# shao-chi/Image-Caption

Measured on AMD Instinct MI355X. Metric: train images/sec @ batch=64, 36×2048 feats, seq_len=20; 1/2/4/8 MI355X, higher is better.
Workload: dtype bf16; 1 GPU; C2 train step: B=64/GPU, N=36 regions x F=2048, P=84, T=20, 6+6 blocks d=512 h=8 f=2048, V=10000, dropout 0.3/0.1, Adam lr 5e-4; global_batch=64, seq_len=20, parallelism=dp1

## Files before the change

image-caption_amd/capgen/_lib.py:

```python
from __future__ import annotations

import ctypes as C
import os

import torch

_HERE = os.path.dirname(os.path.abspath(__file__))
LIB_PATH = os.environ.get("CAPGEN_LIB_PATH") or os.path.join(_HERE, "libcapgen.so")
ABI_VERSION = 13

F32, BF16 = 0, 1


class capgen_config(C.Structure):
    _fields_ = [
        ("num_vocab", C.c_int32), ("max_length", C.c_int32),
        ("dim_features", C.c_int32), ("dim_positions", C.c_int32),
        ("enc_d", C.c_int32), ("enc_ff", C.c_int32), ("enc_blocks", C.c_int32), ("enc_heads", C.c_int32),
        ("dim_word_embedding", C.c_int32),
        ("dec_d", C.c_int32), ("dec_ff", C.c_int32), ("dec_blocks", C.c_int32), ("dec_heads", C.c_int32),
        ("dropout", C.c_float), ("attention_dropout", C.c_float),
        ("pad_idx", C.c_int32), ("encode_mask", C.c_int32), ("focal_loss", C.c_int32),
        ("split_position", C.c_int32), ("split_image_objects", C.c_int32),
        ("move_first_image_feature", C.c_int32),
        ("dtype", C.c_int32), ("max_batch", C.c_int32), ("max_regions", C.c_int32),
        ("lr", C.c_float), ("beta1", C.c_float), ("beta2", C.c_float), ("eps", C.c_float),
        ("seed", C.c_uint64),
    ]


class capgen_param_info(C.Structure):
    _fields_ = [("name", C.c_char * 96), ("ndim", C.c_int32), ("rows", C.c_int64), ("cols", C.c_int64),
                ("offset", C.c_int64), ("row_stride", C.c_int64)]


_P = C.c_void_p
_SIGS = {
    "capgen_last_error": (C.c_char_p, []),
    "capgen_abi_version": (C.c_int, []),
    "capgen_set_knob": (C.c_int, [C.c_char_p, C.c_int, _P]),
    "capgen_debug_build": (C.c_int, []),
    "capgen_param_table": (C.c_int, [C.POINTER(capgen_config), C.POINTER(capgen_param_info), C.c_int,
                                     C.POINTER(C.c_int), C.POINTER(C.c_int64)]),
    "capgen_create": (C.c_int, [C.POINTER(capgen_config), C.c_int, C.POINTER(_P)]),
    "capgen_destroy": (C.c_int, [_P]),
    "capgen_get_params": (C.c_int, [_P, _P, C.c_int64]),
    "capgen_set_params": (C.c_int, [_P, _P, C.c_int64]),
    "capgen_get_grads": (C.c_int, [_P, _P, C.c_int64]),
    "capgen_set_grads": (C.c_int, [_P, _P, C.c_int64]),
    "capgen_get_adam_state": (C.c_int, [_P, C.POINTER(C.c_int64), _P, _P, C.c_int64]),
    "capgen_set_adam_state": (C.c_int, [_P, C.c_int64, _P, _P, C.c_int64]),
    "capgen_arenas": (C.c_int, [_P, C.POINTER(_P), C.POINTER(_P), C.POINTER(C.c_int64)]),
    "capgen_set_training": (C.c_int, [_P, C.c_int]),
    "capgen_set_graph": (C.c_int, [_P, C.c_int]),
    "capgen_set_decode_log_softmax": (C.c_int, [_P, C.c_int]),
    "capgen_set_lr": (C.c_int, [_P, C.c_float]),
    "capgen_get_lr": (C.c_int, [_P, C.POINTER(C.c_float)]),
    "capgen_set_grad_clip": (C.c_int, [_P, C.c_float]),
    "capgen_last_grad_norm": (C.c_int, [_P, C.POINTER(C.c_float)]),
    "capgen_forward": (C.c_int, [_P, _P, C.c_int, _P, _P, C.c_int, C.c_int, C.c_int, _P, _P]),
    "capgen_backward": (C.c_int, [_P, _P]),
    "capgen_adam_step": (C.c_int, [_P, _P]),
    "capgen_train_step": (C.c_int, [_P, _P, C.c_int, _P, _P, C.c_int, C.c_int, C.c_int, _P, _P]),
    "capgen_compute_loss": (C.c_int, [_P, _P, C.c_int, _P, _P, C.c_int, C.c_int, C.c_int, _P, _P]),
    "capgen_copy_logits": (C.c_int, [_P, _P, C.c_int64, _P]),
    "capgen_greedy": (C.c_int, [_P, _P, C.c_int, _P, C.c_int, C.c_int, _P, _P, _P]),
    "capgen_beam": (C.c_int, [_P, _P, C.c_int, _P, C.c_int, C.c_int, C.c_int, _P, _P]),
    "capgen_sample": (C.c_int, [_P, _P, C.c_int, _P, C.c_int, C.c_int, C.c_int, C.c_float, C.c_int, C.c_uint64, _P, _P,
                                _P]),
    "capgen_sample_nucleus": (C.c_int, [_P, _P, C.c_int, _P, C.c_int, C.c_int, C.c_int, C.c_float, C.c_int, C.c_float,
                                        C.c_uint64, _P, _P, _P]),
    "capgen_set_rng_seed": (C.c_int, [_P, C.c_uint64]),
    "capgen_debug_gemm": (C.c_int, [C.c_int, C.c_int, C.c_int, _P, C.c_int64, C.c_int, _P, C.c_int64, C.c_int,
                                    _P, C.c_int64, C.c_int, C.c_int, _P, C.c_float, C.c_int, C.c_int, _P]),
    "capgen_debug_gemm_tiled": (C.c_int, [C.c_int, C.c_int, C.c_int, _P, C.c_int64, _P, C.c_int64, C.c_int, _P, _P,
                                          C.c_int64, C.c_int, _P, C.c_int, C.c_int, _P, C.c_int64, _P]),
    "capgen_debug_gemm_tiled_ln": (C.c_int, [C.c_int, C.c_int, _P, _P, _P, _P, _P, C.c_int, _P, C.c_int, C.c_int, _P, _P,
                                             _P, _P, C.c_int64, C.c_int, _P]),
    "capgen_debug_gemm_variant": (C.c_int, [C.c_int]),
    "capgen_debug_splitk_protocol": (C.c_int, [C.c_int]),
    "capgen_debug_splitk_diag": (C.c_int, [_P, C.c_int]),
    "capgen_debug_gemm_timing_buf": (C.c_int, [_P]),
    "capgen_debug_copy_buffer": (C.c_int, [_P, C.c_int, _P, C.c_int64]),
    "capgen_train_step_indexed": (C.c_int, [_P, _P, C.c_int, _P, C.c_int, _P, _P, C.c_int, C.c_int, C.c_int, _P,
                                            _P]),
    "capgen_train_step_weighted": (C.c_int, [_P, _P, C.c_int, _P, C.c_int, _P, _P, _P, C.c_int, C.c_int, C.c_int, _P,
                                             C.c_int, _P]),
    "capgen_rl_sample": (C.c_int, [_P, _P, C.c_int, _P, _P, C.c_int, C.c_int, C.c_int, _P, _P, _P, _P]),
    "capgen_rl_finish": (C.c_int, [_P, _P, C.c_float, _P, C.c_int, _P]),
    "capgen_debug_attention": (C.c_int, [C.c_int, C.c_int, C.c_int, C.c_int, C.c_int, C.c_int, _P, _P, _P, _P,
                                         C.c_int, C.c_float, _P, _P, _P, _P, _P, _P, _P]),
    "capgen_debug_attention_bwd_wo": (C.c_int, [C.c_int, C.c_int, C.c_int, C.c_int, _P, _P, _P, _P, C.c_int, _P, _P,
                                                _P, _P, _P, _P]),
    "capgen_debug_qkv_attention": (C.c_int, [C.c_int, C.c_int, C.c_int, _P, _P, _P, _P, _P, _P, C.c_int, C.c_int, _P]),
    "capgen_debug_cross_attention": (C.c_int, [C.c_int, C.c_int, C.c_int, C.c_int, _P, _P, _P, _P, _P, _P, _P]),
    "capgen_debug_layernorm_fwd": (C.c_int, [C.c_int, C.c_int, C.c_int, _P, _P, C.c_float, C.c_int, C.c_uint64, _P, _P,
                                             C.c_int, _P, _P, _P, C.c_int64, C.c_int, _P, _P, _P, _P, _P, _P]),
    "capgen_debug_layernorm_bwd": (C.c_int, [C.c_int, C.c_int, C.c_int, _P, _P, _P, _P, _P, _P, C.c_int64, C.c_int, _P,
                                             C.c_float, C.c_int, C.c_uint64, _P, _P, _P, _P, _P, C.c_int, C.c_int64,
                                             _P]),
    "capgen_debug_column_sum": (C.c_int, [C.c_int, _P, C.c_int, C.c_int, C.c_int64, C.c_float, _P, _P, C.c_int,
                                          C.c_int64, _P]),
    "capgen_debug_stripe_reduce": (C.c_int, [_P, C.c_int, C.c_int64, C.c_int64, _P, C.c_int, C.c_int, _P]),
    "capgen_debug_embedding_gather": (C.c_int, [_P, _P, C.c_int64, C.c_int, C.c_int, _P, C.c_int, _P]),
    "capgen_debug_embedding_scatter_add": (C.c_int, [_P, _P, C.c_int, C.c_int, C.c_int, _P, C.c_int, _P]),
    "capgen_debug_pack_encoder_input": (C.c_int, [_P, C.c_int, _P, C.c_int, C.c_int, C.c_int, C.c_int, _P, C.c_int, _P,
                                                  _P, C.c_int, C.c_int, _P, _P]),
    "capgen_debug_prepare_captions": (C.c_int, [_P, C.c_int, C.c_int, C.c_int, _P, _P, _P, _P, _P, _P]),
    "capgen_debug_cross_entropy_rows": (C.c_int, [_P, _P, C.c_int, C.c_int, C.c_int, _P, _P, C.c_int, _P]),
    "capgen_debug_ce_finish": (C.c_int, [_P, C.c_int64, _P, _P, C.c_int, C.c_int, C.c_int, _P, _P, _P]),
    "capgen_debug_cross_entropy_rows_weighted": (C.c_int, [_P, _P, _P, C.c_int, C.c_int, C.c_int, C.c_int, _P, _P,
                                                           C.c_int, _P]),
    "capgen_debug_ce_finish_weighted": (C.c_int, [_P, C.c_int64, _P, _P, _P, C.c_int, C.c_int, C.c_int, C.c_int, _P,
                                                  _P, _P]),
    "capgen_debug_loss_finalize": (C.c_int, [_P, C.c_int, _P, C.c_int, _P, _P, _P, C.c_int, _P]),
    "capgen_debug_adam": (C.c_int, [_P, _P, _P, _P, C.c_int64, C.c_float, C.c_float, C.c_float, C.c_float, _P, _P, _P,
                                    C.c_int64, C.c_int, C.c_int, C.POINTER(C.c_int64), C.POINTER(C.c_int64),
                                    C.POINTER(_P), _P]),
    "capgen_debug_adam_scaled": (C.c_int, [_P, _P, _P, _P, C.c_int64, C.c_float, C.c_float, C.c_float, C.c_float, _P, _P,
                                           _P, C.c_int64, C.c_int, C.c_int, C.POINTER(C.c_int64), C.POINTER(C.c_int64),
                                           C.POINTER(_P), _P, _P]),
    "capgen_debug_grad_norm": (C.c_int, [_P, C.c_int64, C.c_float, C.c_int, _P, C.c_int, _P, _P]),
    "capgen_debug_to_bf16": (C.c_int, [_P, _P, C.c_int64, _P]),
    "capgen_debug_arena_checksum": (C.c_int, [_P, C.c_int64, C.POINTER(C.c_uint64), _P]),
    "capgen_debug_argmax_softmax": (C.c_int, [_P, C.c_int, C.c_int, _P, C.c_int64, C.c_int, _P, C.c_int64, C.c_int,
                                              _P]),
    "capgen_debug_sample_softmax": (C.c_int, [_P, C.c_int, C.c_int, C.c_float, C.c_int, C.c_uint64, C.c_uint32, _P,
                                              C.c_int64, C.c_int, _P, C.c_int64, _P, C.c_int64, C.c_int, _P]),
    "capgen_debug_sample_nucleus": (C.c_int, [_P, C.c_int, C.c_int, C.c_float, C.c_int, C.c_float, C.c_uint64,
                                              C.c_uint32, _P, C.c_int64, C.c_int, _P, C.c_int64, _P, C.c_int64,
                                              C.c_int, _P, _P]),
    "capgen_debug_slab_argmax": (C.c_int, [_P, _P, C.c_int, C.c_int, _P, C.c_int64, C.c_int, _P, C.c_int64, _P]),
    "capgen_debug_beam_step_topk": (C.c_int, [_P, _P, _P, C.c_int, C.c_int, C.c_int, C.c_int, C.c_int, _P, _P, _P, _P,
                                              _P, _P]),
    "capgen_debug_beam_slab_step": (C.c_int, [_P, _P, _P, C.c_int, C.c_int, C.c_int, C.c_int, C.c_int, _P, _P, _P, _P,
                                              _P, C.c_int, _P, _P, _P, _P, C.c_int, C.c_int, _P]),
    "capgen_debug_rl_rows": (C.c_int, [_P, C.c_int, C.c_int, _P, _P, _P, _P, _P]),
    "capgen_debug_rl_image": (C.c_int, [_P, _P, C.c_int, C.c_int, _P, _P, _P]),
    "capgen_debug_rl_numer": (C.c_int, [_P, _P, _P, C.c_int, C.c_int, _P, _P]),
    "capgen_debug_rl_loss": (C.c_int, [_P, _P, C.c_float, _P, _P, _P]),
    "capgen_debug_rl_grad": (C.c_int, [_P, _P, _P, _P, _P, _P, _P, C.c_int, C.c_int, C.c_int, C.c_int, C.c_float, _P,
                                       C.c_int, _P]),
    "capgen_debug_gemm_classifier": (C.c_int, [C.c_int, C.c_int, C.c_int, _P, C.c_int64, _P, C.c_int64, _P, C.c_int64,
                                               _P, _P, C.c_int64, _P, _P, _P]),
    "capgen_dp_unique_id": (C.c_int, [C.c_char_p]),
    "capgen_dp_init": (C.c_int, [_P, C.c_char_p, C.c_int, C.c_int]),
    "capgen_dp_set_global_count": (C.c_int, [_P, C.c_float]),
    "capgen_dp_sync_adam_state": (C.c_int, [_P]),
    "capgen_dp_comm_info": (C.c_int, [_P, _P, _P]),
    "capgen_dp_check": (C.c_int, [_P, _P, _P]),
    "capgen_params_checksum": (C.c_int, [_P, _P]),
    "capgen_dp_buckets": (C.c_int, [_P, _P, _P, C.c_int, _P]),
    "capgen_dp_debug_shard": (C.c_int, [_P, C.c_int, C.c_int]),
    "capgen_tune_load": (C.c_int, [C.c_char_p]),
    "capgen_tune_save": (C.c_int, [C.c_char_p]),
    "capgen_tune_live_count": (C.c_int, []),
    "capgen_debug_hazard": (C.c_int, [C.c_int, C.c_char_p, C.c_int, C.POINTER(C.c_int)]),
    "capgen_debug_side_delay": (C.c_int, [C.c_double]),
    "capgen_debug_collectives": (C.c_int, [_P, C.c_int, C.c_char_p, C.c_int]),
    "capgen_debug_stamps": (C.c_int, [_P, C.c_int, _P, C.c_int, C.c_char_p, C.c_int]),
    "capgen_scst_rewards": (C.c_int, [_P, C.c_int64, _P, C.c_int64, C.c_int, C.c_int, C.c_int, C.c_int, C.c_int,
                                      C.c_int64, C.c_double, C.c_double, _P]),
}
EXPORTED = tuple(_SIGS)

_lib = None


def load():
    global _lib
    if _lib is not None:
        return _lib
    if not os.path.exists(LIB_PATH):
        raise ImportError(f"capgen: {LIB_PATH} is missing — build it with "
                          "`python -c 'import __graft_entry__ as g; g.build()'` (make -C image-caption_amd/csrc)")
    lib = C.CDLL(LIB_PATH)
    for name, (res, args) in _SIGS.items():
        fn = getattr(lib, name)
        fn.restype = res
        fn.argtypes = args
    if lib.capgen_abi_version() != ABI_VERSION:
        raise ImportError("capgen: libcapgen.so ABI version mismatch")
    _lib = lib
    return lib


def check(rc: int) -> None:
    if rc != 0:
        raise RuntimeError("capgen: " + load().capgen_last_error().decode(errors="replace"))


def to_c_config(cfg) -> capgen_config:
    cfg.check_supported()
    c = capgen_config()
    c.num_vocab, c.max_length = cfg.num_vocab, cfg.max_length
    c.dim_features, c.dim_positions = cfg.encode_dim_features, cfg.encode_dim_positions
    c.enc_d, c.enc_ff = cfg.encode_input_size, cfg.encode_hidden_size
    c.enc_blocks, c.enc_heads = cfg.encode_num_blocks, cfg.encode_num_heads
    c.dim_word_embedding = cfg.dim_word_embedding
    c.dec_d, c.dec_ff = cfg.decode_input_size, cfg.decode_hidden_size
    c.dec_blocks, c.dec_heads = cfg.decode_num_blocks, cfg.decode_num_heads
    c.dropout, c.attention_dropout = cfg.dropout, cfg.attention_dropout
    c.pad_idx, c.encode_mask, c.focal_loss = cfg.pad_idx, int(cfg.encode_mask), int(cfg.focal_loss)
    c.split_position = int(cfg.split_position)
    c.split_image_objects = int(cfg.split_image_objects)
    c.move_first_image_feature = int(cfg.move_first_image_feature)
    c.dtype = F32 if cfg.dtype == "fp32" else BF16
    c.max_batch, c.max_regions = cfg.max_batch, cfg.max_regions
    c.lr, c.beta1, c.beta2, c.eps = cfg.learning_rate, cfg.beta1, cfg.beta2, cfg.eps
    c.seed = cfg.seed & 0xFFFFFFFFFFFFFFFF
    return c


def param_table(cfg):
    lib = load()
    c = to_c_config(cfg)
    n = C.c_int(0)
    total = C.c_int64(0)
    check(lib.capgen_param_table(C.byref(c), None, 0, C.byref(n), C.byref(total)))
    arr = (capgen_param_info * n.value)()
    check(lib.capgen_param_table(C.byref(c), arr, n.value, C.byref(n), C.byref(total)))
    out = [(p.name.decode(), p.ndim, p.rows, p.cols, p.offset, p.row_stride) for p in arr]
    return out, total.value


TUNE_TABLE = os.path.join(_HERE, "tune_gfx950.txt")


def tune_save(path: str = TUNE_TABLE) -> int:
    n = load().capgen_tune_save(path.encode())
    if n < 0:
        check(1)
    return n


def tune_load(path: str) -> int:
    return load().capgen_tune_load(path.encode())


def tune_live_count() -> int:
    return load().capgen_tune_live_count()


def hazard_start() -> None:
    check(load().capgen_debug_hazard(1, None, 0, None))


def hazard_stop() -> None:
    check(load().capgen_debug_hazard(0, None, 0, None))


def hazard_check(cap: int = 8192):
    buf = C.create_string_buffer(cap)
    n = C.c_int(0)
    check(load().capgen_debug_hazard(2, buf, cap, C.byref(n)))
    return n.value, buf.value.decode(errors="replace")


def side_delay(us: float) -> None:
    check(load().capgen_debug_side_delay(float(us)))
# ... 11 lines not shown
```

image-caption_amd/csrc/attn_mfma_dev.h:

```cpp
#pragma once
#include "attention.h"

namespace capgen {
namespace amf {

typedef __attribute__((ext_vector_type(8))) __bf16 bf16x8;
typedef __attribute__((ext_vector_type(4))) float f32x4;
typedef __attribute__((ext_vector_type(4))) __bf16 bf16x4;
typedef short s4 __attribute__((ext_vector_type(4)));
typedef __attribute__((address_space(3))) s4 lds_s4;

constexpr int DK = 64;
constexpr int IMG = 64 * 128;

__device__ __forceinline__ int swz(int k, int chunk) { return chunk ^ (((k >> 1) & 3) << 1); }

__device__ __forceinline__ bf16x8 frag_t(const char* img, int cb, int ks, int lane) {
  const int g = lane >> 4, i = lane & 15, q = i >> 2, p = i & 3;
  const int k = ks * 32 + 4 * g + q;
  const int ch = (cb >> 3) + (p >> 1), sub = (p & 1) * 8;
  const s4 lo = __builtin_amdgcn_ds_read_tr16_b64_v4i16((lds_s4*)(img + k * 128 + swz(k, ch) * 16 + sub));
  const s4 hi = __builtin_amdgcn_ds_read_tr16_b64_v4i16((lds_s4*)(img + (k + 16) * 128 + swz(k + 16, ch) * 16 + sub));
  return __builtin_bit_cast(bf16x8, __builtin_shufflevector(lo, hi, 0, 1, 2, 3, 4, 5, 6, 7));
}
// ... 11 lines not shown
                           : uint4{0u, 0u, 0u, 0u};
    }
#pragma unroll
  for (int i = 0; i < NI; ++i)
#pragma unroll
    for (int u = 0; u < 2; ++u) {
      const int c = tid + 256 * u, row = c >> 3, ch = c & 7;
      *reinterpret_cast<uint4*>(img[i] + row * 128 + swz(row, ch) * 16) = v[i][u];
    }
}

__device__ __forceinline__ void stage_key_ok(unsigned char* kok, const AttnGeom& g, int b, int tid) {
  if (tid < 64) {
    const int j = tid;
    bool ok = j < g.Lk;
    if (ok && g.key_valid) ok = g.key_valid[(int64_t)(g.kv_bmod ? b % g.kv_bmod : b) * g.kv_bs + j] != 0;
    if (ok && g.key_ids) ok = g.key_ids[(int64_t)b * g.kid_bs + j] != g.pad_idx;
    kok[j] = ok;
  }
}

__device__ __forceinline__ void put4(char* img, int row, int col, f32x4 v) {
  const bf16x4 b = {(bf16)v[0], (bf16)v[1], (bf16)v[2], (bf16)v[3]};
  *reinterpret_cast<bf16x4*>(img + row * 128 + swz(row, col >> 3) * 16 + (col & 7) * 2) = b;
}

__device__ __forceinline__ bf16x8 frag_r(const char* img, int row, int ks, int lane) {
  return *reinterpret_cast<const bf16x8*>(img + row * 128 + swz(row, ks * 4 + (lane >> 4)) * 16);
}

__device__ __forceinline__ void scores(const char* Aimg, int q0, const char* Bimg, int lane, f32x4 (&s)[4]) {
  const bf16x8 a0 = frag_r(Aimg, q0 + (lane & 15), 0, lane), a1 = frag_r(Aimg, q0 + (lane & 15), 1, lane);
#pragma unroll
  for (int j = 0; j < 4; ++j) {
    s[j] = f32x4{0.f, 0.f, 0.f, 0.f};
    s[j] = __builtin_amdgcn_mfma_f32_16x16x32_bf16(frag_r(Bimg, 16 * j + (lane & 15), 0, lane), a0, s[j], 0, 0, 0);
    s[j] = __builtin_amdgcn_mfma_f32_16x16x32_bf16(frag_r(Bimg, 16 * j + (lane & 15), 1, lane), a1, s[j], 0, 0, 0);
  }
}

__device__ __forceinline__ void softmax_rows(const AttnGeom& g, const unsigned char* kok, int q, int lane,
                                             const f32x4 (&s)[4], f32x4 (&p)[4]) {
  const float inv_t = 1.f / g.temperature;
  float mx = -INFINITY;
  f32x4 x[4];
#pragma unroll
  for (int j = 0; j < 4; ++j)
#pragma unroll
    for (int r = 0; r < 4; ++r) {
      const int key = 16 * j + 4 * (lane >> 4) + r;
      const bool m = !kok[key] || (g.causal && key > g.q_pos0 + q);
      x[j][r] = m ? -INFINITY : s[j][r] * inv_t;
      mx = fmaxf(mx, x[j][r]);
    }
  mx = fmaxf(mx, __shfl_xor(mx, 16, 64));
  mx = fmaxf(mx, __shfl_xor(mx, 32, 64));
  float sum = 0.f;
#pragma unroll
  for (int j = 0; j < 4; ++j)
#pragma unroll
    for (int r = 0; r < 4; ++r) {
      x[j][r] = expf(x[j][r] - mx);
      sum += x[j][r];
    }
  sum += __shfl_xor(sum, 16, 64);
  sum += __shfl_xor(sum, 32, 64);
#pragma unroll
  for (int j = 0; j < 4; ++j)
#pragma unroll
    for (int r = 0; r < 4; ++r) p[j][r] = x[j][r] / sum;
}

__device__ __forceinline__ bf16x8 pack8(const f32x4& lo, const f32x4& hi) {
  return bf16x8{(bf16)lo[0], (bf16)lo[1], (bf16)lo[2], (bf16)lo[3], (bf16)hi[0], (bf16)hi[1], (bf16)hi[2], (bf16)hi[3]};
}

__device__ __forceinline__ void store4(bf16* p, f32x4 v, float mul) {
  *reinterpret_cast<bf16x4*>(p) = bf16x4{(bf16)(v[0] * mul), (bf16)(v[1] * mul), (bf16)(v[2] * mul), (bf16)(v[3] * mul)};
}


__device__ __forceinline__ void attn_fwd_images(const AttnGeom& g, bf16* __restrict__ o, float* __restrict__ probs,
                                                int b, int h, const char* Qimg, const char* Kimg, const char* Vimg,
                                                const unsigned char* kok) {
  const int tid = threadIdx.x, lane = tid & 63, w = tid >> 6;
  const int q0 = 16 * w, q = q0 + (lane & 15);
  if (q0 >= g.Lq) return;
  f32x4 s[4], p[4];
  scores(Qimg, q0, Kimg, lane, s);
  softmax_rows(g, kok, q, lane, s, p);
  const int64_t row_idx = (((int64_t)b * g.H + h) * g.Lq + q) * g.Lk;
  if (probs && q < g.Lq) {
#pragma unroll
    for (int j = 0; j < 4; ++j)
#pragma unroll
      for (int r = 0; r < 4; ++r) {
        const int key = 16 * j + 4 * (lane >> 4) + r;
        if (key < g.Lk) probs[row_idx + key] = p[j][r];
      }
  }
  if (g.drop.seed_ptr) {
    const uint64_t seed = *g.drop.seed_ptr;
#pragma unroll
    for (int j = 0; j < 4; ++j)
#pragma unroll
      for (int r = 0; r < 4; ++r) {
        const int key = 16 * j + 4 * (lane >> 4) + r;
        const bool keep = drop_keep(seed, g.drop.site, (uint32_t)(row_idx + key), g.drop.thresh);
        p[j][r] = keep ? p[j][r] * g.drop.scale : 0.f;
      }
  }
  const bf16x8 pf0 = pack8(p[0], p[1]), pf1 = pack8(p[2], p[3]);
  bf16* ob = o + (int64_t)b * g.o_bs + h * DK;
#pragma unroll
  for (int t = 0; t < 4; ++t) {
    f32x4 acc = f32x4{0.f, 0.f, 0.f, 0.f};
    acc = __builtin_amdgcn_mfma_f32_16x16x32_bf16(frag_t(Vimg, 16 * t, 0, lane), pf0, acc, 0, 0, 0);
    acc = __builtin_amdgcn_mfma_f32_16x16x32_bf16(frag_t(Vimg, 16 * t, 1, lane), pf1, acc, 0, 0, 0);
    if (q < g.Lq) store4(ob + (int64_t)q * g.o_ld + 16 * t + 4 * (lane >> 4), acc, 1.f);
  }
}

__device__ __forceinline__ void attn_fwd_staged(const AttnGeom& g, bf16* __restrict__ o, float* __restrict__ probs,
                                                int b, int h, const char* sm) {
  attn_fwd_images(g, o, probs, b, h, sm, sm + IMG, sm + 2 * IMG, reinterpret_cast<const unsigned char*>(sm + 3 * IMG));
}

__device__ __forceinline__ void attn_fwd_one(const AttnGeom& g, bf16* __restrict__ o, float* __restrict__ probs, int b,
                                             int h, char* sm) {
  char* Qimg = sm;
  char* Kimg = sm + IMG;
  char* Vimg = sm + 2 * IMG;
  unsigned char* kok = reinterpret_cast<unsigned char*>(sm + 3 * IMG);
  const int tid = threadIdx.x;
  const int bk = g.kv_bmod ? b % g.kv_bmod : b;
  {
    char* const img[3] = {Qimg, Kimg, Vimg};
    const bf16* const src[3] = {reinterpret_cast<const bf16*>(g.q) + (int64_t)b * g.q_bs + h * DK,
                                reinterpret_cast<const bf16*>(g.k) + (int64_t)bk * g.k_bs + h * DK,
                                reinterpret_cast<const bf16*>(g.v) + (int64_t)bk * g.v_bs + h * DK};
    const int64_t ld[3] = {g.q_ld, g.k_ld, g.v_ld};
    const int L[3] = {g.Lq, g.Lk, g.Lk};
    stage_images<3>(img, src, ld, L, tid);
    stage_key_ok(kok, g, b, tid);
  }
  __syncthreads();
  attn_fwd_staged(g, o, probs, b, h, sm);
}

__device__ __forceinline__ void attn_bwd_staged(const AttnGeom& g, bf16* __restrict__ dq, bf16* __restrict__ dkp,
                                                bf16* __restrict__ dvp, int b, int h, const char* Kimg,
                                                const char* dOimg, const char* Qimg, const char* Vimg, char* Pdimg,
                                                char* dSimg, const unsigned char* kok) {
  const int tid = threadIdx.x, lane = tid & 63, w = tid >> 6;
  const int64_t qoff = (int64_t)b * g.q_bs + h * DK, koff = (int64_t)b * g.k_bs + h * DK,
                voff = (int64_t)b * g.v_bs + h * DK;
  const int q0 = 16 * w, q = q0 + (lane & 15);
  const float inv_t = 1.f / g.temperature;
  f32x4 ds[4], pd[4];
  if (q0 < g.Lq) {
    f32x4 s[4], p[4], dp[4];
    scores(Qimg, q0, Kimg, lane, s);
    softmax_rows(g, kok, q, lane, s, p);
    scores(dOimg, q0, Vimg, lane, dp);
    const int64_t row_idx = (((int64_t)b * g.H + h) * g.Lq + q) * g.Lk;
    const uint64_t seed = g.drop.seed_ptr ? *g.drop.seed_ptr : 0;
    float rs = 0.f;
#pragma unroll
    for (int j = 0; j < 4; ++j)
#pragma unroll
      for (int r = 0; r < 4; ++r) {
        const int key = 16 * j + 4 * (lane >> 4) + r;
        float d = dp[j][r], pp = p[j][r];
        if (g.drop.seed_ptr) {
          const bool keep = drop_keep(seed, g.drop.site, (uint32_t)(row_idx + key), g.drop.thresh);
          d = keep ? d * g.drop.scale : 0.f;
          pp = keep ? pp * g.drop.scale : 0.f;
        }
        dp[j][r] = d;
        pd[j][r] = pp;
        rs += p[j][r] * d;
      }
    rs += __shfl_xor(rs, 16, 64);
    rs += __shfl_xor(rs, 32, 64);
    const bool live = q < g.Lq;
#pragma unroll
    for (int j = 0; j < 4; ++j)
#pragma unroll
      for (int r = 0; r < 4; ++r) {
        ds[j][r] = live ? p[j][r] * (dp[j][r] - rs) : 0.f;
        pd[j][r] = live ? pd[j][r] : 0.f;
      }
  } else {
#pragma unroll
    for (int j = 0; j < 4; ++j) ds[j] = pd[j] = f32x4{0.f, 0.f, 0.f, 0.f};
  }
#pragma unroll
  for (int j = 0; j < 4; ++j) {
    put4(Pdimg, q, 16 * j + 4 * (lane >> 4), pd[j]);
    put4(dSimg, q, 16 * j + 4 * (lane >> 4), ds[j]);
  }
  __syncthreads();
  if (q0 < g.Lq) {
    const bf16x8 f0 = pack8(ds[0], ds[1]), f1 = pack8(ds[2], ds[3]);
    bf16* dqb = dq + qoff;
#pragma unroll
    for (int t = 0; t < 4; ++t) {
      f32x4 acc = f32x4{0.f, 0.f, 0.f, 0.f};
      acc = __builtin_amdgcn_mfma_f32_16x16x32_bf16(frag_t(Kimg, 16 * t, 0, lane), f0, acc, 0, 0, 0);
      acc = __builtin_amdgcn_mfma_f32_16x16x32_bf16(frag_t(Kimg, 16 * t, 1, lane), f1, acc, 0, 0, 0);
      if (q < g.Lq) store4(dqb + (int64_t)q * g.q_ld + 16 * t + 4 * (lane >> 4), acc, inv_t);
    }
  }
  const int k0 = 16 * w;
  if (k0 >= g.Lk) return;
  const int key = k0 + (lane & 15);
  const int nks = (g.Lq + 31) / 32;
  bf16* dvb = dvp + voff;
  bf16* dkb = dkp + koff;
#pragma unroll
  for (int t = 0; t < 4; ++t) {
    f32x4 av = f32x4{0.f, 0.f, 0.f, 0.f}, ak = f32x4{0.f, 0.f, 0.f, 0.f};
    for (int ks = 0; ks < nks; ++ks) {
      av = __builtin_amdgcn_mfma_f32_16x16x32_bf16(frag_t(dOimg, 16 * t, ks, lane), frag_t(Pdimg, k0, ks, lane), av,
                                                   0, 0, 0);
      ak = __builtin_amdgcn_mfma_f32_16x16x32_bf16(frag_t(Qimg, 16 * t, ks, lane), frag_t(dSimg, k0, ks, lane), ak,
                                                   0, 0, 0);
    }
    if (key < g.Lk) {
      store4(dvb + (int64_t)key * g.v_ld + 16 * t + 4 * (lane >> 4), av, 1.f);
      store4(dkb + (int64_t)key * g.k_ld + 16 * t + 4 * (lane >> 4), ak, inv_t);
    }
  }
}

constexpr int kFwdSmem = 3 * IMG + 64;

}
}
```

image-caption_amd/csrc/capgen_host.h:

```cpp
#pragma once
#include <string>
#include <utility>

namespace capgen {

struct Error {
  std::string msg;
  explicit Error(std::string m) : msg(std::move(m)) {}
};

inline void require(bool ok, const std::string& what) {
  if (!ok) throw Error(what);
}

enum class Knob : int {
  FusedCe, GroupDw, FusedQkv, FusedAttnBwd, ColsumSide, DecodeCrossMfma, SlabDecode, DecodeGroupLds, AttnWave,
  CeVec8, BregDecode, DecodeLnFold, FusedBeamStep, OverlapFront, OverlapDec0, StripeClear, BucketBlocks, Zero, FwdGraph, Streams,
  EventFence, DeferLoss, FrontJoin, ClipAdamGrid, Autotune, AutotuneLog,
  Skip, DebugDropJoin, SplitkProto, AllowPartialLines, DwVariant, HostTiming,
  Count
};
int knob(Knob k);
int knob_set(const char* name, int value, int* old);
bool debug_build();

}
```

image-caption_amd/csrc/engine.hip:

```cpp
#include <rccl/rccl.h>

#include <algorithm>
#include <array>
#include <chrono>
#include <cstdio>
#include <cstdlib>
#include <cmath>
#include <cstring>
#include <map>
#include <memory>
#include <vector>

#include "../../include/capgen.h"
#include "attention.h"
#include "gemm.h"
#include "hazard.h"
#include "layout.h"
#include "ops.h"
#include "qkv_attn.h"
#include "variants.h"
#include "rl.h"

using namespace capgen;

// ... 470 lines not shown
    l.prio = prio(s);
    if (stamp_on) l.stamp = stamp(s, "ln_bwd " + std::to_string(l.M));
    layernorm_bwd(l, act, s);
  }
  void attf(AttnGeom g, void* o, float* probs, DType t, hipStream_t s) {
    g.prio = prio(s);
    if (stamp_on) g.stamp = stamp(s, "attn_fwd " + std::to_string(g.Lq) + "x" + std::to_string(g.Lk));
    attention_fwd(g, o, probs, t, s);
  }
  void attb(AttnGeom g, const float* probs, const void* dout, void* dq, void* dk, void* dv, DType t,
            hipStream_t s) {
    g.prio = prio(s);
    if (stamp_on) g.stamp = stamp(s, "attn_bwd " + std::to_string(g.Lq) + "x" + std::to_string(g.Lk));
    attention_bwd(g, probs, dout, dq, dk, dv, t, s);
  }

  bool fused_qkv_on = knob(Knob::FusedQkv) != 0;
  void self_attention(const void* X, int64_t wqkv, int M, int d, const AttnGeom& g, void* qkv, void* att, float* probs,
                      hipStream_t s) {
    if (fused_qkv_on && act == DType::BF16 && !keep_probs(g)) {
      QkvAttn qa;
      qa.g = g, qa.g.prio = prio(s);
      qa.X = reinterpret_cast<const bf16*>(X), qa.ldx = d, qa.W = WT(wqkv);
      qa.d = d, qa.qkv = reinterpret_cast<bf16*>(qkv), qa.ldqkv = 3 * d, qa.o = reinterpret_cast<bf16*>(att);
      if (qkv_attn_ok(qa)) {
        if (stamp_on) qa.g.stamp = stamp(s, "qkv_attn " + std::to_string(g.Lq) + "x" + std::to_string(g.Lk));
        qkv_attn_fwd(qa, s);
        return;
      }
    }
    linear(X, d, wqkv, d, qkv, 3 * d, act, M, 3 * d, d, nullptr, 0, s);
    attf(g, att, probs, act, s);
  }

  bool cross_fusable(int Lq) const {
    return fused_qkv_on && act == DType::BF16 && wtile && L.dd == 512 && L.Hd * 64 == L.dd && Lq >= 1 && Lq <= 64;
  }
  void cross_attention(const AttnGeom& c, const void* D1, int64_t wq, int d, void* qc, void* attc, float* probs,
                       bool q_done, hipStream_t s) {
    if (!q_done) {
      QkvAttn qa;
      qa.g = c, qa.g.prio = prio(s), qa.cross = 1;
      qa.X = reinterpret_cast<const bf16*>(D1), qa.ldx = d, qa.W = WT(wq);
      qa.d = d, qa.qkv = reinterpret_cast<bf16*>(qc), qa.ldqkv = d, qa.o = reinterpret_cast<bf16*>(attc);
      require(!probs && qkv_attn_ok(qa), "internal: cross-attention geometry the fused launch does not take");
      if (stamp_on) qa.g.stamp = stamp(s, "qkv_attn cross " + std::to_string(c.Lq) + "x" + std::to_string(c.Lk));
      qkv_attn_fwd(qa, s);
      return;
    }
    attf(c, attc, probs, act, s);
  }

  void linear(const void* X, int64_t ldx, int64_t woff, int64_t ldw, void* C, int64_t ldc, DType tout, int M,
              int N, int K, const float* bias, int relu, hipStream_t s, const void* bt = nullptr) {
    GemmArgs ga;
    ga.M = M, ga.N = N, ga.K = K, ga.A = X, ga.lda = ldx, ga.B = W(woff), ga.ldb = ldw, ga.C = C, ga.ldc = ldc;
    ga.bt = bt;
    ga.bias = bias;
    ga.relu = relu;
    ga.prio = prio(s);
    if (stamp_on) ga.stamp = stamp(s, "gemm fwd " + dims(M, N, K));
    gemm(ga, act, tout, false, false, s);
  }
  void linear_ln(const void* X, int64_t ldx, int64_t woff, int64_t ldw, int M, int N, int K, const LnFwd& ln,
                 hipStream_t s) {
    linear(X, ldx, woff, ldw, const_cast<void*>(ln.a), N, act, M, N, K, nullptr, 0, s);
    lnf(ln, s);
  }
  void linear_dx(const void* dY, int64_t ldy, int64_t woff, int64_t ldw, void* dX, int64_t ldx, int M, int N, int K,
                 int beta, const void* relu_aux, const float* alpha_ptr, hipStream_t s, float* colsum = nullptr) {
    GemmArgs ga;
    ga.colsum = colsum;
    ga.colsum_stripes = NSTRIPE, ga.colsum_stride = n_small;
    ga.M = M, ga.N = K, ga.K = N, ga.A = dY, ga.lda = ldy, ga.B = W(woff), ga.ldb = ldw, ga.C = dX, ga.ldc = ldx;
    ga.beta = beta;
    ga.aux = relu_aux;
    ga.ldaux = ldx;
    ga.alpha_ptr = alpha_ptr;
    ga.prio = prio(s);
    if (stamp_on) ga.stamp = stamp(s, "gemm dX " + dims(M, K, N));
    gemm(ga, act, act, false, true, s);
  }
  void linear_dw(const void* dY, int64_t ldy, const void* X, int64_t ldx, int64_t goff, int64_t ldg, int M, int N,
                 int K, const float* alpha_ptr, hipStream_t s) {
    GemmArgs ga;
    ga.M = N, ga.N = K, ga.K = M, ga.A = dY, ga.lda = ldy, ga.B = X, ga.ldb = ldx, ga.C = G(goff), ga.ldc = ldg;
    ga.alpha_ptr = alpha_ptr;
    ga.prio = prio(s);
    if (stamp_on) ga.stamp = stamp(s, "gemm dW " + dims(N, K, M));
    gemm(ga, act, DType::F32, true, true, s);
  }

  void plan_acts(Planner& p, int B, int N, int T) {
    const int64_t Me = (int64_t)B * N, L = T - 1, Md = (int64_t)B * L, d = L_().d, dd = L_().dd;
    const int64_t Mx = std::max(Me, Md);
    const size_t e = es_();
    auto T_ = [&](void*& ptr, int64_t n) { ptr = p.raw(n * e); };
    T_(a.Aenc, Me * L_().Kp);
    p.take(a.valid, Me);
    T_(a.ev0, Me * d);
    p.take(a.em0, Me);
    p.take(a.er0, Me);
    a.X.resize(L_().Le + 1);
    for (auto& x : a.X) T_(x, Me * d);
    a.enc.resize(L_().Le);
    for (auto& l : a.enc) {
      T_(l.qkv, Me * 3 * d);
      p.take(l.P, (size_t)B * L_().He * N * N);
      T_(l.att, Me * d);
      T_(l.v1, Me * d);
      p.take(l.m1, Me);
      p.take(l.r1, Me);
      T_(l.Y, Me * d);
      T_(l.H, Me * L_().fe);
      T_(l.v2, Me * d);
      p.take(l.m2, Me);
      p.take(l.r2, Me);
    }
    T_(a.KV, Me * L_().Ld * 2 * dd);
    p.take(a.ids, Md);
    p.take(a.tgt, Md);
    p.take(a.count, 4);
    T_(a.E, Md * L_().dwe);
    T_(a.dv0, Md * dd);
    T_(a.tmpf, Md * dd);
    p.take(a.dm0, Md);
    p.take(a.dr0, Md);
    a.D.resize(L_().Ld + 1);
    for (auto& x : a.D) T_(x, Md * dd);
    a.dec.resize(L_().Ld);
    for (auto& l : a.dec) {
      T_(l.qkv, Md * 3 * dd);
      p.take(l.Ps, (size_t)B * L_().Hd * L * L);
      T_(l.atts, Md * dd);
      T_(l.vs, Md * dd);
      p.take(l.ms, Md);
      p.take(l.rs, Md);
      T_(l.D1, Md * dd);
      T_(l.qc, Md * dd);
      p.take(l.Pc, (size_t)B * L_().Hd * L * N);
      T_(l.attc, Md * dd);
      T_(l.vc, Md * dd);
      p.take(l.mc, Md);
      p.take(l.rc, Md);
      T_(l.D2, Md * dd);
      T_(l.H, Md * L_().fd);
      T_(l.vf, Md * dd);
      p.take(l.mf, Md);
      p.take(l.rf, Md);
    }
    p.take(a.logits, Md * L_().V);
    T_(a.dlogits, Md * L_().V);
    a.ce_stats = reinterpret_cast<float2*>(p.raw((size_t)Md * ((L_().V + 15) / 16) * sizeof(float2)));
    p.take(a.ce_tl, Md);
    p.take(a.loss_row, Md);
    p.take(a.grad_scale, 4);
    p.take(a.loss, 4);
    p.take(a.loss_ce, 4);
    T_(a.gEnc, Me * d);
    p.take(a.rl_sample, Md);
    p.take(a.rl_lse, Md);
    p.take(a.rl_logp, Md);
    p.take(a.rl_ent, Md);
    p.take(a.rl_ent_img, B);
    p.take(a.rl_score, B);
    p.take(a.rl_scal, 8);
    const int64_t dmax = std::max<int64_t>(std::max(d, dd), L_().dwe);
    T_(a.tmp, Mx * dmax);
    T_(a.gOut, Mx * dmax);
    T_(a.gRes, Mx * dmax);
// ... 199 lines not shown
      hz::record(ev_fj, es2);
    }

    if (L.has_img) image_objects_fwd(B, N, drop_on, s);
    else enc_embed_fwd(Me, true, s);
    const int fj = std::max(0, std::min(front_join, L.Le + 1));
    for (int l = 0; l < L.Le; ++l) {
      if (front && l == fj) hz::wait(s, ev_fj);
      enc_layer_fwd(L.enc[l], a.enc[l], a.X[l], a.X[l + 1], B, N, cfg.encode_mask ? a.valid : nullptr, l, drop_on, s);
    }
    if (front && fj == L.Le) hz::wait(s, ev_fj);
    linear(a.X[L.Le], d, L.Wkv_all, d, a.KV, (int64_t)L.Ld * 2 * dd, act, Me, L.Ld * 2 * dd, d, nullptr, 0, s);

    if (front && fj > L.Le) hz::wait(s, ev_fj);
    else if (!front) dec_embed(a.tmp, s);
    for (int l = 0; l < L.Ld; ++l) {
      const auto& w = L.dec[l];
      auto& A = a.dec[l];
      const bool q_done = front && l == 0;
      if (!q_done) dec_self_half(l, a.tmp, s, !cross_fusable(Lq));
      const AttnGeom c = dec_cross_geom(l, B, Lq, N, drop_on);
      cross_attention(c, A.D1, w.Wq_c, dd, A.qc, A.attc, keep_probs(c) ? A.Pc : nullptr, q_done || !cross_fusable(Lq), s);
      linear_ln(A.attc, dd, w.Wo_c, dd, Md, dd, dd, ln_fwd(dec_cross_site(l, Md, drop_on), a.tmp, A.D1, A.D2), s);
      linear(A.D2, dd, w.W1, dd, A.H, L.fd, act, Md, L.fd, dd, P(w.b1), 1, s);
      linear_ln(A.H, L.fd, w.W2, L.fd, Md, dd, L.fd, ln_fwd(dec_ffn_site(l, Md, drop_on), a.tmp, A.D2, a.D[l + 1]), s);
    }
    if (L.has_mf)
      move_first_fwd(a.D[L.Ld], a.X[L.Le], Md, Lq, 0, N, a.mfU, a.mfH, a.tmp, a.mfOut, true, drop_on, s);
    if (fused_ce()) {
      GemmArgs ga;
      ga.M = Md, ga.N = L.V, ga.K = dd, ga.A = dec_out(), ga.lda = dd, ga.B = W(L.Wc), ga.ldb = dd;
      ga.C = a.dlogits, ga.ldc = L.V, ga.bias = P(L.bc), ga.prio = prio(s);
      ga.ce_stats = a.ce_stats, ga.ce_ld = (L.V + 15) / 16, ga.ce_tgt = a.tgt, ga.ce_tlogit = a.ce_tl;
      if (stamp_on) ga.stamp = stamp(s, "gemm classifier+CE " + dims(Md, L.V, dd));
      gemm(ga, act, act, false, false, s);
      ce_finish(a.ce_stats, (L.V + 15) / 16, a.ce_tl, a.tgt, Md, L.V, cfg.pad_idx, a.loss_row,
                reinterpret_cast<bf16*>(a.dlogits), s, in.w, Lq);
    } else {
      linear(dec_out(), dd, L.Wc, dd, a.logits, L.V, DType::F32, Md, L.V, dd, P(L.bc), 0, s);
      cross_entropy_rows(a.logits, a.tgt, Md, L.V, cfg.pad_idx, a.loss_row, a.dlogits, act, s, in.w, Lq);
    }
    float* lo = loss_out ? loss_out : a.loss;
    last_loss = lo;
    if (comm) {
      loss_finalize(a.loss_row, Md, a.count, 0, a.loss_ce, nullptr, s, nullptr, 1);
      nccl_op(s, "allreduce(ce)", a.loss_ce, 4);
      NCCL_CHECK(ncclAllReduce(a.loss_ce, a.loss_ce, 1, ncclFloat, ncclSum, comm, s));
      loss_finalize(nullptr, 0, a.count, cfg.focal_loss, lo, a.grad_scale, s, a.loss_ce);
    } else if (!defer) {
      loss_finalize(a.loss_row, Md, a.count, cfg.focal_loss, lo, a.grad_scale, s);
    }
    stamp_fwd_end = stamp_next;
  }

  static void dep(hipStream_t from, hipStream_t to, hipEvent_t e) {
    if (from == to) return;
    hz::record(e, from);
    hz::wait(to, e);
  }
  static void memset_async(void* p, size_t bytes, hipStream_t s) {
    if (hz::active()) hz::op(s, "memset", {hz::wr(p, (int64_t)bytes)});
    CAPGEN_HIP(hipMemsetAsync(p, 0, bytes, s));
  }
  bool coll_log_on = false;
  std::vector<std::string> coll_log;
  void nccl_op(hipStream_t s, const char* name, const void* p, int64_t bytes) {
    if (hz::g_log) hz::op(s, name, {hz::wr(p, bytes)});
    if (coll_log_on) {
      const char* role = s == ec ? "bucket" : s == es2 ? "side" : "critical";
      coll_log.push_back(std::string(name) + " " + std::to_string(bytes) + " B on " + role);
    }
  }
  void fork(hipStream_t s) { dep(s, es2, ev_fork); }
  void join(hipStream_t s) {
    flush(s);
    if (!dbg_drop_join) dep(es2, s, ev_join);
  }
  bool dbg_drop_join = knob(Knob::DebugDropJoin) == 1;
  struct DwJob {
    const void *dY, *X;
    int64_t ldy, ldx, goff, ldg;
    int M, N, K;
    const float* alpha_ptr;
  };
  std::vector<DwJob> dw_pending;
  bool group_dw = knob(Knob::GroupDw) != 0;
  void dw_side(const void* dY, int64_t ldy, const void* X, int64_t ldx, int64_t goff, int64_t ldg, int M, int N,
               int K, const float* alpha_ptr, hipStream_t s) {
    if (es2 == s) {
      linear_dw(dY, ldy, X, ldx, goff, ldg, M, N, K, alpha_ptr, s);
      return;
    }
    dw_pending.push_back(DwJob{dY, X, ldy, ldx, goff, ldg, M, N, K, alpha_ptr});
  }
  GemmArgs dw_args(const DwJob& j) const {
    GemmArgs ga;
    ga.M = j.N, ga.N = j.K, ga.K = j.M, ga.A = j.dY, ga.lda = j.ldy, ga.B = j.X, ga.ldb = j.ldx;
    ga.C = G(j.goff), ga.ldc = j.ldg, ga.alpha_ptr = j.alpha_ptr;
    return ga;
  }
  void dw_launch(const DwJob* jobs, size_t n, hipStream_t st) {
    if (act == DType::BF16 && group_dw) {
      std::vector<GemmArgs> probs;
      for (size_t i = 0; i < n; ++i) probs.push_back(dw_args(jobs[i]));
      for (size_t i = 0; i < n; i += kMaxGroup) {
        if (stamp_on) probs[i].stamp = stamp(st, "gemm dW group of " + std::to_string(std::min<size_t>(kMaxGroup, n - i)));
        gemm_grouped(probs.data() + i, (int)std::min<size_t>(kMaxGroup, n - i), DType::F32, true, true, st);
      }
    } else {
      for (size_t i = 0; i < n; ++i) {
        const DwJob& j = jobs[i];
        linear_dw(j.dY, j.ldy, j.X, j.ldx, j.goff, j.ldg, j.M, j.N, j.K, j.alpha_ptr, st);
      }
    }
  }
  struct ColJob {
    const void* X;
    int M, N;
    float* db;
  };
  std::vector<ColJob> col_pending;
  bool colsum_side = knob(Knob::ColsumSide) != 0;
  void flush(hipStream_t s) {
    fork(s);
    dw_launch(dw_pending.data(), dw_pending.size(), es2);
    dw_pending.clear();
    for (const ColJob& j : col_pending) column_sum(j.X, j.M, j.N, j.N, 1.f, nullptr, j.db, act, es2, NSTRIPE, n_small);
    col_pending.clear();
  }
  bool overlap_front = knob(Knob::OverlapFront) != 0;
  bool overlap_dec0 = knob(Knob::OverlapDec0) != 0;
  GemmArgs dx_args(const void* dY, int64_t ldy, int64_t woff, int64_t ldw, void* dX, int64_t ldx, int M, int N,
                   int K, int beta) const {
    GemmArgs ga;
    ga.M = M, ga.N = K, ga.K = N, ga.A = dY, ga.lda = ldy, ga.B = W(woff), ga.ldb = ldw, ga.C = dX, ga.ldc = ldx;
    ga.beta = beta;
    return ga;
  }

  void ffn_bwd(int M, int d, int f, const LnBwd& lb, const void* X, const void* H, int64_t W1, int64_t b1, int64_t W2,
               void* gH, hipStream_t s) {
    lnb(lb, s);
    void* gA = lb.d_a;
    dw_side(gA, d, H, f, W2, f, M, d, f, nullptr, s);
    const bool side = colsum_side && es2 != s;
    linear_dx(gA, d, W2, f, gH, f, M, d, f, 0, H, nullptr, s, side ? nullptr : GS(b1));
    if (side) col_pending.push_back(ColJob{gH, M, f, GS(b1)});
    dw_side(gH, f, X, d, W1, d, M, f, d, nullptr, s);
    linear_dx(gH, f, W1, d, lb.d_res, d, M, f, d, 1, nullptr, nullptr, s);
  }
  void mha_out_bwd(int M, int d, const LnBwd& lb, const void* att, int64_t Wo, void* gATT, hipStream_t s) {
    lnb(lb, s);
    dw_side(lb.d_a, d, att, d, Wo, d, M, d, d, nullptr, s);
    linear_dx(lb.d_a, d, Wo, d, gATT, d, M, d, d, 0, nullptr, nullptr, s);
  }
  bool fused_attn_bwd_on = knob(Knob::FusedAttnBwd) != 0;
  void mha_bwd(int M, int d, const LnBwd& lb, const void* att, int64_t Wo, void* gATT, const AttnGeom& g,
               const float* probs, void* dq, void* dk, void* dv, hipStream_t s) {
    if (fused_attn_bwd_on && act == DType::BF16 && WTo(Wo) && attention_mfma_ok(g)) {
      QkvBwd qb;
      qb.g = g, qb.g.prio = prio(s);
      qb.dA = reinterpret_cast<const bf16*>(lb.d_a), qb.ldda = d, qb.Wt = WTo(Wo);
      qb.dq = reinterpret_cast<bf16*>(dq), qb.dk = reinterpret_cast<bf16*>(dk), qb.dv = reinterpret_cast<bf16*>(dv);
      if (qkv_bwd_ok(qb)) {
        lnb(lb, s);
        dw_side(lb.d_a, d, att, d, Wo, d, M, d, d, nullptr, s);
        if (stamp_on) qb.g.stamp = stamp(s, "attn_bwd_wo " + std::to_string(g.Lq) + "x" + std::to_string(g.Lk));
        qkv_attn_bwd(qb, s);
        return;
      }
    }
    mha_out_bwd(M, d, lb, att, Wo, gATT, s);
    attb(g, probs, gATT, dq, dk, dv, act, s);
  }

  void adam_range(int64_t off, int64_t n, hipStream_t s, int grid_cap = 0, const float* gscale = nullptr) {
    ++wver;
    const int64_t ns = shadow ? std::max<int64_t>(0, std::min(n, L.n_dense - off)) : 0;
    AdamTiles at;
    bool fused_tiles = true;
    for (auto& kv : tiled)
      if (ns > 0 && kv.second.second > 0 && kv.first < off + ns && kv.first + (int64_t)kv.second.second * 512 > off) {
        if (at.n == AdamTiles::kMax || kv.first < off || kv.first + (int64_t)kv.second.second * 512 > off + ns ||
            (kv.first - off) % 4 != 0) {
          fused_tiles = false;
          break;
        }
        at.off[at.n] = kv.first - off, at.len[at.n] = (int64_t)kv.second.second * 512;
        at.dst[at.n++] = wtile + kv.second.first;
      }
    adam_update(params + off, grads + off, am + off, av + off, (size_t)n, cfg.beta1, cfg.beta2, cfg.eps, adam_scal,
                ns > 0 ? shadow + off : nullptr, (size_t)ns, s, grid_cap, fused_tiles ? at : AdamTiles{}, gscale);
    if (ns > 0) retile(off, ns, s, fused_tiles);
  }
  static constexpr int tail_grid = 0;

  bool bstep = false;
  int bucket_blocks = std::max(1, knob(Knob::BucketBlocks));
  void bucket(int64_t off, int64_t n, hipStream_t s, bool sync = true, bool from_s = false) {
    if (sync && !from_s) flush(s);
    if (!bstep) return;
    if (from_s) dep(s, ec, ev_b1);
    else dep(es2, ec, ev_b2);
    bucket_update(off, n);
  }
  void bucket_update(int64_t off, int64_t n, int grid_cap = 0) {
    ++wver;
    zbuckets.push_back({off, n});
    bucket_reduce(off, n);
    if (clip_on()) {
      gn_deferred.push_back({off, n, grid_cap});
      return;
    }
    bucket_adam(off, n, grid_cap, nullptr);
  }
  bool bucket_sharded(int64_t n) const { return zsharded() && n % (4 * zworld()) == 0; }
  void bucket_reduce(int64_t off, int64_t n) {
    const int zw = zworld();
    const bool sharded = bucket_sharded(n);
    int64_t noff = off, nn = n;
    if (sharded) {
      const int64_t c = n / zw, o = off + (int64_t)zrank() * c;
      if (zw > 1) moments_sharded = true;
      if (comm && zw > 1) grads_sharded = true;
      if (comm) {
        nccl_op(ec, "reduce_scatter", grads + off, n * 4);
        NCCL_CHECK(ncclReduceScatter(grads + off, grads + o, (size_t)c, ncclFloat, ncclSum, comm, ec));
        noff = o, nn = c;
      }
    } else if (comm) {
      nccl_op(ec, "allreduce(bucket)", grads + off, n * 4);
// ... 73 lines not shown
  }

  void move_first_bwd(int Md, bool on, hipStream_t s) {
    const int dd = L.dd, fd = L.fd;
    lnb(ln_bwd(move_first_site(Md, on), a.gOut, a.gRes, a.mfGA), s);
    dw_side(a.mfGA, dd, a.mfH, fd, L.mf_W2, fd, Md, dd, fd, nullptr, s);
    linear_dx(a.mfGA, dd, L.mf_W2, fd, a.mfGH, fd, Md, dd, fd, 0, a.mfH, nullptr, s, GS(L.mf_b1));
    dw_side(a.mfGH, fd, a.mfU, dd, L.mf_W1, dd, Md, fd, dd, nullptr, s);
    linear_dx(a.mfGH, fd, L.mf_W1, dd, a.mfGU, dd, Md, fd, dd, 0, nullptr, nullptr, s);
    add_inplace(a.gRes, a.mfGU, (int64_t)Md * dd, act, s);
  }

  bool dec0_on_side = false;
  void backward(hipStream_t s, bool step_params = false) {
    bstep = step_params;
    require(fB > 0, "backward: call forward first");
    grads_sharded = false;
    stamp_next = stamp_fwd_end;
    const int B = fB, N = fN, Lq = fT - 1, Me = B * N, Md = B * Lq, d = L.d, dd = L.dd;
    const bool on = fwd_drop;
    const bool emb_zero_side = es2 != s && !L.has_img && !L.has_mf;
    if (!emb_zero_side) memset_async(grads + L.n_dense, (L.enc_lng - L.n_dense) * sizeof(float), s);
    if (stripes_dirty || !stripe_clear) memset_async(gstripe, (size_t)NSTRIPE * n_small * sizeof(float), s);
    stripes_dirty = true;
    int folds = 0;
    if (bstep) {
      hipStreamCaptureStatus cst = hipStreamCaptureStatusNone;
      CAPGEN_HIP(hipStreamIsCapturing(s, &cst));
      adam_prepare(step, opt, cfg.beta1, cfg.beta2, adam_scal, cst == hipStreamCaptureStatusNone ? ec : s);
      zbuckets.clear();
      gn_deferred.clear();
      gn_slots = 0;
    }

    dw_side(a.dlogits, L.V, dec_out(), dd, L.Wc, dd, Md, L.V, dd, a.grad_scale, s);
    linear_dx(a.dlogits, L.V, L.Wc, dd, a.gOut, dd, Md, L.V, dd, 0, nullptr, a.grad_scale, s);
    flush(s);
    bucket(L.Wc, L.n_dense - L.Wc, s, false);
    if (emb_zero_side) memset_async(grads + L.n_dense, (L.enc_lng - L.n_dense) * sizeof(float), es2);
    column_sum(a.dlogits, Md, L.V, L.V, 1.f, a.grad_scale, GS(L.bc), act, es2, NSTRIPE, n_small);
    if (pending_loss) {
      loss_finalize(a.loss_row, Md, a.count, 0, pending_loss, nullptr, es2);
      pending_loss = nullptr;
    }

    const int64_t kvld = (int64_t)L.Ld * 2 * dd;
    void* gO = a.gOut;
    void* gR = a.gRes;
    if (L.has_mf) {
      move_first_bwd(Md, on, s);
      std::swap(gO, gR);
    }
    for (int l = L.Ld - 1; l >= 0; --l) {
      const auto& w = L.dec[l];
      auto& A = a.dec[l];
      auto& gb = a.gdec[l];
      const LnBwd lffn = ln_bwd(dec_ffn_site(l, Md, on), gO, gR, gb.gAf);
      const LnBwd lcross = ln_bwd(dec_cross_site(l, Md, on), gR, gO, gb.gA2);
      const LnBwd lself = ln_bwd(dec_self_site(l, Md, on), gO, gR, gb.gA1);
      ffn_bwd(Md, dd, L.fd, lffn, A.D2, A.H, w.W1, w.b1, w.W2, gb.gH, s);
      mha_bwd(Md, dd, lcross, A.attc, w.Wo_c, gb.gATT2, dec_cross_geom(l, B, Lq, N, on), A.Pc, gb.gQc,
              at(a.gKV, (int64_t)l * 2 * dd), at(a.gKV, (int64_t)l * 2 * dd + dd), s);
      const bool ov = l == 0 && overlap_dec0 && es2 != s;
      const hipStream_t hs = ov ? es2 : s;
      if (ov) flush(s);
      dw_side(gb.gQc, dd, A.D1, dd, w.Wq_c, dd, Md, dd, dd, nullptr, hs);
      linear_dx(gb.gQc, dd, w.Wq_c, dd, gO, dd, Md, dd, dd, 1, nullptr, nullptr, hs);
      mha_bwd(Md, dd, lself, A.atts, w.Wo_s, gb.gATT1, dec_self_geom(l, B, Lq, on), A.Ps, gb.gQKV, at(gb.gQKV, dd),
              at(gb.gQKV, 2 * dd), hs);
      dw_side(gb.gQKV, 3 * dd, a.D[l], dd, w.Wqkv, dd, Md, 3 * dd, dd, nullptr, hs);
      linear_dx(gb.gQKV, 3 * dd, w.Wqkv, dd, gR, dd, Md, 3 * dd, dd, 1, nullptr, nullptr, hs);
      if (l % bucket_blocks == 0)
        bucket(w.Wqkv, dec_end(std::min(l + bucket_blocks - 1, L.Ld - 1)) - w.Wqkv, hs);
      if (ov) dec0_on_side = true;
      std::swap(gO, gR);
    }
    void* eO = dec0_on_side ? a.gEnc : gO == a.gOut ? a.gRes : a.gOut;
    dec0_on_side = false;
    {
      const LnBwd lb = ln_bwd(dec_embed_site(Md), gO, nullptr, a.gAd);
      flush(s);
      lnb(lb, es2);
      linear_dx(a.gAd, dd, L.Wel, L.dwe, a.gE, L.dwe, Md, dd, L.dwe, 0, nullptr, nullptr, es2);
      const DwJob wel{a.gAd, a.E, dd, L.dwe, L.Wel, L.dwe, Md, dd, L.dwe, nullptr};
      dw_launch(&wel, 1, es2);
      embedding_scatter_add(a.gE, a.ids, Md, L.dwe, cfg.pad_idx, G(L.emb), act, es2, L.V);
      stripe_reduce(GS(L.dec_lng), NSTRIPE, n_small, L.total - L.dec_lng, G(L.dec_lng), 0, es2, stripe_clear);
      ++folds;
    }
    gO = eO;
    gR = a.tmp;
    linear_dx(a.gKV, kvld, L.Wkv_all, d, gO, d, Me, L.Ld * 2 * dd, d, 0, nullptr, nullptr, s);
    if (L.has_mf) first_region_grad(a.mfGU, B, Lq, N, d, gO, act, s);
    dw_side(a.gKV, kvld, a.X[L.Le], d, L.Wkv_all, d, Me, L.Ld * 2 * dd, d, nullptr, s);
    bucket(L.Wkv_all, L.Wc - L.Wkv_all, s);
    bucket(L.Wel, L.dec[0].Wqkv - L.Wel, s, false);
    bucket(L.emb, L.enc_lng - L.emb, s, false);
    bucket(L.dec_lng, L.total - L.dec_lng, s, false);
    for (int l = L.Le - 1; l >= 0; --l) {
      const auto& w = L.enc[l];
      enc_layer_bwd(w, a.enc[l], a.genc[l], a.X[l], B, N, cfg.encode_mask ? a.valid : nullptr, l, on, gO, gR, s);
      if (l % bucket_blocks == 0) bucket(w.Wqkv, enc_end(std::min(l + bucket_blocks - 1, L.Le - 1)) - w.Wqkv, s);
    }
    if (L.has_img) {
      image_objects_bwd(gO, B, N, on, s);
      flush(s);
    } else {
      lnb(ln_bwd(enc_embed_site(Me), gO, nullptr, a.gAe), s);
      linear_dw(a.gAe, d, a.Aenc, L.Kp, L.enc_emb_W, L.Kp, Me, d, L.Kp, nullptr, s);
    }
    const hipStream_t tail = bstep ? ec : s;
    if (!bstep) join(s);
    if (bstep) dep(s, ec, ev_b1);
    if (bstep && L.has_img) dep(es2, ec, ev_b2);
    stripe_reduce(GS(L.enc_lng), NSTRIPE, n_small, L.dec_lng - L.enc_lng, G(L.enc_lng), 0, tail, stripe_clear);
    if (++folds == 2) stripes_dirty = false;
    if (bstep) {
      bucket_update(0, L.enc[0].Wqkv, tail_grid);
      bucket_update(L.enc_lng, L.dec_lng - L.enc_lng, tail_grid);
      if (clip_on()) clip_tail();
    }
    join(s);
    if (bstep) {
      dep(ec, s, ev_cj);
      bstep = false;
      check_buckets();
    }
  }

  void allreduce_grads(hipStream_t s) {
    if (!comm) return;
    nccl_op(s, "allreduce(grads)", grads, L.total * 4);
    NCCL_CHECK(ncclAllReduce(grads, grads, (size_t)L.total, ncclFloat, ncclSum, comm, s));
  }

  void adam(hipStream_t s) {
    ++wver;
    adam_prepare(step, opt, cfg.beta1, cfg.beta2, adam_scal, s);
    const float* gscale = nullptr;
    if (clip_on()) {
      const int slots = grad_sumsq(grads, (size_t)L.total, gn_part, gn_slots_cap, s);
      grad_norm_finish(gn_part, slots, nullptr, opt + 1, 0.f, opt + 2, 3, s);
      gscale = opt + 3;
      norm_valid = true;
    }
    adam_update(params, grads, am, av, (size_t)L.total, cfg.beta1, cfg.beta2, cfg.eps, adam_scal, shadow,
                shadow ? (size_t)L.n_dense : 0, s, 0, AdamTiles{}, gscale);
    if (shadow) retile(0, L.n_dense, s);
  }

  void refresh_shadow(hipStream_t s) {
    if (shadow) to_bf16(params, shadow, (size_t)L.n_dense, s);
    if (shadow) retile(0, L.n_dense, s);
  }

  void enter(hipStream_t cs) {
    hz::record(ev_in, cs);
    hz::wait(es, ev_in);
    hz::set_critical(es);
  }
  void leave(hipStream_t cs) {
    hz::record(ev_out, es);
    hz::wait(cs, ev_out);
  }

  bool dp_checked = false;
  float* dp_chk = nullptr;
// ... 810 lines not shown
}

int capgen_copy_logits(capgen_t* h, float* dst, int64_t n, void* stream) {
  return guarded([&] {
    set_device(h);
    require(h->fB > 0, "copy_logits: no forward yet");
    const int64_t want = (int64_t)h->fB * (h->fT - 1) * h->L.V;
    require(n == want, "copy_logits: size mismatch");
    hipStream_t cs = (hipStream_t)stream;
    h->enter(cs);
    if (h->fused_ce())
      h->linear(h->dec_out(), h->L.dd, h->L.Wc, h->L.dd, h->a.logits, h->L.V, DType::F32, h->fB * (h->fT - 1),
                h->L.V, h->L.dd, h->P(h->L.bc), 0, h->es);
    CAPGEN_HIP(hipMemcpyAsync(dst, h->a.logits, n * 4, hipMemcpyDeviceToDevice, h->es));
    h->leave(cs);
  });
}

int capgen_greedy(capgen_t* h, const void* feats, int ft, const float* pos, int B, int N, int64_t* ids_out,
                  float* attn_out, void* stream) {
  return guarded([&] {
    set_device(h);
    hipStream_t cs = (hipStream_t)stream;
    h->enter(cs);
    h->greedy(feats, dt(ft), pos, B, N, ids_out, attn_out, h->es);
    h->leave(cs);
  });
}

int capgen_beam(capgen_t* h, const void* feats, int ft, const float* pos, int B, int N, int k, int64_t* ids_out,
                void* stream) {
  return guarded([&] {
    set_device(h);
    hipStream_t cs = (hipStream_t)stream;
    h->enter(cs);
    h->beam(feats, dt(ft), pos, B, N, k, ids_out, h->es);
    h->leave(cs);
  });
}

int capgen_sample(capgen_t* h, const void* feats, int ft, const float* pos, int B, int N, int n_samples,
                  float temperature, int top_k, uint64_t sd, int64_t* ids_out, float* logp_out, void* stream) {
  return guarded([&] {
    set_device(h);
    hipStream_t cs = (hipStream_t)stream;
    h->enter(cs);
    h->sample(feats, dt(ft), pos, B, N, n_samples, temperature, top_k, 1.f, sd, ids_out, logp_out, h->es);
    h->leave(cs);
  });
}

int capgen_sample_nucleus(capgen_t* h, const void* feats, int ft, const float* pos, int B, int N, int n_samples,
                          float temperature, int top_k, float top_p, uint64_t sd, int64_t* ids_out, float* logp_out,
                          void* stream) {
  return guarded([&] {
    set_device(h);
    hipStream_t cs = (hipStream_t)stream;
    h->enter(cs);
    h->sample(feats, dt(ft), pos, B, N, n_samples, temperature, top_k, top_p, sd, ids_out, logp_out, h->es);
    h->leave(cs);
  });
}

int capgen_set_rng_seed(capgen_t* h, uint64_t sd) {
  return guarded([&] {
    set_device(h);
    hz::host_sync(h->es);
    CAPGEN_HIP(hipMemcpy(h->seed, &sd, 8, hipMemcpyHostToDevice));
  });
}

int capgen_debug_gemm(int M, int N, int K, const void* A, int64_t lda, int ta, const void* B, int64_t ldb, int tb,
                      void* Cp, int64_t ldc, int in_dtype, int out_dtype, const float* bias, float alpha, int beta,
                      int relu, void* stream) {
  return guarded([&] {
    gemm_init();
    GemmArgs ga;
    ga.M = M, ga.N = N, ga.K = K, ga.A = A, ga.lda = lda, ga.B = B, ga.ldb = ldb, ga.C = Cp, ga.ldc = ldc;
    ga.bias = bias, ga.alpha = alpha, ga.beta = beta, ga.relu = relu;
    gemm(ga, dt(in_dtype), dt(out_dtype), ta != 0, tb != 0, (hipStream_t)stream);
  });
}

int capgen_debug_gemm_tiled(int M, int N, int K, const void* A, int64_t lda, const void* B, int64_t ldb, int tb,
                            void* Bt, void* Cp, int64_t ldc, int out_dtype, const float* bias, int beta, int relu,
                            const void* aux, int64_t ldaux, void* stream) {
  return guarded([&] {
    gemm_init();
    const hipStream_t s = (hipStream_t)stream;
    gemm_tile_b(reinterpret_cast<const bf16*>(B), ldb, tb, N, K, reinterpret_cast<bf16*>(Bt), s);
    GemmArgs ga;
    ga.M = M, ga.N = N, ga.K = K, ga.A = A, ga.lda = lda, ga.B = B, ga.ldb = ldb, ga.C = Cp, ga.ldc = ldc;
    ga.bias = bias, ga.beta = beta, ga.relu = relu, ga.aux = aux, ga.ldaux = ldaux, ga.bt = Bt;
    require(gemm_breg_ok(ga), "debug_gemm_tiled: a shape / epilogue the register-B kernel does not take");
    gemm(ga, DType::BF16, dt(out_dtype), false, tb != 0, s);
  });
}

int capgen_debug_gemm_tiled_ln(int M, int N, const void* A, const void* ln_res, const void* B, void* Bt, void* Cp,
                               int out_dtype, const float* bias, int beta, int relu, const float* ln_gamma,
                               const float* ln_beta, void* ln_y, const int32_t* ln_ids, int64_t ln_ids_ld, int ln_pad,
                               void* stream) {
  return guarded([&] {
    gemm_init();
    const hipStream_t s = (hipStream_t)stream;
    const int K = 512;
    gemm_tile_b(reinterpret_cast<const bf16*>(B), K, 0, N, K, reinterpret_cast<bf16*>(Bt), s);
    GemmArgs ga;
    ga.M = M, ga.N = N, ga.K = K, ga.A = A, ga.lda = K, ga.B = B, ga.ldb = K, ga.C = Cp, ga.ldc = N;
    ga.bias = bias, ga.beta = beta, ga.relu = relu, ga.bt = Bt;
    ga.ln_res = ln_res, ga.ln_gamma = ln_gamma, ga.ln_beta = ln_beta, ga.ln_y = ln_y;
    ga.ln_ids = ln_ids, ga.ln_ids_ld = ln_ids_ld, ga.ln_pad = ln_pad;
    require(ln_gamma && gemm_breg_ok(ga), "debug_gemm_tiled_ln: a shape the folded-LayerNorm kernel does not take");
    gemm(ga, DType::BF16, dt(out_dtype), false, false, s);
  });
}

int capgen_train_step_indexed(capgen_t* h, const void* feat_store, int feats_dtype, const float* pos_store,
                              int n_images, const int32_t* img_idx, const int32_t* caps, int B, int N, int T,
                              float* loss_out, void* stream) {
  return guarded([&] {
    set_device(h);
    require(n_images >= 1, "train_step_indexed: empty store");
    {
      Scoped<StepIn> inputs(h->in, StepIn{img_idx, n_images, nullptr});
      h->train_step(feat_store, dt(feats_dtype), pos_store, caps, B, N, T, loss_out, (hipStream_t)stream);
    }
    h->dp_check((hipStream_t)stream, loss_out);
  });
}

int capgen_train_step_weighted(capgen_t* h, const void* feats, int feats_dtype, const float* pos, int n_images,
                               const int32_t* img_idx, const int32_t* caps, const float* weights, int B, int N, int T,
                               float* loss_out, int train, void* stream) {
  return guarded([&] {
    set_device(h);
    require(weights != nullptr, "train_step_weighted: weights is null");
    require(!h->cfg.focal_loss, "train_step_weighted: focal_loss transforms an unweighted mean");
    require(!img_idx || n_images >= 1, "train_step_weighted: empty store");
    hipStream_t cs = (hipStream_t)stream;
    const DType ft = dt(feats_dtype);
    Scoped<StepIn> inputs(h->in, StepIn{img_idx, img_idx ? n_images : 0, weights});
    if (train) {
      h->train_step(feats, ft, pos, caps, B, N, T, loss_out, cs);
      h->dp_check(cs, loss_out);
    } else {
      h->ensure_acts(B, N, T);
      h->enter(cs);
      h->forward(feats, ft, pos, caps, B, N, T, loss_out, h->training, h->es);
      h->leave(cs);
    }
  });
}

int capgen_debug_cross_entropy_rows_weighted(const float* logits, const int32_t* tgt, const float* row_w,
                                             int rows_per_w, int M, int V, int pad, float* loss_row, void* dlogits,
                                             int dtype, void* stream) {
  return guarded([&] {
    require(row_w != nullptr, "debug_cross_entropy_rows_weighted: row_w is null");
    require(rows_per_w >= 1 && M % rows_per_w == 0,
            "debug_cross_entropy_rows_weighted: rows_per_w must be >= 1 and divide M");
    cross_entropy_rows(logits, tgt, M, V, pad, loss_row, dlogits, dt(dtype), (hipStream_t)stream, row_w, rows_per_w);
  });
}

int capgen_debug_ce_finish_weighted(const void* stats, int64_t ld, const float* tlogit, const int32_t* tgt,
// ... 339 lines not shown

int capgen_debug_beam_step_topk(const float* logits, const void* stats, const float* prev, int k_in, int B, int V,
                                int k, int logsm, float* cand_v, int32_t* cand_i, float* out_prob, int32_t* out_src,
                                int32_t* out_tok, void* stream) {
  return guarded([&] {
    const hipStream_t s = (hipStream_t)stream;
    if (stats)
      beam_step_topk_slab(logits, reinterpret_cast<const float2*>(stats), prev, k_in, B, V, k, logsm, cand_v, cand_i,
                          out_prob, out_src, out_tok, s);
    else
      beam_step_topk(logits, prev, k_in, B, V, k, logsm, cand_v, cand_i, out_prob, out_src, out_tok, s);
  });
}

int capgen_debug_beam_slab_step(const float* logits, const void* stats, const float* prev, int k_in, int B, int V,
                                int k, int logsm, float* out_prob, int32_t* out_src, int32_t* out_tok,
                                const int64_t* seq_src, int64_t* seq_dst, int Tw, const int32_t* ids_src,
                                int32_t* ids_dst, const int32_t* kv_src, int32_t* kv_dst, int Tc, int t, void* stream) {
  return guarded([&] {
    require(t >= 0, "debug_beam_slab_step: t >= 0");
    beam_slab_step(logits, reinterpret_cast<const float2*>(stats), prev, k_in, B, V, k, logsm, out_prob, out_src,
                   out_tok, seq_src, seq_dst, Tw, ids_src, ids_dst, kv_src, kv_dst, Tc, t, (hipStream_t)stream);
  });
}

int capgen_debug_rl_rows(const float* logits, int M, int V, int32_t* sample, float* lse, float* logp_s, float* ent,
                         void* stream) {
  return guarded([&] {
    require(M >= 1 && V >= 1, "debug_rl_rows: M, V >= 1");
    rl_rows(logits, M, V, sample, lse, logp_s, ent, (hipStream_t)stream);
  });
}

int capgen_debug_rl_image(const int32_t* sample, const float* ent, int B, int L, float* ent_img, float* scal,
                          void* stream) {
  return guarded([&] { rl_image(sample, ent, B, L, ent_img, scal, (hipStream_t)stream); });
}

int capgen_debug_rl_numer(const int32_t* sample, const float* logp_s, const float* score, int B, int L, float* scal,
                          void* stream) {
  return guarded([&] { rl_numer(sample, logp_s, score, B, L, scal, (hipStream_t)stream); });
}

int capgen_debug_rl_loss(const float* scal, const float* lm, float w, float* out, float* grad_scale, void* stream) {
  return guarded([&] { rl_loss(scal, lm, w, out, grad_scale, (hipStream_t)stream); });
}

int capgen_debug_rl_grad(const float* logits, const int32_t* tgt, const int32_t* sample, const float* lse,
                         const float* score, const float* count, const float* scal, int B, int L, int V, int pad,
                         float w, void* dl, int dtype, void* stream) {
  return guarded([&] {
    require(B >= 1 && L >= 1 && V >= 1, "debug_rl_grad: B, L, V >= 1");
    rl_grad(logits, tgt, sample, lse, score, count, scal, B, L, V, pad, w, dl, dt(dtype), (hipStream_t)stream);
  });
}

int capgen_debug_gemm_classifier(int M, int N, int K, const void* A, int64_t lda, const void* B, int64_t ldb, void* Cp,
                                 int64_t ldc, const float* bias, void* stats, int64_t stats_ld, const int32_t* ce_tgt,
                                 float* ce_tlogit, void* stream) {
  return guarded([&] {
    require(stats != nullptr, "debug_gemm_classifier: stats is required");
    gemm_init();
    GemmArgs ga;
    ga.M = M, ga.N = N, ga.K = K, ga.A = A, ga.lda = lda, ga.B = B, ga.ldb = ldb, ga.C = Cp, ga.ldc = ldc;
    ga.bias = bias;
    if (ce_tgt) {
      ga.ce_stats = reinterpret_cast<float2*>(stats), ga.ce_ld = stats_ld, ga.ce_tgt = ce_tgt, ga.ce_tlogit = ce_tlogit;
      gemm(ga, DType::BF16, DType::BF16, false, false, (hipStream_t)stream);
    } else {
      ga.dec_stats = reinterpret_cast<float2*>(stats), ga.dec_ld = stats_ld;
      gemm(ga, DType::BF16, DType::F32, false, false, (hipStream_t)stream);
    }
  });
}

int capgen_debug_copy_buffer(capgen_t* h, int which, void* host_dst, int64_t bytes) {
  return guarded([&] {
    set_device(h);
    require(h->ws != nullptr, "debug_copy_buffer: no workspace yet");
    const int Le = h->L.Le;
    void* src = which == 0 ? h->a.tmp : which == 1 ? h->a.gOut : which == 2 ? h->a.gRes : which == 3 ? h->a.gKV
              : which == 4 ? h->a.genc[Le - 1].gH : which == 5 ? h->a.genc[Le - 1].gAf
              : which == 6 ? h->a.genc[Le - 1].gA1 : which == 7 ? h->a.genc[Le - 1].gQKV
              : which >= 32 && (which - 32) / 8 < Le && (which - 32) % 8 < 5
                  ? (&h->a.genc[(which - 32) / 8].gAf)[(which - 32) % 8 == 0 ? 0 : (which - 32) % 8 == 1 ? 1
                                                        : (which - 32) % 8 == 2 ? 2 : (which - 32) % 8 == 3 ? 3 : 4]
              : which >= 80 && which - 80 <= Le ? h->a.X[which - 80]
              : which >= 128 && (which - 128) / 8 < Le
                  ? ((which - 128) % 8 == 0 ? h->a.enc[(which - 128) / 8].att
                     : (which - 128) % 8 == 1 ? h->a.enc[(which - 128) / 8].v1
                     : (which - 128) % 8 == 2 ? (void*)h->a.enc[(which - 128) / 8].m1
                     : (which - 128) % 8 == 3 ? (void*)h->a.enc[(which - 128) / 8].r1
                     : (which - 128) % 8 == 4 ? h->a.enc[(which - 128) / 8].Y
                     : (which - 128) % 8 == 5 ? h->a.enc[(which - 128) / 8].v2
                     : (which - 128) % 8 == 6 ? (void*)h->a.enc[(which - 128) / 8].m2
                                             : (void*)h->a.enc[(which - 128) / 8].r2)
              : which >= 200 && which - 200 < Le ? h->a.enc[which - 200].H
              : which >= 216 && which - 216 < h->L.Ld ? h->a.dec[which - 216].H
                  : nullptr;
    require(src != nullptr,
            "debug_copy_buffer: which in 0..7, 32 + 8 l + 0..4, 80 + 0..Le, 128 + 8 l + 0..7, 200 + l, 216 + l");
    hz::host_sync(nullptr);
    CAPGEN_HIP(hipMemcpy(host_dst, src, (size_t)bytes, hipMemcpyDeviceToHost));
  });
}

int capgen_debug_gemm_timing_buf(void* dev_buf) {
  return guarded([&] { gemm_set_timing_buf(reinterpret_cast<uint64_t*>(dev_buf)); });
}

int capgen_debug_splitk_diag(int* out4, int reset) {
  return guarded([&] { gemm_splitk_diag(out4, reset != 0); });
}

int capgen_debug_splitk_protocol(int proto) {
  return guarded([&] {
    require(proto >= 0 && proto < 8192, "debug_splitk_protocol: bits 0..12 only (10-12: ablation build)");
    gemm_set_splitk_protocol(proto);
  });
}

int capgen_tune_load(const char* path) {
  int n = -1;
  const int rc = guarded([&] {
    require(path != nullptr, "tune_load: null path");
    n = gemm_tune_load(path);
  });
  return rc ? -2 : n;
}
int capgen_tune_save(const char* path) {
  int n = -1;
  const int rc = guarded([&] {
    require(path != nullptr, "tune_save: null path");
    n = gemm_tune_save(path);
    require(n >= 0, std::string("tune_save: cannot write ") + path);
  });
  return rc ? -2 : n;
}
int capgen_tune_live_count(void) { return gemm_tune_live_count(); }

int capgen_debug_hazard(int op, char* report, int cap, int* n_conflicts) {
  return guarded([&] {
    require(op >= 0 && op <= 2, "debug_hazard: op 0 (off), 1 (on + clear) or 2 (check)");
    if (op == 0) return hz::enable(false);
    if (op == 1) {
      hz::reset();
      return hz::enable(true);
    }
    std::string rep;
    const int n = hz::check(&rep);
    if (n_conflicts) *n_conflicts = n;
    if (report && cap > 0) {
      const size_t k = std::min<size_t>(rep.size(), (size_t)cap - 1);
      std::memcpy(report, rep.data(), k);
      report[k] = 0;
    }
  });
}
int capgen_debug_collectives(capgen_t* h, int op, char* out, int cap) {
  return guarded([&] {
    require(h != nullptr, "null engine handle");
    require(op >= 0 && op <= 2, "debug_collectives: op 0 (off), 1 (on + clear) or 2 (dump)");
    if (op < 2) {
      h->coll_log_on = op == 1;
      h->coll_log.clear();
      return;
    }
    std::string all;
    for (auto& l : h->coll_log) all += l + "\n";
    if (out && cap > 0) {
      const size_t k = std::min<size_t>(all.size(), (size_t)cap - 1);
      std::memcpy(out, all.data(), k);
      out[k] = 0;
    }
  });
}

int capgen_debug_stamps(capgen_t* h, int op, double* out, int cap, char* names, int names_cap) {
  int count = 0;
  const int rc = guarded([&] {
    require(h != nullptr, "null engine handle");
    require(op >= 0 && op <= 3, "debug_stamps: op 0 (off), 1 (on), 2 (read), 3 (arm)");
    set_device(h);
    if (op == 0 || op == 1) {
      hz::host_sync(nullptr);
      h->stamp_on = op == 1;
      if (h->stamp_on && !h->stamp_ring)
// ... 139 lines not shown
```

image-caption_amd/csrc/gemm.h:

```cpp
#pragma once
#include <type_traits>

#include "capgen_common.h"

namespace capgen {

enum class DType : int { F32 = 0, BF16 = 1 };

inline size_t dsize(DType t) { return t == DType::F32 ? 4 : 2; }

struct GemmArgs {
  int M = 0, N = 0, K = 0, pad0_ = 0;
  const void* A = nullptr;
  int64_t lda = 0;
  const void* B = nullptr;
  int64_t ldb = 0;
  void* C = nullptr;
  int64_t ldc = 0;
  const float* bias = nullptr;
  const void* aux = nullptr;
  int64_t ldaux = 0;
  float alpha = 1.f;
  int pad1_ = 0;
  const float* alpha_ptr = nullptr;
  int beta = 0;
  int prio = 0;
  const void* bt = nullptr;
  int64_t bt_pad_ = 0;
  void* C2 = nullptr;
  int64_t ldc2 = 0;
  int nsplit = 0;
  int relu = 0;
  float* colsum = nullptr;
  int colsum_stripes = 1;
  int pad2_ = 0;
  int64_t colsum_stride = 0;
  float2* ce_stats = nullptr;
  int64_t ce_ld = 0;
  const int32_t* ce_tgt = nullptr;
  float* ce_tlogit = nullptr;
  float2* dec_stats = nullptr;
  int64_t dec_ld = 0;
  uint64_t* stamp = nullptr;
  const float* ln_gamma = nullptr;
  const float* ln_beta = nullptr;
  void* ln_y = nullptr;
  const int32_t* ln_ids = nullptr;
  int64_t ln_ids_ld = 0;
  int ln_pad = 0;
  int a_table_rows = 0;
  const void* ln_res = nullptr;
  const int32_t* a_ids = nullptr;
  int64_t a_ids_ld = 0;
};
static_assert(sizeof(GemmArgs) == 16 + 36 * 8, "GemmArgs must have no padding");

constexpr int kMaxGroup = 8;
struct GemmGroup {
  int n = 0;
  int start[kMaxGroup + 1] = {};
  int tiles_n[kMaxGroup] = {};
  GemmArgs p[kMaxGroup];
};
static_assert(sizeof(GemmGroup) == 4 * (1 + 2 * kMaxGroup + 1) + kMaxGroup * sizeof(GemmArgs), "GemmGroup must have no padding");

void gemm(const GemmArgs& g, DType in, DType out, bool ta, bool tb, hipStream_t s);
bool gemm_breg_ok(const GemmArgs& g);
void gemm_breg(const GemmArgs& g, DType out, hipStream_t s);
void gemm_tile_b(const bf16* B, int64_t ldb, int tb, int N, int K, bf16* Bt, hipStream_t s);
void gemm_init();
void gemm_set_variant(int v);
void gemm_set_splitk_protocol(int p);
void gemm_set_timing_buf(uint64_t* p);
void gemm_splitk_diag(int* out4, bool reset);
void gemm_grouped(const GemmArgs* probs, int n, DType out, bool ta, bool tb, hipStream_t s);
void gemm_bf16(const GemmArgs& g, DType out, bool ta, bool tb, hipStream_t s);

int gemm_tune_load(const char* path);
int gemm_tune_save(const char* path);
int gemm_tune_live_count();

}
```

image-caption_amd/csrc/gemm.hip:

```cpp
#include <chrono>
#include <cstdio>
#include <vector>
#include "gemm.h"
#include "hazard.h"
#include "ops.h"

namespace capgen {

typedef __attribute__((ext_vector_type(8))) __bf16 bf16x8;
typedef __attribute__((ext_vector_type(4))) float f32x4;

template <typename T> struct GemmTraits;
template <> struct GemmTraits<float> {
  static constexpr int VEC = 4;
  static constexpr int PAD = 4;
};
template <> struct GemmTraits<bf16> {
  static constexpr int VEC = 8;
  static constexpr int PAD = 8;
};

constexpr int BK = 32;
constexpr int NTHREADS = 256;

// ... 134 lines not shown
          for (int j = 0; j < FN; ++j)
            acc[i][j] = __builtin_amdgcn_mfma_f32_16x16x4f32(af[i], bfr[j], acc[i][j], 0, 0, 0);
      }
    }
    if (kt + 1 < nk) {
      la.store(As[cur ^ 1], tid);
      lb.store(Bs[cur ^ 1], tid);
    }
    __syncthreads();
  }

  if constexpr (sizeof(T) == 4) {
    if (nk > KP1) {
#pragma unroll
      for (int i = 0; i < FM; ++i)
#pragma unroll
        for (int j = 0; j < FN; ++j) acc[i][j] = tot[i][j] + (mid[i][j] + acc[i][j]);
    }
  }
  const float alpha = g.alpha_ptr ? g.alpha * *g.alpha_ptr : g.alpha;
  TO* __restrict__ C = reinterpret_cast<TO*>(g.C);
  const T* __restrict__ aux = reinterpret_cast<const T*>(g.aux);
#pragma unroll
  for (int i = 0; i < FM; ++i) {
#pragma unroll
    for (int j = 0; j < FN; ++j) {
      const int n = n0 + wn * (BN / 2) + j * 16 + fr;
      if (n >= g.N) continue;
      const float bn = g.bias ? g.bias[n] : 0.f;
#pragma unroll
      for (int r = 0; r < 4; ++r) {
        const int m = m0 + wm * (BM / 2) + i * 16 + fq * 4 + r;
        if (m >= g.M) continue;
        float v = alpha * acc[i][j][r] + bn;
        if (aux && !(to_f(aux[(int64_t)m * g.ldaux + n]) > 0.f)) v = 0.f;
        if (g.relu) v = fmaxf(v, 0.f);
        TO* cp = C + (int64_t)m * g.ldc + n;
        if (g.beta) v += to_f(*cp);
        *cp = from_f<TO>(v);
      }
    }
  }
}

template <typename T, typename TO, bool TA, bool TB>
static void launch_tiles(const GemmArgs& g, hipStream_t s) {
  auto blocks = [&](int bm, int bn) { return (long)((g.M + bm - 1) / bm) * ((g.N + bn - 1) / bn); };
  if (blocks(128, 128) >= 240) {
    dim3 grid((g.N + 127) / 128, (g.M + 127) / 128);
    gemm_kernel<T, TO, TA, TB, 128, 128><<<grid, NTHREADS, 0, s>>>(g);
  } else if (blocks(128, 64) >= 240) {
    dim3 grid((g.N + 63) / 64, (g.M + 127) / 128);
    gemm_kernel<T, TO, TA, TB, 128, 64><<<grid, NTHREADS, 0, s>>>(g);
  } else {
    dim3 grid((g.N + 63) / 64, (g.M + 63) / 64);
    gemm_kernel<T, TO, TA, TB, 64, 64><<<grid, NTHREADS, 0, s>>>(g);
  }
}

template <typename T, typename TO>
static void launch_layout(const GemmArgs& g, bool ta, bool tb, hipStream_t s) {
  if (!ta && !tb) launch_tiles<T, TO, false, false>(g, s);
  else if (!ta && tb) launch_tiles<T, TO, false, true>(g, s);
  else if (ta && !tb) launch_tiles<T, TO, true, false>(g, s);
  else launch_tiles<T, TO, true, true>(g, s);
}

void gemm_hz_regions(const GemmArgs& g, DType in, DType out, bool ta, bool tb, std::vector<hz::Rgn>& v) {
  using namespace hz;
  const int64_t ei = dsize(in), eo = dsize(out);
  const int ncol = g.C2 ? g.nsplit : g.N;
  v.push_back(g.a_ids ? blk(g.A, g.a_table_rows, g.K * ei, g.lda * ei, RD)
                      : ta ? blk(g.A, g.K, g.M * ei, g.lda * ei, RD) : blk(g.A, g.M, g.K * ei, g.lda * ei, RD));
  v.push_back(blk(g.a_ids, g.a_ids ? g.M : 0, 4, g.a_ids_ld * 4, RD));
  v.push_back(tb ? blk(g.B, g.K, g.N * ei, g.ldb * ei, RD) : blk(g.B, g.N, g.K * ei, g.ldb * ei, RD));
  v.push_back(blk(g.C, g.M, ncol * eo, g.ldc * eo, WR));
  if (g.beta) v.push_back(blk(g.C, g.M, ncol * eo, g.ldc * eo, RD));
  if (g.C2) v.push_back(blk(g.C2, g.M, (int64_t)(g.N - g.nsplit) * eo, g.ldc2 * eo, WR));
  v.push_back(blk(g.aux, g.M, g.N * ei, g.ldaux * ei, RD));
  v.push_back(rd(g.bt, (int64_t)g.N * g.K * 2));
  v.push_back(rd(g.bias, g.N * 4));
  v.push_back(rd(g.alpha_ptr, 4));
  v.push_back(blk(g.colsum, g.colsum_stripes, g.N * 4, g.colsum_stride * 4, ACC));
  v.push_back(blk(g.ce_stats, g.M, (int64_t)((g.N + 15) / 16) * 8, g.ce_ld * 8, WR));
  v.push_back(blk(g.dec_stats, g.M, (int64_t)((g.N + 15) / 16) * 8, g.dec_ld * 8, WR));
  v.push_back(rd(g.ce_tgt, (int64_t)g.M * 4));
  v.push_back(wr(g.ce_tlogit, (int64_t)g.M * 4));
  v.push_back(rd(g.ln_gamma, g.K * 4));
  v.push_back(rd(g.ln_beta, g.K * 4));
  v.push_back(blk(g.ln_ids, g.ln_ids ? g.M : 0, 4, g.ln_ids_ld * 4, RD));
  v.push_back(wr(g.ln_y, (int64_t)g.M * g.K * 2));
  v.push_back(rd(g.ln_res, (int64_t)g.M * g.K * 2));
}

static void gemm_impl(const GemmArgs& g, DType in, DType out, bool ta, bool tb, hipStream_t s);
void gemm(const GemmArgs& g, DType in, DType out, bool ta, bool tb, hipStream_t s) {
  if (!knob(Knob::HostTiming)) return gemm_impl(g, in, out, ta, tb, s);
  static double tot = 0;
  static long n = 0;
  const auto t0 = std::chrono::steady_clock::now();
  gemm_impl(g, in, out, ta, tb, s);
  tot += std::chrono::duration<double, std::micro>(std::chrono::steady_clock::now() - t0).count();
  if (++n % 2000 == 0) {
    std::fprintf(stderr, "[capgen host] gemm() call: %.2f us average over 2000\n", tot / 2000);
    tot = 0;
  }
}
static void gemm_impl(const GemmArgs& g, DType in, DType out, bool ta, bool tb, hipStream_t s) {
  if (g.M <= 0 || g.N <= 0) return;
  if ((skip_mask() & 16) && out == DType::F32) return;
  if ((skip_mask() & 64) && out == DType::BF16) return;
  const int vec = in == DType::F32 ? 4 : 8;
  require((ta ? g.M : g.K) % vec == 0 && g.lda % vec == 0, "gemm: A contiguous dim/ld not a multiple of 16 B");
  require((tb ? g.N : g.K) % vec == 0 && g.ldb % vec == 0, "gemm: B contiguous dim/ld not a multiple of 16 B");
  require(((uintptr_t)g.A & 15) == 0 && ((uintptr_t)g.B & 15) == 0, "gemm: operands must be 16-B aligned");
  require(g.K > 0, "gemm: K must be positive");
  require(!g.colsum || !g.beta, "gemm: colsum requires beta == 0");
  require(!g.bt || (in == DType::BF16 && !ta), "gemm: a tiled B (bt) needs the bf16 path with A stored [M][K]");
  require(!g.dec_stats || in == DType::BF16, "gemm: dec_stats is a bf16-path epilogue output");
  require(!g.a_ids || (in == DType::BF16 && !ta && !tb && g.bt && gemm_breg_ok(g) && g.a_table_rows > 0),
          "gemm: gathered A rows (a_ids) need the register-B path");
  require(!g.ln_gamma || (in == DType::BF16 && !ta && !tb && g.bt && gemm_breg_ok(g)),
          "gemm: a folded LayerNorm (ln_gamma) needs the register-B path (bf16, bt, K = 512)");
  require(!g.C2 || (in == DType::BF16 && g.nsplit % 4 == 0 && !g.beta && !g.colsum),
          "gemm: a split output (C2) needs the bf16 path, nsplit % 4 == 0, no beta / colsum");
  if (hz::active()) {
    std::vector<hz::Rgn> v;
    gemm_hz_regions(g, in, out, ta, tb, v);
    hz::op(s, ta ? "gemm TN (dW)" : tb ? "gemm NN (dX)" : "gemm NT (fwd)", v.data(), v.size());
  }
  if (in == DType::F32) {
    if (out == DType::F32) launch_layout<float, float>(g, ta, tb, s);
    else launch_layout<float, bf16>(g, ta, tb, s);
    if (g.colsum) column_sum(g.C, g.M, g.N, g.ldc, 1.f, nullptr, g.colsum, out, s, g.colsum_stripes, g.colsum_stride);
  } else {
    gemm_bf16(g, out, ta, tb, s);
  }
  CAPGEN_HIP(hipGetLastError());
}

}
```

image-caption_amd/csrc/gemm_bf16.hip:

```cpp
#include <chrono>
#include <algorithm>
#include <dlfcn.h>
#include <string>
#include <cmath>
#include <cstdio>
#include <cstdlib>
#include <map>
#include <mutex>
#include <tuple>
#include <vector>

#include <cstring>
#include "gemm.h"
#include "hazard.h"
#include "gemm_tile.h"
#include "tune_parse.h"

namespace capgen {

void gemm_hz_regions(const GemmArgs& g, DType in, DType out, bool ta, bool tb, std::vector<hz::Rgn>& v);

namespace {
void* g_zero_page[64] = {};
}


template <typename TO, bool TA, bool TB, int BM, int BN, int WM, int WN, int STAGES, int KG = 1>
__global__ void __launch_bounds__(64 * WM * WN * KG) gemm_bf16_kernel(GemmArgs g, int tiles_n, int nblk,
                                                                     const void* zero, int splitk, float* ws,
                                                                     int* tile_cnt, int group_m, int proto) {
  __shared__ __attribute__((aligned(1024))) char smem[TileCfg<TA, TB, BM, BN, WM, WN, STAGES, KG>::SMEM];
  StampScope stamp_scope(g.stamp);
  if (g.prio) __builtin_amdgcn_s_setprio(3);
  const int slot = xcd_slot(blockIdx.x, nblk);
  const int tile = slot / splitk, split = slot % splitk;
  int mt = tile / tiles_n, nt = tile % tiles_n;
  if (group_m > 1) {
    const int tiles_m = (g.M + BM - 1) / BM, per = group_m * tiles_n, first = (tile / per) * group_m;
    const int gsz = min(tiles_m - first, group_m), r = tile % per;
    mt = first + r % gsz, nt = r / gsz;
  }
  gemm_tile<TO, TA, TB, BM, BN, WM, WN, STAGES, KG>(g, mt, nt, tile, split, splitk, zero, ws, tile_cnt, smem, proto);
}

template <typename TO, bool TA, bool TB, int BM, int BN, int WM, int WN, int STAGES>
__global__ void __launch_bounds__(64 * WM * WN) gemm_bf16_grouped_kernel(GemmGroup gg, int nblk, int G,
                                                                        const void* zero) {
  __shared__ __attribute__((aligned(1024))) char smem[TileCfg<TA, TB, BM, BN, WM, WN, STAGES>::SMEM];
  StampScope stamp_scope(gg.p[0].stamp);
  for (int b = blockIdx.x; b < nblk; b += G) {
    if (b != (int)blockIdx.x) __syncthreads();
    const int slot = xcd_slot(b, nblk);
    int q = 0;
    while (q + 1 < gg.n && slot >= gg.start[q + 1]) ++q;
    const int tile = slot - gg.start[q];
    const int mt = tile / gg.tiles_n[q], nt = tile % gg.tiles_n[q];
    gemm_tile<TO, TA, TB, BM, BN, WM, WN, STAGES>(gg.p[q], mt, nt, tile, 0, 1, zero, nullptr, nullptr, smem);
  }
}

template <typename TO, bool TA, bool TB, int BM, int BN, int WM, int WN, int STAGES>
__global__ void __launch_bounds__(64 * WM * WN) gemm_bf16_grouped_dev_kernel(const GemmGroup* __restrict__ ggp,
                                                                            int nblk, int G, const void* zero) {
  __shared__ __attribute__((aligned(1024))) char smem[TileCfg<TA, TB, BM, BN, WM, WN, STAGES>::SMEM];
  const GemmGroup& gg = *ggp;
  StampScope stamp_scope(gg.p[0].stamp);
  for (int b = blockIdx.x; b < nblk; b += G) {
    if (b != (int)blockIdx.x) __syncthreads();
    const int slot = xcd_slot(b, nblk);
    int q = 0;
    while (q + 1 < gg.n && slot >= gg.start[q + 1]) ++q;
    const int tile = slot - gg.start[q];
    const int mt = tile / gg.tiles_n[q], nt = tile % gg.tiles_n[q];
    gemm_tile<TO, TA, TB, BM, BN, WM, WN, STAGES>(gg.p[q], mt, nt, tile, 0, 1, zero, nullptr, nullptr, smem);
  }
}

struct Workspace {
  float* p = nullptr;
  size_t bytes = 0;
  int* cnt = nullptr;
};
constexpr int kMaxTiles = 1 << 16;
std::map<hipStream_t, Workspace> g_ws;
int g_splitk_proto = 0;
std::mutex g_ws_mu;
uint64_t* g_timing_buf = nullptr;

void ensure_ws(hipStream_t s, size_t bytes) {
  std::lock_guard<std::mutex> lk(g_ws_mu);
  Workspace& w = g_ws[s];
  if (!w.cnt) {
    CAPGEN_HIP(hipMalloc(&w.cnt, kMaxTiles * sizeof(int)));
    CAPGEN_HIP(hipMemsetAsync(w.cnt, 0, kMaxTiles * sizeof(int), s));
  }
  if (w.bytes >= bytes) return;
  static std::vector<float*> retired;
  if (w.p) retired.push_back(w.p);
  CAPGEN_HIP(hipMalloc(&w.p, bytes));
  w.bytes = bytes;
}
Workspace get_ws(hipStream_t s) {
  std::lock_guard<std::mutex> lk(g_ws_mu);
  auto it = g_ws.find(s);
  return it == g_ws.end() ? Workspace{} : it->second;
}

template <typename TO, bool TA, bool TB, int BM, int BN, int WM, int WN, int ST, int KG = 1>
static void launch_cfg(const GemmArgs& g, hipStream_t s, int splitk) {
  require(KG == 1 || splitk == 1, "gemm: k-group variants run without grid split-K");
  const int tn = (g.N + BN - 1) / BN, tm = (g.M + BM - 1) / BM;
  const int nblk = tn * tm * splitk;
  int dev = 0;
  CAPGEN_HIP(hipGetDevice(&dev));
  float* ws = nullptr;
  int* cnt = nullptr;
  if (splitk > 1) {
    const size_t bytes = (size_t)tn * tm * splitk * BM * BN * sizeof(float);
    const Workspace w = get_ws(s);
    require(w.bytes >= bytes && w.cnt, "gemm: split-K workspace too small (tune outside capture)");
    require(tn * tm <= kMaxTiles, "gemm: too many tiles for split-K");
    ws = w.p, cnt = w.cnt;
    if (g_splitk_proto & 32) {
      static std::map<hipStream_t, int> rot;
      cnt += (rot[s]++ & 3) * (kMaxTiles / 4);
      require(tn * tm <= kMaxTiles / 4, "gemm: too many tiles for ticket rotation");
    }
    if (g_splitk_proto & 8) CAPGEN_HIP(hipMemsetAsync(cnt, 0, (size_t)(tn * tm + 3) / 4 * 16, s));
  }
  int group_m = 0;
  {
    const double per_xcd = (double)tn * tm / 8.0;
    group_m = std::max(1, std::min(tm, (int)std::lround(std::sqrt(per_xcd))));
  }
  GemmArgs gk = g;
  if ((g_splitk_proto & 4096) && g_timing_buf) gk.stamp = g_timing_buf;
  gemm_bf16_kernel<TO, TA, TB, BM, BN, WM, WN, ST, KG>
      <<<nblk, 64 * WM * WN * KG, 0, s>>>(gk, tn, nblk, g_zero_page[dev], splitk, ws, cnt, group_m, g_splitk_proto & ~8);
}

size_t splitk_bytes(const GemmArgs& g, int splitk) {
  return (size_t)((g.M + 255) / 256 * 256) * ((g.N + 127) / 128 * 128) * splitk * sizeof(float);
}

int g_variant = 0;

constexpr int NVARIANTS = 30;
const char* kVariantName[NVARIANTS + 1] = {"auto",        "128x128w4s3", "128x128w8s2",  "128x128w4s2",
                                           "128x64w4s2",  "64x128w4s2",  "64x64w4s2",    "64x64w4s3",
                                           "128x64w8s2",  "256x128w16s2", "128x128w16s2", "256x64w8s2",
                                           "64x64w4s4",   "64x64w4s6",   "128x64w4s4",   "64x128w4s4",
                                           "128x128w4s4", "32x64w4s2",   "64x32w4s2",    "32x32w4s2",
                                           "64x64w8s2",   "32x64w4s3",   "64x32w4s3",
                                           "64x64w4k2s2", "64x64w4k2s3", "32x64w4k2s3", "64x64w4k4s2",
                                           "32x64w4k4s2", "128x64w4k2s2", "64x128w4k2s2", "32x64w4k2s2"};

constexpr int kVariantBN[NVARIANTS + 1] = {0,  128, 128, 128, 64, 128, 64, 64, 64, 128, 128, 64,
// ... 208 lines not shown
  GroupTable& t = g_group_table[dev];
  auto& bucket = t.by_hash[h];
  for (auto& e : bucket)
    if (std::memcmp(&e.first, &gg, sizeof(GemmGroup)) == 0) return e.second;
  if (t.used >= kGroupTableCap) return nullptr;
  hipStreamCaptureStatus st = hipStreamCaptureStatusNone;
  CAPGEN_HIP(hipStreamIsCapturing(s, &st));
  if (st != hipStreamCaptureStatusNone) return nullptr;
  if (!t.dev) CAPGEN_HIP(hipMalloc(&t.dev, sizeof(GemmGroup) * kGroupTableCap));
  GemmGroup* slot = t.dev + t.used++;
  CAPGEN_HIP(hipMemcpy(slot, &gg, sizeof(GemmGroup), hipMemcpyHostToDevice));
  bucket.push_back({gg, slot});
  return slot;
}

template <typename TO, bool TA, bool TB, int BM, int BN, int WM, int WN, int ST>
static void launch_group_cfg(const GemmArgs* ps, int n, hipStream_t s) {
  int dev = 0;
  CAPGEN_HIP(hipGetDevice(&dev));
  GemmGroup gg;
  gg.n = n;
  int tot = 0;
  for (int i = 0; i < n; ++i) {
    const int tn = (ps[i].N + BN - 1) / BN, tm = (ps[i].M + BM - 1) / BM;
    gg.start[i] = tot, gg.tiles_n[i] = tn, gg.p[i] = ps[i];
    tot += tn * tm;
  }
  gg.start[n] = tot;
  static const int cap = [] {
    int n = 0, dev = 0;
    CAPGEN_HIP(hipGetDevice(&dev));
    CAPGEN_HIP(hipDeviceGetAttribute(&n, hipDeviceAttributeMultiprocessorCount, dev));
    return std::max(8, n / 8 * 8);
  }();
  const int G = cap > 0 ? std::min(tot, cap) : tot;
  if (const GemmGroup* d = grouped_args_dev(gg, dev, s))
    gemm_bf16_grouped_dev_kernel<TO, TA, TB, BM, BN, WM, WN, ST><<<G, 64 * WM * WN, 0, s>>>(d, tot, G, g_zero_page[dev]);
  else
    gemm_bf16_grouped_kernel<TO, TA, TB, BM, BN, WM, WN, ST><<<G, 64 * WM * WN, 0, s>>>(gg, tot, G, g_zero_page[dev]);
}

constexpr int kGroupVariants[] = {6, 20, 17, 18, 19, 4, 8, 1, 3, 10};

template <typename TO, bool TA, bool TB>
static void launch_group_variant(int v, const GemmArgs* ps, int n, hipStream_t s) {
  switch (v) {
    case 1: return launch_group_cfg<TO, TA, TB, 128, 128, 2, 2, 3>(ps, n, s);
    case 3: return launch_group_cfg<TO, TA, TB, 128, 128, 2, 2, 2>(ps, n, s);
    case 4: return launch_group_cfg<TO, TA, TB, 128, 64, 2, 2, 2>(ps, n, s);
    case 6: return launch_group_cfg<TO, TA, TB, 64, 64, 2, 2, 2>(ps, n, s);
    case 8: return launch_group_cfg<TO, TA, TB, 128, 64, 4, 2, 2>(ps, n, s);
    case 10: return launch_group_cfg<TO, TA, TB, 128, 128, 4, 4, 2>(ps, n, s);
    case 17: return launch_group_cfg<TO, TA, TB, 32, 64, 2, 2, 2>(ps, n, s);
    case 18: return launch_group_cfg<TO, TA, TB, 64, 32, 2, 2, 2>(ps, n, s);
    case 19: return launch_group_cfg<TO, TA, TB, 32, 32, 2, 2, 2>(ps, n, s);
    case 20: return launch_group_cfg<TO, TA, TB, 64, 64, 4, 2, 2>(ps, n, s);
    default: throw Error("gemm_grouped: unknown variant");
  }
}

std::map<std::vector<int>, int> g_group_tuned;

template <typename TO, bool TA, bool TB>
static void launch_group(const GemmArgs* ps, int n, hipStream_t s) {
  std::vector<int> key{TA, TB, (int)sizeof(TO)};
  for (int i = 0; i < n; ++i) key.insert(key.end(), {ps[i].M, ps[i].N, ps[i].K});
  int v = g_variant % 100;
  if (v == 0) {
    std::lock_guard<std::mutex> lk(g_tune_mu);
    auto it = g_group_tuned.find(key);
    if (it != g_group_tuned.end()) {
      v = it->second;
    } else {
      v = kGroupVariants[0];
      hipStreamCaptureStatus st = hipStreamCaptureStatusNone;
      CAPGEN_HIP(hipStreamIsCapturing(s, &st));
      if (st == hipStreamCaptureStatusNone && autotune_enabled()) {
        CAPGEN_HIP(hipDeviceSynchronize());
        ++g_live_tuned;
        std::vector<GemmArgs> t(ps, ps + n);
        std::vector<void*> scratch(n);
        for (int i = 0; i < n; ++i) {
          CAPGEN_HIP(hipMalloc(&scratch[i], (size_t)t[i].M * t[i].ldc * sizeof(TO)));
          t[i].C = scratch[i], t[i].beta = 0, t[i].colsum = nullptr, t[i].stamp = nullptr;
        }
        hipEvent_t e0, e1;
        CAPGEN_HIP(hipEventCreate(&e0));
        CAPGEN_HIP(hipEventCreate(&e1));
        float best = 1e30f;
        for (int cand : kGroupVariants) {
          if (!whole_lines<TO>(cand)) continue;
          const float ms = tune_time([&] { launch_group_variant<TO, TA, TB>(cand, t.data(), n, s); }, s, e0, e1);
          if (ms < best) best = ms, v = cand;
        }
        CAPGEN_HIP(hipEventDestroy(e0));
        CAPGEN_HIP(hipEventDestroy(e1));
        for (void* p : scratch) CAPGEN_HIP(hipFree(p));
        CAPGEN_HIP(hipStreamSynchronize(s));
        g_group_tuned[key] = v;
        if (knob(Knob::AutotuneLog))
          std::fprintf(stderr, "[capgen gemm] group of %d (M=%d N=%d K=%d first) -> %s (%.2f us)\n", n, ps[0].M,
                       ps[0].N, ps[0].K, kVariantName[v], best * 1e3f / 3);
      }
    }
  }
  launch_group_variant<TO, TA, TB>(v, ps, n, s);
}

static void gemm_grouped_impl(const GemmArgs* ps, int n, DType out, bool ta, bool tb, hipStream_t s);
void gemm_grouped(const GemmArgs* ps, int n, DType out, bool ta, bool tb, hipStream_t s) {
  if (!knob(Knob::HostTiming)) return gemm_grouped_impl(ps, n, out, ta, tb, s);
  static double tot = 0;
  static long cnt = 0;
  const auto t0 = std::chrono::steady_clock::now();
  gemm_grouped_impl(ps, n, out, ta, tb, s);
  tot += std::chrono::duration<double, std::micro>(std::chrono::steady_clock::now() - t0).count();
  if (++cnt % 500 == 0) {
    std::fprintf(stderr, "[capgen host] gemm_grouped() call: %.2f us average over 500\n", tot / 500);
    tot = 0;
  }
}
static void gemm_grouped_impl(const GemmArgs* ps, int n, DType out, bool ta, bool tb, hipStream_t s) {
  require(n >= 1 && n <= kMaxGroup, "gemm_grouped: 1..kMaxGroup problems");
  if ((skip_mask() & 16) && out == DType::F32) return;
  int dev = 0;
  CAPGEN_HIP(hipGetDevice(&dev));
  require(g_zero_page[dev] != nullptr, "gemm: gemm_init() not called on this device");
  for (int i = 0; i < n; ++i) {
    const GemmArgs& g = ps[i];
    require(g.M > 0 && g.N > 0 && g.K > 0 && g.N % 4 == 0 && g.ldc % 4 == 0 && (g.aux == nullptr || g.ldaux % 4 == 0),
            "gemm_grouped: bad problem shape");
    require(((uintptr_t)g.A & 15) == 0 && ((uintptr_t)g.B & 15) == 0, "gemm_grouped: operands must be 16-B aligned");
  }
  if (hz::active()) {
    std::vector<hz::Rgn> v;
    for (int i = 0; i < n; ++i) gemm_hz_regions(ps[i], DType::BF16, out, ta, tb, v);
    hz::op(s, "gemm grouped (dW)", v.data(), v.size());
  }
  if (out == DType::F32) {
    if (ta && tb) launch_group<float, true, true>(ps, n, s);
    else if (!ta && tb) launch_group<float, false, true>(ps, n, s);
    else throw Error("gemm_grouped: layout not instantiated");
  } else {
    if (!ta && tb) launch_group<bf16, false, true>(ps, n, s);
    else if (!ta && !tb) launch_group<bf16, false, false>(ps, n, s);
    else throw Error("gemm_grouped: layout not instantiated");
  }
  CAPGEN_HIP(hipGetLastError());
}

int gemm_tune_load(const char* path) {
  FILE* f = std::fopen(path, "r");
  if (!f) return -1;
  std::lock_guard<std::mutex> lk(g_tune_mu);
  int n = 0;
  char line[1024];
  while (std::fgets(line, sizeof line, f)) {
    if (line[0] == 'g') {
      TuneLineG t;
      if (parse_tune_g(line + 1, NVARIANTS, &t)) {
        g_tuned.emplace(TuneKey{t.M, t.N, t.K, t.ta, t.tb, t.out}, Choice{t.variant, t.splitk});
        ++n;
      }
    } else if (line[0] == 'G') {
      std::vector<int> key;
      int var = 0;
      if (parse_tune_G(line + 1, kGroupVariants, (int)(sizeof kGroupVariants / sizeof kGroupVariants[0]), kMaxGroup,
                       &key, &var)) {
        g_group_tuned.emplace(key, var);
        ++n;
      }
    }
  }
  std::fclose(f);
  return n;
}

int gemm_tune_save(const char* path) {
  FILE* f = std::fopen(path, "w");
  if (!f) return -1;
  std::lock_guard<std::mutex> lk(g_tune_mu);
  std::fprintf(f, "# capgen bf16 GEMM autotune table (gfx950): g M N K ta tb out_bytes variant splitk | "
                  "G ta tb out_bytes n (M N K)xn variant\n");
  int n = 0;
  for (auto& kv : g_tuned) {
    const TuneKey& k = kv.first;
    std::fprintf(f, "g %d %d %d %d %d %d %d %d  # %s\n", k.M, k.N, k.K, k.ta, k.tb, k.out, kv.second.variant,
                 kv.second.splitk,
                 kv.second.variant >= 0 && kv.second.variant <= NVARIANTS ? kVariantName[kv.second.variant] : "?");
    ++n;
  }
  for (auto& kv : g_group_tuned) {
    const std::vector<int>& k = kv.first;
    std::fprintf(f, "G %d %d %d %d", k[0], k[1], k[2], (int)(k.size() - 3) / 3);
    for (size_t i = 3; i < k.size(); ++i) std::fprintf(f, " %d", k[i]);
    std::fprintf(f, " %d  # %s\n", kv.second,
                 kv.second >= 0 && kv.second <= NVARIANTS ? kVariantName[kv.second] : "?");
    ++n;
  }
  std::fclose(f);
  return n;
}

int gemm_tune_live_count() { return g_live_tuned; }

void gemm_set_variant(int v) { g_variant = v; }
void gemm_set_splitk_protocol(int p) {
  require(p == 0 || debug_build(), "split-K protocol bits are a debug-build diagnostic (libcapgen_debug.so)");
  g_splitk_proto = p;
}
void gemm_set_timing_buf(uint64_t* p) { g_timing_buf = p; }
void gemm_splitk_diag(int* out4, bool reset) {
  CAPGEN_HIP(hipDeviceSynchronize());
  CAPGEN_HIP(hipMemcpyFromSymbol(out4, HIP_SYMBOL(g_sk_diag), 4 * sizeof(int)));
  if (reset) {
// ... 62 lines not shown
```

image-caption_amd/csrc/gemm_tile.h:

```cpp
#pragma once
#include "gemm.h"

namespace capgen {

typedef __attribute__((ext_vector_type(8))) __bf16 bf16x8;
typedef __attribute__((ext_vector_type(4))) float f32x4;
typedef short s4 __attribute__((ext_vector_type(4)));
typedef __attribute__((address_space(3))) s4 lds_s4;
typedef __attribute__((address_space(3))) void lds_void;

namespace {

constexpr int BK = 64;


__device__ __forceinline__ int swz_k(int row, int chunk) { return chunk ^ (((row >> 1) ^ (row >> 4)) & 7); }
template <int ROWS>
__device__ __forceinline__ int swz_t(int k, int chunk) {
  if constexpr (ROWS == 128) return chunk ^ ((k & 7) << 1);
  else if constexpr (ROWS == 64) return chunk ^ (((k >> 1) & 3) << 1);
  else return chunk ^ (((k >> 2) & 1) << 1);
}

template <bool TRANS, int ROWS, int NW>
// ... 41 lines not shown
    }
  }

  __device__ __forceinline__ void dma(uint32_t v, uint32_t soff, char* lds) const {
    asm volatile("s_nop 4\n\tbuffer_load_dwordx4 %0, %1, %2 offen lds" ::"v"(v), "s"(rsrc), "s"(soff),
                 "{m0}"((unsigned)(uintptr_t)lds)
                 : "memory");
  }

  static __device__ __forceinline__ bf16x8 frag(const char* img, int rb, int ks, int lane) {
    const int g = lane >> 4;
    s4 lo, hi;
    if constexpr (!TRANS) {
      const int row = rb + (lane & 15);
      const int c1 = ks * 4 + (g >> 1), sub = (g & 1) * 8;
      lo = *reinterpret_cast<const s4*>(img + row * 128 + swz_k(row, c1) * 16 + sub);
      hi = *reinterpret_cast<const s4*>(img + row * 128 + swz_k(row, c1 + 2) * 16 + sub);
    } else {
      const int i = lane & 15, q = i >> 2, p = i & 3;
      const int k = ks * 32 + 4 * g + q;
      const int ch = (rb >> 3) + (p >> 1), sub = (p & 1) * 8;
      lo = __builtin_amdgcn_ds_read_tr16_b64_v4i16(
          (lds_s4*)(img + k * (ROWS * 2) + swz_t<ROWS>(k, ch) * 16 + sub));
      hi = __builtin_amdgcn_ds_read_tr16_b64_v4i16(
          (lds_s4*)(img + (k + 16) * (ROWS * 2) + swz_t<ROWS>(k + 16, ch) * 16 + sub));
    }
    return __builtin_bit_cast(bf16x8, __builtin_shufflevector(lo, hi, 0, 1, 2, 3, 4, 5, 6, 7));
  }
};

template <int N>
__device__ __forceinline__ void wait_vmcnt() {
  if constexpr (N == 0) asm volatile("s_waitcnt vmcnt(0)" ::: "memory");
  else asm volatile("s_waitcnt vmcnt(%0)" ::"n"(N) : "memory");
}

template <int LPT, int MAXY>
__device__ __forceinline__ void wait_younger(int younger) {
  if constexpr (MAXY == 0) {
    wait_vmcnt<0>();
  } else {
    if (younger >= MAXY) wait_vmcnt<MAXY * LPT>();
    else wait_younger<LPT, MAXY - 1>(younger);
  }
}

template <typename TO>
__device__ __forceinline__ void load4(const TO* p, float (&v)[4]) {
  if constexpr (sizeof(TO) == 4) {
    float4 x = *reinterpret_cast<const float4*>(p);
    v[0] = x.x, v[1] = x.y, v[2] = x.z, v[3] = x.w;
  } else {
    typedef __attribute__((ext_vector_type(4))) __bf16 b4;
    b4 x = *reinterpret_cast<const b4*>(p);
    v[0] = (float)x[0], v[1] = (float)x[1], v[2] = (float)x[2], v[3] = (float)x[3];
  }
}
template <typename TO>
__device__ __forceinline__ void store4(TO* p, const float (&v)[4]) {
  if constexpr (sizeof(TO) == 4) {
    *reinterpret_cast<float4*>(p) = float4{v[0], v[1], v[2], v[3]};
  } else {
    typedef __attribute__((ext_vector_type(4))) __bf16 b4;
    *reinterpret_cast<b4*>(p) = b4{(bf16)v[0], (bf16)v[1], (bf16)v[2], (bf16)v[3]};
  }
}

}

template <bool TA, bool TB, int BM, int BN, int WM, int WN, int STAGES, int KG = 1>
struct TileCfg {
  static constexpr int NW = WM * WN;
  static constexpr int NWT = NW * KG;
  typedef Op<TA, BM, NW> OA;
  typedef Op<TB, BN, NW> OB;
  static constexpr int SB = OA::BYTES + OB::BYTES;
  static constexpr int XCH = KG > 1 ? (BM / WM / 16) * (BN / WN / 16) * KG * NW * 64 * 16 : 0;
  static constexpr int SMEM = KG * STAGES * SB > XCH ? KG * STAGES * SB : XCH;
};

template <typename TO, int FM, int FN, int TM, int TN>
__device__ __forceinline__ void tile_epilogue(const GemmArgs& g, const f32x4 (&acc)[FM][FN], int m0, int n0, int wm,
                                              int wn, int lane, float alpha, int kgrp = 0, int kgs = 1);

#ifdef CAPGEN_GEMM_ABLATE
#define ABL_NO_MFMA (proto & 1024)
#define ABL_NO_DMA (proto & 2048)
#define ABL_DMA_FIRST (proto & 8192)
#define ABL_T(slot)                                                                                   \
  do {                                                                                                \
    if ((proto & 4096) && g.stamp && blockIdx.x == 0 && threadIdx.x == 0) {                           \
      g.stamp[16 + 2 * (slot)] = __builtin_amdgcn_s_memtime();                                        \
      g.stamp[17 + 2 * (slot)] = __builtin_amdgcn_s_memrealtime();                                    \
    }                                                                                                 \
  } while (0)
#else
#define ABL_NO_MFMA 0
#define ABL_NO_DMA 0
#define ABL_DMA_FIRST 0
#define ABL_T(slot) \
  do {              \
  } while (0)
#endif

static __device__ int g_sk_diag[4];

template <typename TO, bool TA, bool TB, int BM, int BN, int WM, int WN, int STAGES, int KG = 1>
__device__ __forceinline__ void gemm_tile(const GemmArgs& g, int mt, int nt, int tile, int split, int splitk,
                                          const void* zero, float* ws, int* tile_cnt, char* smem, int proto = 0) {
  typedef TileCfg<TA, TB, BM, BN, WM, WN, STAGES, KG> Cfg;
  constexpr int NW = Cfg::NW;
  typedef typename Cfg::OA OA;
  typedef typename Cfg::OB OB;
  constexpr int SB = Cfg::SB;
  constexpr int LPT = OA::PER_WAVE + OB::PER_WAVE;
  constexpr int TM = BM / WM, TN = BN / WN;
  constexpr int FM = TM / 16, FN = TN / 16;
  static_assert(STAGES >= 2, "need >= 2 stages");
  const int m0 = mt * BM, n0 = nt * BN;

  ABL_T(0);
  const bf16* __restrict__ A = reinterpret_cast<const bf16*>(g.A);
  const bf16* __restrict__ B = reinterpret_cast<const bf16*>(g.B);
  const int lane = threadIdx.x & 63;
  const int wave_all = __builtin_amdgcn_readfirstlane(threadIdx.x >> 6);
  const int kgrp = KG > 1 ? wave_all / NW : 0;
  const int wave = KG > 1 ? wave_all % NW : wave_all;
  const int wm = wave / WN, wn = wave % WN;

  f32x4 acc[FM][FN];
#pragma unroll
  for (int i = 0; i < FM; ++i)
#pragma unroll
    for (int j = 0; j < FN; ++j) acc[i][j] = f32x4{0.f, 0.f, 0.f, 0.f};

  const int nk_all = (g.K + BK - 1) / BK;
  const int per = (nk_all + splitk - 1) / splitk;
  const int nks = max(0, min(nk_all - split * per, per));
  const int per_g = (nks + KG - 1) / KG;
  const int kt0 = split * per + kgrp * per_g;
  const int nk = max(0, min(nks - kgrp * per_g, per_g));
  if (KG > 1) smem += kgrp * (STAGES * SB);
  OA oa;
  OB ob;
  oa.setup(A, g.lda, m0, g.M, g.K, kt0, wave, lane);
  ob.setup(B, g.ldb, n0, g.N, g.K, kt0, wave, lane);
  auto issue = [&](int t, char* st) {
    if (ABL_NO_DMA) return;
    const int kb = (kt0 + t) * BK;
    const bool tail = kb + BK > g.K;
    oa.issue(t, st, tail, kb, g.K, wave);
    ob.issue(t, st + OA::BYTES, tail, kb, g.K, wave);
  };
#pragma unroll
  for (int p = 0; p < STAGES - 1; ++p)
    if (p < nk) issue(p, smem + p * SB);
  ABL_T(1);

  static_assert((STAGES - 2) * LPT <= 63, "vmcnt range");
  for (int kb = 0; kb < per_g; kb += STAGES) {
#pragma unroll
    for (int s = 0; s < STAGES; ++s) {
      const int kt = kb + s;
      if (kt < per_g) {
        const bool work = KG == 1 || kt < nk;
        if (!ABL_NO_DMA && work) wait_younger<LPT, STAGES - 2>(nk - 1 - kt);
        if (kt < 8) ABL_T(2 + 4 * kt);
        __builtin_amdgcn_s_barrier();
        if (kt < 8) ABL_T(3 + 4 * kt);
        const char* st = smem + s * SB;
        if (NW * KG > 4 || ABL_DMA_FIRST) {
          if (kt + STAGES - 1 < nk) issue(kt + STAGES - 1, smem + ((s + STAGES - 1) % STAGES) * SB);
          if (kt < 8) ABL_T(4 + 4 * kt);
#pragma unroll
          for (int ks = 0; ks < BK / 32; ++ks) {
            if (!work) break;
            bf16x8 af[FM], bfr[FN];
#pragma unroll
            for (int i = 0; i < FM; ++i) af[i] = OA::frag(st, wm * TM + i * 16, ks, lane);
#pragma unroll
            for (int j = 0; j < FN; ++j) bfr[j] = OB::frag(st + OA::BYTES, wn * TN + j * 16, ks, lane);
            if (ABL_NO_MFMA) {
#pragma unroll
              for (int i = 0; i < FM; ++i)
#pragma unroll
                for (int j = 0; j < FN; ++j) acc[i][j][0] += (float)af[i][0] + (float)bfr[j][0];
              continue;
            }
#pragma unroll
            for (int i = 0; i < FM; ++i)
#pragma unroll
              for (int j = 0; j < FN; ++j)
                acc[i][j] = __builtin_amdgcn_mfma_f32_16x16x32_bf16(bfr[j], af[i], acc[i][j], 0, 0, 0);
          }
        } else {
          constexpr int KS = BK / 32;
          bf16x8 af[KS][FM], bfr[KS][FN];
          if (work) {
#pragma unroll
            for (int ks = 0; ks < KS; ++ks) {
#pragma unroll
              for (int i = 0; i < FM; ++i) af[ks][i] = OA::frag(st, wm * TM + i * 16, ks, lane);
#pragma unroll
              for (int j = 0; j < FN; ++j) bfr[ks][j] = OB::frag(st + OA::BYTES, wn * TN + j * 16, ks, lane);
            }
          }
          if (kt + STAGES - 1 < nk) issue(kt + STAGES - 1, smem + ((s + STAGES - 1) % STAGES) * SB);
          if (kt < 8) ABL_T(4 + 4 * kt);
          if (work) {
#pragma unroll
            for (int ks = 0; ks < KS; ++ks) {
              if (ABL_NO_MFMA) {
#pragma unroll
                for (int i = 0; i < FM; ++i)
#pragma unroll
                  for (int j = 0; j < FN; ++j) acc[i][j][0] += (float)af[ks][i][0] + (float)bfr[ks][j][0];
                continue;
              }
#pragma unroll
              for (int i = 0; i < FM; ++i)
#pragma unroll
                for (int j = 0; j < FN; ++j)
                  acc[i][j] = __builtin_amdgcn_mfma_f32_16x16x32_bf16(bfr[ks][j], af[ks][i], acc[i][j], 0, 0, 0);
            }
          }
        }
        if (kt < 8) ABL_T(5 + 4 * kt);
      }
    }
  }
  ABL_T(34);

  const float alpha = g.alpha_ptr ? g.alpha * *g.alpha_ptr : g.alpha;
  if constexpr (KG > 1) {
    if (KG > 1) smem -= kgrp * (STAGES * SB);
    f32x4* ex = reinterpret_cast<f32x4*>(smem);
    constexpr int NF = FM * FN;
    __syncthreads();
#pragma unroll
    for (int i = 0; i < FM; ++i)
#pragma unroll
      for (int j = 0; j < FN; ++j)
        if ((i * FN + j) % KG != kgrp) ex[(((i * FN + j) * KG + kgrp) * NW + wave) * 64 + lane] = acc[i][j];
    __syncthreads();
#pragma unroll
    for (int i = 0; i < FM; ++i)
#pragma unroll
      for (int j = 0; j < FN; ++j) {
        if ((i * FN + j) % KG != kgrp) continue;
        f32x4 sum = f32x4{0.f, 0.f, 0.f, 0.f};
#pragma unroll
        for (int h = 0; h < KG; ++h) sum += h == kgrp ? acc[i][j] : ex[(((i * FN + j) * KG + h) * NW + wave) * 64 + lane];
        acc[i][j] = sum;
      }
    tile_epilogue<TO, FM, FN, TM, TN>(g, acc, m0, n0, wm, wn, lane, alpha, kgrp, KG);
    ABL_T(35);
    return;
  }
  if (splitk > 1) {
    constexpr int NT = 64 * NW, NF = FM * FN;
    const int tid = threadIdx.x;
    const int64_t tile_bytes = (int64_t)splitk * NF * NT * 16;
    char* tbase = reinterpret_cast<char*>(ws) + (int64_t)tile * tile_bytes;
    const __amdgpu_buffer_rsrc_t rsrc = __builtin_amdgcn_make_buffer_rsrc(tbase, 0, (int)tile_bytes, 0x00020000);
    typedef __attribute__((ext_vector_type(4))) unsigned int u32x4;
#pragma unroll
    for (int i = 0; i < FM; ++i)
#pragma unroll
      for (int j = 0; j < FN; ++j)
        if (proto & 512)
          __builtin_amdgcn_raw_buffer_store_b128(__builtin_bit_cast(u32x4, acc[i][j]), rsrc,
                                                 ((split * NF + i * FN + j) * NT + tid) * 16, 0, 17);
        else
          __builtin_amdgcn_raw_buffer_store_b128(__builtin_bit_cast(u32x4, acc[i][j]), rsrc,
                                                 ((split * NF + i * FN + j) * NT + tid) * 16, 0, 16 );
    asm volatile("s_waitcnt vmcnt(0)" ::: "memory");
    __syncthreads();
    typedef __attribute__((address_space(3))) volatile int lds_int;
    lds_int* flag = (lds_int*)smem;
    if (tid == 0) {
      if (proto & 1) {
        __builtin_amdgcn_fence(__ATOMIC_RELEASE, "agent");
        asm volatile("s_waitcnt vmcnt(0)" ::: "memory");
      }
      const int old = __hip_atomic_fetch_add(tile_cnt + tile, 1, __ATOMIC_RELAXED, __HIP_MEMORY_SCOPE_AGENT);
      const int last = old == splitk - 1;
      if (proto & 64) {
        if (old < 0 || old >= splitk) atomicAdd(&g_sk_diag[0], 1);
        if (last) atomicAdd(&g_sk_diag[1], 1);
      }
      if (last) {
        if (proto & 16) __hip_atomic_store(tile_cnt + tile, 0, __ATOMIC_RELAXED, __HIP_MEMORY_SCOPE_AGENT);
        else (void)__hip_atomic_exchange(tile_cnt + tile, 0, __ATOMIC_RELAXED, __HIP_MEMORY_SCOPE_AGENT);
        if (proto & 128) {
          __builtin_amdgcn_fence(__ATOMIC_ACQUIRE, "");
          asm volatile("s_waitcnt vmcnt(0)" ::: "memory");
        } else if (!(proto & 2)) {
          __builtin_amdgcn_fence(__ATOMIC_ACQUIRE, "agent");
          asm volatile("s_waitcnt vmcnt(0)" ::: "memory");
        }
      }
      *flag = last;
    }
    __syncthreads();
    if (!*flag) return;
    __builtin_amdgcn_fence(__ATOMIC_ACQUIRE, "wavefront");
    const int lpol = (proto & 256) ? 17 : (proto & 4) ? 16  : 0;
    f32x4 sum[FM][FN];
#pragma unroll
    for (int i = 0; i < FM; ++i)
#pragma unroll
      for (int j = 0; j < FN; ++j) sum[i][j] = f32x4{0.f, 0.f, 0.f, 0.f};
    for (int sl = 0; sl < splitk; ++sl) {
      if (sl == split) {
#pragma unroll
        for (int i = 0; i < FM; ++i)
#pragma unroll
          for (int j = 0; j < FN; ++j) sum[i][j] += acc[i][j];
        continue;
      }
      u32x4 o[FM][FN];
#pragma unroll
      for (int i = 0; i < FM; ++i)
#pragma unroll
        for (int j = 0; j < FN; ++j) {
          const int off = ((sl * NF + i * FN + j) * NT + tid) * 16;
          o[i][j] = lpol == 17 ? __builtin_amdgcn_raw_buffer_load_b128(rsrc, off, 0, 17)
                    : lpol     ? __builtin_amdgcn_raw_buffer_load_b128(rsrc, off, 0, 16)
                               : __builtin_amdgcn_raw_buffer_load_b128(rsrc, off, 0, 0);
        }
#pragma unroll
      for (int i = 0; i < FM; ++i)
#pragma unroll
        for (int j = 0; j < FN; ++j) sum[i][j] += __builtin_bit_cast(f32x4, o[i][j]);
    }
#pragma unroll
    for (int i = 0; i < FM; ++i)
#pragma unroll
      for (int j = 0; j < FN; ++j) acc[i][j] = sum[i][j];
  }
  tile_epilogue<TO, FM, FN, TM, TN>(g, acc, m0, n0, wm, wn, lane, alpha);
  ABL_T(35);
}

template <typename TO, int FM, int FN, int TM, int TN>
__device__ __forceinline__ void tile_epilogue(const GemmArgs& g, const f32x4 (&acc)[FM][FN], int m0, int n0, int wm,
                                              int wn, int lane, float alpha, int kgrp, int kgs) {
  TO* __restrict__ C = reinterpret_cast<TO*>(g.C);
  TO* __restrict__ C2 = reinterpret_cast<TO*>(g.C2);
  const bf16* __restrict__ aux = reinterpret_cast<const bf16*>(g.aux);
  const int fr = lane & 15, fq = lane >> 4;
  if constexpr (sizeof(TO) == 2) {
    if (g.ce_stats) {
      float4 bq[FN];
      int tgq[FM];
#pragma unroll
      for (int j = 0; j < FN; ++j) {
        const int n = min(n0 + wn * TN + j * 16 + fq * 4, g.N - 4);
        bq[j] = g.bias ? *reinterpret_cast<const float4*>(g.bias + n) : float4{0.f, 0.f, 0.f, 0.f};
      }
#pragma unroll
      for (int i = 0; i < FM; ++i) tgq[i] = g.ce_tgt[min(m0 + wm * TM + i * 16 + fr, g.M - 1)];
#pragma unroll
      for (int i = 0; i < FM; ++i) {
        const int m = m0 + wm * TM + i * 16 + fr;
        const bool mok = m < g.M;
        const int tg = mok ? tgq[i] : -1;
#pragma unroll
        for (int j = 0; j < FN; ++j) {
          if ((i * FN + j) % kgs != kgrp) continue;
          const int nb = n0 + wn * TN + j * 16, n = nb + fq * 4;
          const bool nok = n < g.N;
          float v[4], mx = -INFINITY;
          if (nok) {
            const float4 b4 = bq[j];
            v[0] = alpha * acc[i][j][0] + b4.x, v[1] = alpha * acc[i][j][1] + b4.y;
            v[2] = alpha * acc[i][j][2] + b4.z, v[3] = alpha * acc[i][j][3] + b4.w;
            mx = fmaxf(fmaxf(v[0], v[1]), fmaxf(v[2], v[3]));
          }
          mx = fmaxf(mx, __shfl_xor(mx, 16, 64));
          mx = fmaxf(mx, __shfl_xor(mx, 32, 64));
          float e[4], sum = 0.f;
#pragma unroll
          for (int r = 0; r < 4; ++r) {
            e[r] = nok ? __expf(v[r] - mx) : 0.f;
            sum += e[r];
          }
          sum += __shfl_xor(sum, 16, 64);
          sum += __shfl_xor(sum, 32, 64);
          if (mok && nok) {
            store4<TO>(C + (int64_t)m * g.ldc + n, e);
            if (tg >= n && tg < n + 4) g.ce_tlogit[m] = v[tg - n];
          }
          if (mok && fq == 0 && nb < g.N) g.ce_stats[(int64_t)m * g.ce_ld + nb / 16] = float2{mx, sum};
        }
      }
      return;
    }
  }
  if constexpr (sizeof(TO) == 4) {
    if (g.dec_stats) {
      float4 bq[FN];
#pragma unroll
      for (int j = 0; j < FN; ++j) {
        const int n = min(n0 + wn * TN + j * 16 + fq * 4, g.N - 4);
        bq[j] = g.bias ? *reinterpret_cast<const float4*>(g.bias + n) : float4{0.f, 0.f, 0.f, 0.f};
      }
#pragma unroll
      for (int i = 0; i < FM; ++i) {
        const int m = m0 + wm * TM + i * 16 + fr;
        const bool mok = m < g.M;
#pragma unroll
        for (int j = 0; j < FN; ++j) {
          if ((i * FN + j) % kgs != kgrp) continue;
          const int nb = n0 + wn * TN + j * 16, n = nb + fq * 4;
          const bool nok = n < g.N;
          float v[4], mx = -INFINITY;
          if (nok) {
            const float4 b4 = bq[j];
            v[0] = alpha * acc[i][j][0] + b4.x, v[1] = alpha * acc[i][j][1] + b4.y;
            v[2] = alpha * acc[i][j][2] + b4.z, v[3] = alpha * acc[i][j][3] + b4.w;
            mx = fmaxf(fmaxf(v[0], v[1]), fmaxf(v[2], v[3]));
          }
// ... 107 lines not shown
```

image-caption_amd/csrc/knobs.cpp:

```cpp
#include <atomic>
#include <cstdlib>
#include <cstring>
#include <mutex>
#include <string>

#include "capgen_host.h"

namespace capgen {
namespace {

struct KnobDef {
  Knob k;
  const char* name;
  int dflt;
  bool debug_only;
};

constexpr KnobDef kDefs[] = {
    {Knob::FusedCe, "FUSED_CE", 1, false},
    {Knob::GroupDw, "GROUP_DW", 1, false},
    {Knob::FusedQkv, "FUSED_QKV", 1, false},
    {Knob::FusedAttnBwd, "FUSED_ATTN_BWD", 1, false},
    {Knob::ColsumSide, "COLSUM_SIDE", 1, false},
    {Knob::DecodeCrossMfma, "DECODE_CROSS_MFMA", 1, false},
    {Knob::SlabDecode, "SLAB_DECODE", 1, false},
    {Knob::DecodeGroupLds, "DECODE_GROUP_LDS", 1, false},
    {Knob::AttnWave, "ATTN_WAVE", 1, false},
    {Knob::CeVec8, "CE_VEC8", 1, false},
    {Knob::BregDecode, "BREG_DECODE", 1, false},
    {Knob::DecodeLnFold, "DECODE_LN_FOLD", 1, false},
    {Knob::FusedBeamStep, "FUSED_BEAM_STEP", 1, false},
    {Knob::OverlapFront, "OVERLAP_FRONT", 1, false},
    {Knob::OverlapDec0, "OVERLAP_DEC0", 1, false},
    {Knob::StripeClear, "STRIPE_CLEAR", 1, false},
    {Knob::BucketBlocks, "BUCKET_BLOCKS", 1, false},
    {Knob::Zero, "ZERO", 1, false},
    {Knob::FwdGraph, "FWD_GRAPH", 1, false},
    {Knob::Streams, "STREAMS", 3, false},
    {Knob::EventFence, "EVENT_FENCE", 1, false},
    {Knob::DeferLoss, "DEFER_LOSS", 1, false},
    {Knob::FrontJoin, "FRONT_JOIN", 99, false},
    {Knob::ClipAdamGrid, "CLIP_ADAM_GRID", 2048, false},
    {Knob::Autotune, "AUTOTUNE", 1, false},
    {Knob::AutotuneLog, "AUTOTUNE_LOG", 0, false},
    {Knob::Skip, "SKIP", 0, true},
    {Knob::DebugDropJoin, "DEBUG_DROP_JOIN", 0, true},
    {Knob::SplitkProto, "SPLITK_PROTO", 0, true},
    {Knob::AllowPartialLines, "ALLOW_PARTIAL_LINES", 0, true},
    {Knob::DwVariant, "DW_VARIANT", 0, true},
    {Knob::HostTiming, "HOST_TIMING", 0, true},
};
static_assert(sizeof(kDefs) / sizeof(kDefs[0]) == (size_t)Knob::Count, "one definition per knob");

#ifdef CAPGEN_DEBUG
constexpr bool kDebugBuild = true;
#else
constexpr bool kDebugBuild = false;
#endif

std::atomic<int> g_val[(int)Knob::Count];
std::once_flag g_once;

void init() {
  for (const KnobDef& d : kDefs) {
    int v = d.dflt;
    if (!d.debug_only || kDebugBuild) {
      const std::string env = std::string("CAPGEN_") + d.name;
      if (const char* e = std::getenv(env.c_str())) v = std::atoi(e);
    }
    g_val[(int)d.k].store(v, std::memory_order_relaxed);
  }
}

}

int knob(Knob k) {
  std::call_once(g_once, init);
  return g_val[(int)k].load(std::memory_order_relaxed);
}

int knob_set(const char* name, int value, int* old) {
  std::call_once(g_once, init);
  for (const KnobDef& d : kDefs)
    if (std::strcmp(d.name, name) == 0) {
      if (d.debug_only && !kDebugBuild) return -2;
      const int prev = g_val[(int)d.k].exchange(value, std::memory_order_relaxed);
      if (old) *old = prev;
      return 0;
    }
  return -1;
}

bool debug_build() { return kDebugBuild; }

}
```

image-caption_amd/csrc/qkv_attn.hip:

```cpp
#include <cstdlib>

#include "qkv_attn.h"

#include "attn_mfma_dev.h"
#include "hazard.h"

namespace capgen {
using namespace amf;

namespace {

constexpr int QD = 512;
constexpr int QKS = QD / 32;
constexpr int QKB = 4;

__device__ __forceinline__ int xswz(int row, int chunk) { return chunk ^ (row & 15); }
__device__ int32_t g_qa_dummy[64];

template <int LT>
__device__ __forceinline__ void dma_rows(const bf16* rows, int64_t ld, int L, char* xs, int w, int lane) {
  const __amdgpu_buffer_rsrc_t rs =
      __builtin_amdgcn_make_buffer_rsrc(const_cast<bf16*>(rows), 0, (int)((int64_t)L * ld * 2), 0x00020000);
#pragma unroll
  for (int j = 0; j < 4 * LT; ++j) {
    const int row = w + 4 * j;
    const uint32_t voff = row < L ? (uint32_t)(((int64_t)row * ld + (lane ^ (row & 15)) * 8) * 2) : 0x80000000u;
    asm volatile("s_nop 4\n\tbuffer_load_dwordx4 %0, %1, %2 offen lds" ::"v"(voff), "s"(rs), "s"(0u),
                 "{m0}"((unsigned)(uintptr_t)(xs + row * (QD * 2)))
                 : "memory");
  }
}

__device__ __forceinline__ void bf8_to_f(const uint4& u, float (&f)[8]) {
  const uint32_t w[4] = {u.x, u.y, u.z, u.w};
#pragma unroll
  for (int e = 0; e < 4; ++e) {
    f[2 * e] = __uint_as_float(w[e] << 16);
    f[2 * e + 1] = __uint_as_float(w[e] & 0xffff0000u);
  }
}

template <int LT, int NP>
__global__ void __launch_bounds__(256) qkv_attn_kernel(QkvAttn a) {
  __shared__ __attribute__((aligned(16))) char sm[kFwdSmem];
  __shared__ __attribute__((aligned(16))) char xs[LT * 16 * QD * 2];
  StampScope stamp_scope(a.g.stamp);
  if (a.g.prio) __builtin_amdgcn_s_setprio(3);
  const AttnGeom& g = a.g;
  const int b = blockIdx.x / g.H, h = blockIdx.x % g.H;
  const int tid = threadIdx.x, lane = tid & 63;
  const int w = __builtin_amdgcn_readfirstlane(tid >> 6);
  constexpr int NF = NP;
  const int L = g.Lq;
  const bf16* xb = a.X + (int64_t)b * L * a.ldx;

  const int fr = lane & 15, fg = lane >> 4;
  const bf16* wrow[NF];
#pragma unroll
  for (int f = 0; f < NF; ++f) {
    const int c = 16 * NF * w + 16 * f, which = c >> 6, within = c & 63;
    wrow[f] = a.W + ((int64_t)((which * QD + h * DK + within) >> 4) * QKS * 64 + lane) * 8;
  }
  bf16x8 bq[2][QKB][NF];
#pragma unroll
  for (int kk = 0; kk < QKB; ++kk)
#pragma unroll
    for (int f = 0; f < NF; ++f) bq[0][kk][f] = *reinterpret_cast<const bf16x8*>(wrow[f] + 512 * kk);
  {
    dma_rows<LT>(xb, a.ldx, L, xs, w, lane);
    uint4 kv[2][2];
    if constexpr (NP == 1) {
      const int bk = g.kv_bmod ? b % g.kv_bmod : b;
      const bf16* src[2] = {reinterpret_cast<const bf16*>(g.k) + (int64_t)bk * g.k_bs + h * DK,
                            reinterpret_cast<const bf16*>(g.v) + (int64_t)bk * g.v_bs + h * DK};
      const int64_t ld[2] = {g.k_ld, g.v_ld};
#pragma unroll
      for (int i = 0; i < 2; ++i)
#pragma unroll
        for (int u = 0; u < 2; ++u) {
          const int c = tid + 256 * u, row = c >> 3, ch = c & 7;
          kv[i][u] = row < g.Lk
                         ? *reinterpret_cast<const uint4*>(src[i] + (int64_t)min(row, g.Lk - 1) * ld[i] + ch * 8)
                         : uint4{0u, 0u, 0u, 0u};
        }
    }
    int kid = 0, kvl = 1;
    if (w == 0) {
      const int j = min(lane, g.Lk - 1);
      const int bk = g.kv_bmod ? b % g.kv_bmod : b;
      kid = opaque(g.key_ids ? g.key_ids : g_qa_dummy)[g.key_ids ? (int64_t)b * g.kid_bs + j : lane];
      kvl = opaque(g.key_valid ? g.key_valid : reinterpret_cast<const uint8_t*>(g_qa_dummy))[
          g.key_valid ? (int64_t)bk * g.kv_bs + j : lane];
    }
#pragma unroll
    for (int u = 0; u < NP * IMG / 16 / 256; ++u)
      reinterpret_cast<uint4*>(sm)[tid + 256 * u] = uint4{0u, 0u, 0u, 0u};
    if constexpr (NP == 1) {
#pragma unroll
      for (int i = 0; i < 2; ++i)
#pragma unroll
        for (int u = 0; u < 2; ++u) {
          const int c = tid + 256 * u, row = c >> 3, ch = c & 7;
          *reinterpret_cast<uint4*>(sm + (1 + i) * IMG + row * 128 + swz(row, ch) * 16) =
              row < g.Lk ? kv[i][u] : uint4{0u, 0u, 0u, 0u};
        }
    }
    if (w == 0)
      reinterpret_cast<unsigned char*>(sm + 3 * IMG)[lane] =
          lane < g.Lk && (!g.key_valid || kvl != 0) && (!g.key_ids || kid != g.pad_idx);
  }
  f32x4 acc[LT][NF];
#pragma unroll
  for (int i = 0; i < LT; ++i)
#pragma unroll
    for (int f = 0; f < NF; ++f) acc[i][f] = f32x4{0.f, 0.f, 0.f, 0.f};
  asm volatile("s_waitcnt vmcnt(0)" ::: "memory");
  __syncthreads();
#pragma unroll
  for (int grp = 0; grp < QKS / QKB; ++grp) {
    const int cur = grp & 1;
    if (grp + 1 < QKS / QKB) {
#pragma unroll
      for (int kk = 0; kk < QKB; ++kk)
#pragma unroll
        for (int f = 0; f < NF; ++f)
          bq[cur ^ 1][kk][f] = *reinterpret_cast<const bf16x8*>(wrow[f] + 512 * ((grp + 1) * QKB + kk));
    }
    __builtin_amdgcn_sched_barrier(0);
#pragma unroll
    for (int kk = 0; kk < QKB; ++kk) {
      const int ks = grp * QKB + kk;
#pragma unroll
      for (int i = 0; i < LT; ++i) {
        const int row = 16 * i + fr;
        const bf16x8 af = *reinterpret_cast<const bf16x8*>(xs + row * (QD * 2) + xswz(row, 4 * ks + fg) * 16);
#pragma unroll
        for (int f = 0; f < NF; ++f) acc[i][f] = __builtin_amdgcn_mfma_f32_16x16x32_bf16(bq[cur][kk][f], af, acc[i][f], 0, 0, 0);
      }
    }
  }

  bf16* qkvb = a.qkv ? a.qkv + (int64_t)b * L * a.ldqkv : nullptr;
#pragma unroll
  for (int f = 0; f < NF; ++f) {
    const int c = 16 * NF * w + 16 * f + 4 * fg, which = c >> 6, within = c & 63;
    char* img = sm + which * IMG;
#pragma unroll
    for (int i = 0; i < LT; ++i) {
      const int row = 16 * i + fr;
      const f32x4 v = acc[i][f];
      const bf16x4 r4 = {(bf16)v[0], (bf16)v[1], (bf16)v[2], (bf16)v[3]};
      if (row < L) {
        if (a.qkv) *reinterpret_cast<bf16x4*>(qkvb + (int64_t)row * a.ldqkv + which * QD + h * DK + within) = r4;
        *reinterpret_cast<bf16x4*>(img + row * 128 + swz(row, within >> 3) * 16 + (within & 7) * 2) = r4;
      }
    }
  }
  __syncthreads();
  attn_fwd_staged(g, a.o, nullptr, b, h, sm);
}

template <int LT>
__global__ void __launch_bounds__(256) qkv_attn_bwd_kernel(QkvBwd a) {
  constexpr int XS = LT * 16 * QD * 2;
  constexpr int RA = XS > 5 * IMG ? XS : 5 * IMG;
  __shared__ __attribute__((aligned(16))) char sm[RA + IMG + 64];
  char* xs = sm;
  char* Kimg = sm;
  char* Qimg = sm + IMG;
  char* Vimg = sm + 2 * IMG;
  char* Pdimg = sm + 3 * IMG;
  char* dSimg = sm + 4 * IMG;
  char* dOimg = sm + RA;
  unsigned char* kok = reinterpret_cast<unsigned char*>(sm + RA + IMG);
  const AttnGeom& g = a.g;
  StampScope stamp_scope(g.stamp);
  if (g.prio) __builtin_amdgcn_s_setprio(3);
  const int b = blockIdx.x / g.H, h = blockIdx.x % g.H;
  const int tid = threadIdx.x, lane = tid & 63;
  const int w = __builtin_amdgcn_readfirstlane(tid >> 6);
  const int fr = lane & 15, fg = lane >> 4;
  const int L = g.Lq;
  const bf16* wrow = a.Wt + ((int64_t)((h * DK + 16 * w) >> 4) * QKS * 64 + lane) * 8;
  bf16x8 bq[QKS];
#pragma unroll
  for (int ks = 0; ks < QKS; ++ks) bq[ks] = *reinterpret_cast<const bf16x8*>(wrow + 512 * ks);
  dma_rows<LT>(a.dA + (int64_t)b * L * a.ldda, a.ldda, L, xs, w, lane);
  const int bk = g.kv_bmod ? b % g.kv_bmod : b;
  const bf16* src[3] = {reinterpret_cast<const bf16*>(g.k) + (int64_t)bk * g.k_bs + h * DK,
                        reinterpret_cast<const bf16*>(g.q) + (int64_t)b * g.q_bs + h * DK,
                        reinterpret_cast<const bf16*>(g.v) + (int64_t)bk * g.v_bs + h * DK};
  const int64_t ld[3] = {g.k_ld, g.q_ld, g.v_ld};
  const int Ls[3] = {g.Lk, g.Lq, g.Lk};
  uint4 kqv[3][2];
#pragma unroll
  for (int i = 0; i < 3; ++i)
#pragma unroll
    for (int u = 0; u < 2; ++u) {
      const int c = tid + 256 * u, row = c >> 3, ch = c & 7;
      kqv[i][u] = row < Ls[i]
                      ? *reinterpret_cast<const uint4*>(src[i] + (int64_t)min(row, Ls[i] - 1) * ld[i] + ch * 8)
                      : uint4{0u, 0u, 0u, 0u};
    }
  int kid = 0, kvl = 1;
  if (w == 0) {
    const int j = min(lane, g.Lk - 1);
    kid = opaque(g.key_ids ? g.key_ids : g_qa_dummy)[g.key_ids ? (int64_t)b * g.kid_bs + j : lane];
    kvl = opaque(g.key_valid ? g.key_valid : reinterpret_cast<const uint8_t*>(g_qa_dummy))[
        g.key_valid ? (int64_t)bk * g.kv_bs + j : lane];
  }
#pragma unroll
  for (int u = 0; u < 2; ++u) reinterpret_cast<uint4*>(dOimg)[tid + 256 * u] = uint4{0u, 0u, 0u, 0u};
  asm volatile("s_waitcnt vmcnt(0)" ::: "memory");
  __syncthreads();
  f32x4 acc[LT];
#pragma unroll
  for (int i = 0; i < LT; ++i) acc[i] = f32x4{0.f, 0.f, 0.f, 0.f};
#pragma unroll
  for (int ks = 0; ks < QKS; ++ks)
#pragma unroll
    for (int i = 0; i < LT; ++i) {
      const int row = 16 * i + fr;
      const bf16x8 af = *reinterpret_cast<const bf16x8*>(xs + row * (QD * 2) + xswz(row, 4 * ks + fg) * 16);
      acc[i] = __builtin_amdgcn_mfma_f32_16x16x32_bf16(bq[ks], af, acc[i], 0, 0, 0);
    }
#pragma unroll
  for (int i = 0; i < LT; ++i) {
    const int row = 16 * i + fr, col = 16 * w + 4 * fg;
    const bf16x4 r4 = {(bf16)acc[i][0], (bf16)acc[i][1], (bf16)acc[i][2], (bf16)acc[i][3]};
    *reinterpret_cast<bf16x4*>(dOimg + row * 128 + swz(row, col >> 3) * 16 + (col & 7) * 2) = r4;
  }
  __syncthreads();
  {
    char* const img[3] = {Kimg, Qimg, Vimg};
#pragma unroll
    for (int i = 0; i < 3; ++i)
#pragma unroll
      for (int u = 0; u < 2; ++u) {
        const int c = tid + 256 * u, row = c >> 3, ch = c & 7;
        *reinterpret_cast<uint4*>(img[i] + row * 128 + swz(row, ch) * 16) = row < Ls[i] ? kqv[i][u] : uint4{0u, 0u, 0u, 0u};
      }
    if (w == 0) kok[lane] = lane < g.Lk && (!g.key_valid || kvl != 0) && (!g.key_ids || kid != g.pad_idx);
  }
  __syncthreads();
  attn_bwd_staged(g, a.dq, a.dk, a.dv, b, h, Kimg, dOimg, Qimg, Vimg, Pdimg, dSimg, kok);
}

__global__ void __launch_bounds__(256) tile_weights_t_kernel(const bf16* __restrict__ src, int64_t ld,
                                                             bf16* __restrict__ dst) {
  __shared__ bf16 t[32][64 + 8];
  const int tid = threadIdx.x, k0 = blockIdx.y * 32, n0 = blockIdx.x * 64;
  {
    const int row = tid >> 3, ch = tid & 7;
    const bf16x8 v = *reinterpret_cast<const bf16x8*>(src + (int64_t)(k0 + row) * ld + n0 + ch * 8);
#pragma unroll
    for (int e = 0; e < 8; ++e) t[row][ch * 8 + e] = v[e];
  }
  __syncthreads();
  const int jj = tid >> 6, lane = tid & 63;
  const int nl = 16 * jj + (lane & 15), kk = 8 * (lane >> 4);
  bf16x8 o;
#pragma unroll
  for (int e = 0; e < 8; ++e) o[e] = t[kk + e][nl];
  const int64_t piece = (int64_t)(n0 / 16 + jj) * QKS + k0 / 32;
  reinterpret_cast<bf16x8*>(dst)[piece * 64 + lane] = o;
}
__global__ void tile_weights_kernel(const bf16* __restrict__ src, int64_t n, int64_t ld, bf16* __restrict__ dst) {
  const int64_t i = (int64_t)blockIdx.x * 256 + threadIdx.x;
  if (i >= n) return;
  const int lane = (int)(i & 63), ks = (int)((i >> 6) % QKS);
  const int64_t j = (i >> 6) / QKS;
  const uint4 v = *reinterpret_cast<const uint4*>(src + (16 * j + (lane & 15)) * ld + 32 * ks + 8 * (lane >> 4));
  reinterpret_cast<uint4*>(dst)[i] = v;
}

}

void qkv_tile_weights(const bf16* src, int R, int64_t ld, bf16* dst, hipStream_t s) {
  require(R > 0 && R % 16 == 0 && ld % 8 == 0 && ld >= QD, "qkv_tile_weights: R % 16 == 0, ld >= 512");
  if (hz::active()) {
    using namespace hz;
    hz::op(s, "qkv_tile_weights", {blk(src, R, QD * 2, ld * 2, RD), wr(dst, (int64_t)R * QD * 2)});
  }
  const int64_t n = (int64_t)R * QD / 8;
  tile_weights_kernel<<<(unsigned)((n + 255) / 256), 256, 0, s>>>(src, n, ld, dst);
  CAPGEN_HIP(hipGetLastError());
}

bool qkv_attn_ok(const QkvAttn& a) {
  const AttnGeom& g = a.g;
  const bool shape = a.cross ? (g.Lk >= 1 && g.Lk <= 64 && g.k_ld % 8 == 0 && g.v_ld % 8 == 0 && g.k_bs % 8 == 0 &&
                                g.v_bs % 8 == 0)
                             : (g.Lq == g.Lk && g.kv_bmod == 0);
  return shape && g.dk == DK && g.H * DK == QD && a.d == QD && g.Lq >= 1 && g.Lq <= 64 && !g.kv_row && a.W &&
         a.ldx % 8 == 0 && a.ldqkv % 8 == 0 && g.o_ld % 8 == 0 && g.o_bs % 8 == 0;
}

void qkv_attn_fwd(const QkvAttn& a_in, hipStream_t s) {
  QkvAttn a = a_in;
  require(qkv_attn_ok(a), "qkv_attn_fwd: unsupported geometry (head size 64, d = 512, self attention, L <= 64)");
  const AttnGeom& g = a.g;
  if (hz::active()) {
    using namespace hz;
    const int L = g.Lq;
    const int np = a.cross ? 1 : 3, Bk = g.kv_bmod > 0 ? std::min(g.B, g.kv_bmod) : g.B;
    const Rgn r[] = {rows_blk(a.X, g.B, L, (int64_t)L * a.ldx, a.ldx, a.d, 2, RD),
                     rd(a.W, (int64_t)np * QD * QD * 2),
                     blk(g.key_valid, Bk, g.Lk, g.kv_bs, RD), blk(g.key_ids, g.B, (int64_t)g.Lk * 4, g.kid_bs * 4, RD),
                     rows_blk(a.cross ? g.k : nullptr, Bk, g.Lk, g.k_bs, g.k_ld, a.d, 2, RD),
                     rows_blk(a.cross ? g.v : nullptr, Bk, g.Lk, g.v_bs, g.v_ld, a.d, 2, RD),
                     rd(g.drop.seed_ptr, 8), rows_blk(a.qkv, g.B, L, (int64_t)L * a.ldqkv, a.ldqkv, np * a.d, 2, WR),
                     rows_blk(a.o, g.B, L, g.o_bs, g.o_ld, a.d, 2, WR)};
    op(s, "qkv_attn", r, sizeof r / sizeof r[0]);
  }
  const int lt = (a.g.Lq + 15) / 16;
  const dim3 grid(a.g.B * a.g.H);
  if (a.cross) {
    switch (lt) {
      case 1: qkv_attn_kernel<1, 1><<<grid, 256, 0, s>>>(a); break;
      case 2: qkv_attn_kernel<2, 1><<<grid, 256, 0, s>>>(a); break;
      case 3: qkv_attn_kernel<3, 1><<<grid, 256, 0, s>>>(a); break;
      default: qkv_attn_kernel<4, 1><<<grid, 256, 0, s>>>(a); break;
    }
  } else {
    switch (lt) {
      case 1: qkv_attn_kernel<1, 3><<<grid, 256, 0, s>>>(a); break;
      case 2: qkv_attn_kernel<2, 3><<<grid, 256, 0, s>>>(a); break;
      case 3: qkv_attn_kernel<3, 3><<<grid, 256, 0, s>>>(a); break;
// ... 54 lines not shown
```

include/capgen.h:

```cpp
#ifndef CAPGEN_H
#define CAPGEN_H

#include <stddef.h>
#include <stdint.h>

#ifdef __cplusplus
extern "C" {
#endif

#define CAPGEN_ABI_VERSION 13

typedef struct capgen_engine capgen_t;

enum capgen_dtype { CAPGEN_F32 = 0, CAPGEN_BF16 = 1 };

typedef struct capgen_config {
  int32_t num_vocab, max_length;
  int32_t dim_features, dim_positions;
  int32_t enc_d, enc_ff, enc_blocks, enc_heads;
  int32_t dim_word_embedding;
  int32_t dec_d, dec_ff, dec_blocks, dec_heads;
  float dropout;
  float attention_dropout;
  int32_t pad_idx;
  int32_t encode_mask;
  int32_t focal_loss;
  int32_t split_position;
  int32_t split_image_objects;
  int32_t move_first_image_feature;
  int32_t dtype;
  int32_t max_batch, max_regions;
  float lr, beta1, beta2, eps;
  uint64_t seed;
} capgen_config;

typedef struct capgen_param_info {
  char name[96];
  int32_t ndim;
  int64_t rows, cols;
  int64_t offset, row_stride;
} capgen_param_info;

const char* capgen_last_error(void);
int capgen_abi_version(void);
int capgen_set_knob(const char* name, int value, int* old);
int capgen_debug_build(void);

int capgen_param_table(const capgen_config* cfg, capgen_param_info* out, int cap, int* count,
                       int64_t* arena_elems);

int capgen_create(const capgen_config* cfg, int device, capgen_t** out);
int capgen_destroy(capgen_t* h);

int capgen_get_params(capgen_t* h, float* host_dst, int64_t n);
int capgen_set_params(capgen_t* h, const float* host_src, int64_t n);
int capgen_get_grads(capgen_t* h, float* host_dst, int64_t n);
int capgen_set_grads(capgen_t* h, const float* host_src, int64_t n);
int capgen_get_adam_state(capgen_t* h, int64_t* step, float* exp_avg, float* exp_avg_sq, int64_t n);
int capgen_set_adam_state(capgen_t* h, int64_t step, const float* exp_avg, const float* exp_avg_sq, int64_t n);
int capgen_arenas(capgen_t* h, float** params, float** grads, int64_t* n);

int capgen_set_training(capgen_t* h, int training);

int capgen_forward(capgen_t* h, const void* feats, int feats_dtype, const float* pos, const int32_t* caps,
                   int B, int N, int T, float* loss_out, void* stream);
int capgen_backward(capgen_t* h, void* stream);
int capgen_adam_step(capgen_t* h, void* stream);
int capgen_train_step(capgen_t* h, const void* feats, int feats_dtype, const float* pos, const int32_t* caps,
                      int B, int N, int T, float* loss_out, void* stream);
int capgen_set_graph(capgen_t* h, int enable);
int capgen_set_lr(capgen_t* h, float lr);
int capgen_get_lr(capgen_t* h, float* lr);
int capgen_set_grad_clip(capgen_t* h, float max_norm);
int capgen_last_grad_norm(capgen_t* h, float* host_out);
int capgen_compute_loss(capgen_t* h, const void* feats, int feats_dtype, const float* pos, const int32_t* caps,
                        int B, int N, int T, float* loss_out, void* stream);
int capgen_copy_logits(capgen_t* h, float* dst, int64_t n, void* stream);

int capgen_greedy(capgen_t* h, const void* feats, int feats_dtype, const float* pos, int B, int N,
                  int64_t* ids_out, float* attn_out, void* stream);
int capgen_beam(capgen_t* h, const void* feats, int feats_dtype, const float* pos, int B, int N, int beam_size,
                int64_t* ids_out, void* stream);

int capgen_sample(capgen_t* h, const void* feats, int feats_dtype, const float* pos, int B, int N, int n_samples,
                  float temperature, int top_k, uint64_t seed, int64_t* ids_out, float* logp_out, void* stream);
int capgen_sample_nucleus(capgen_t* h, const void* feats, int feats_dtype, const float* pos, int B, int N,
                          int n_samples, float temperature, int top_k, float top_p, uint64_t seed, int64_t* ids_out,
                          float* logp_out, void* stream);

int capgen_set_decode_log_softmax(capgen_t* h, int enable);

int capgen_set_rng_seed(capgen_t* h, uint64_t seed);
int capgen_debug_gemm(int M, int N, int K, const void* A, int64_t lda, int ta, const void* B, int64_t ldb, int tb,
                      void* C, int64_t ldc, int in_dtype, int out_dtype, const float* bias, float alpha, int beta,
                      int relu, void* stream);

int capgen_debug_gemm_tiled(int M, int N, int K, const void* A, int64_t lda, const void* B, int64_t ldb, int tb,
                            void* Bt, void* C, int64_t ldc, int out_dtype, const float* bias, int beta, int relu,
                            const void* aux, int64_t ldaux, void* stream);

int capgen_debug_gemm_tiled_ln(int M, int N, const void* A, const void* ln_res, const void* B, void* Bt, void* C,
                               int out_dtype, const float* bias, int beta, int relu, const float* ln_gamma,
                               const float* ln_beta, void* ln_y, const int32_t* ln_ids, int64_t ln_ids_ld, int ln_pad,
                               void* stream);

int capgen_debug_gemm_variant(int variant);
int capgen_debug_splitk_protocol(int proto);
int capgen_debug_splitk_diag(int* out4, int reset);
int capgen_debug_gemm_timing_buf(void* dev_buf);
int capgen_debug_copy_buffer(capgen_t* h, int which, void* host_dst, int64_t bytes);

int capgen_train_step_indexed(capgen_t* h, const void* feat_store, int feats_dtype, const float* pos_store,
                              int n_images, const int32_t* img_idx, const int32_t* caps, int B, int N, int T,
                              float* loss_out, void* stream);

int capgen_train_step_weighted(capgen_t* h, const void* feats, int feats_dtype, const float* pos, int n_images,
                               const int32_t* img_idx, const int32_t* caps, const float* weights, int B, int N,
                               int T, float* loss_out, int train, void* stream);

int capgen_rl_sample(capgen_t* h, const void* feats, int feats_dtype, const float* pos, const int32_t* caps, int B,
                     int N, int T, int64_t* sample_out, float* entropy_out, float* lm_loss_out, void* stream);
int capgen_rl_finish(capgen_t* h, const float* scores, float structure_loss_weight, float* loss_out, int train,
                     void* stream);

int capgen_scst_rewards(const int64_t* target, int64_t target_ld, const int64_t* sample, int64_t sample_ld, int B,
                        int L, int start_id, int end_id, int null_id, int64_t dot_id, double cider_w, double bleu_w,
                        double* out);

int capgen_debug_attention(int dtype, int B, int H, int Lq, int Lk, int dk, const void* q, const void* k,
                           const void* v, const unsigned char* key_valid, int causal, float temperature, void* o,
                           float* probs, const void* dout, void* dq, void* dk_, void* dv, void* stream);

int capgen_debug_qkv_attention(int B, int L, int H, const void* X, const void* W, void* qkv, void* o,
                               const unsigned char* key_valid, const int32_t* key_ids, int pad_idx, int causal,
                               void* stream);

int capgen_debug_cross_attention(int B, int Lq, int Lk, int H, const void* X, const void* Wq, const void* KV, void* q,
                                 void* o, const unsigned char* key_valid, void* stream);

int capgen_debug_attention_bwd_wo(int B, int Lq, int Lk, int H, const void* q, const void* k, const void* v,
                                  const unsigned char* key_valid, int causal, const void* dA, const void* Wo, void* dq,
                                  void* dk, void* dv, void* stream);

int capgen_debug_layernorm_fwd(int dtype, int M, int d, const void* a, const float* a_bias, float drop_p,
                               int drop_site, uint64_t drop_seed, const void* res, const float* pe, int pe_L,
                               const float* gamma, const float* beta, const int32_t* ids, int64_t ids_ld, int pad_idx,
                               const unsigned char* valid, void* y, void* v_save, float* mean, float* rstd,
                               void* stream);
int capgen_debug_layernorm_bwd(int dtype, int M, int d, const void* dy, const void* v, const float* mean,
                               const float* rstd, const float* gamma, const int32_t* ids, int64_t ids_ld, int pad_idx,
                               const unsigned char* valid, float drop_p, int drop_site, uint64_t drop_seed,
                               void* d_res, void* d_a, float* dgamma, float* dbeta, float* dbias, int stripes,
                               int64_t stripe_stride, void* stream);
int capgen_debug_column_sum(int dtype, const void* X, int M, int N, int64_t ldx, float alpha, const float* alpha_ptr,
                            float* db, int stripes, int64_t stripe_stride, void* stream);
int capgen_debug_stripe_reduce(float* S, int stripes, int64_t stride, int64_t n, float* dst, int accumulate, int clear,
                               void* stream);
int capgen_debug_embedding_gather(const float* table, const int32_t* ids, int64_t ids_ld, int M, int d, void* out,
                                  int dtype, void* stream);
int capgen_debug_embedding_scatter_add(const void* dE, const int32_t* ids, int M, int d, int pad, float* grad,
                                       int dtype, void* stream);
int capgen_debug_pack_encoder_input(const void* feats, int feats_dtype, const float* pos, int M, int F, int P, int Kp,
                                    void* out, int out_dtype, unsigned char* valid, const int32_t* img_idx, int N,
                                    int n_img, uint64_t* seed_bump, void* stream);
int capgen_debug_prepare_captions(const int32_t* caps, int B, int T, int pad, int32_t* ids_in, int32_t* tgt,
                                  float* count, uint64_t* seed_bump, float* inv_count, void* stream);
int capgen_debug_cross_entropy_rows(const float* logits, const int32_t* tgt, int M, int V, int pad, float* loss_row,
                                    void* dlogits, int dtype, void* stream);
int capgen_debug_ce_finish(const void* stats, int64_t ld, const float* tlogit, const int32_t* tgt, int M, int V,
                           int pad, float* loss_row, void* dl, void* stream);
int capgen_debug_cross_entropy_rows_weighted(const float* logits, const int32_t* tgt, const float* row_w,
                                             int rows_per_w, int M, int V, int pad, float* loss_row, void* dlogits,
                                             int dtype, void* stream);
int capgen_debug_ce_finish_weighted(const void* stats, int64_t ld, const float* tlogit, const int32_t* tgt,
                                    const float* row_w, int rows_per_w, int M, int V, int pad, float* loss_row,
                                    void* dl, void* stream);
int capgen_debug_loss_finalize(const float* loss_row, int M, const float* count, int focal, float* loss_out,
                               float* grad_scale, const float* ce_in, int partial, void* stream);
int capgen_debug_adam(float* p, const float* g, float* m, float* v, int64_t n, float lr, float b1, float b2,
                      float eps, int64_t* step, float* scal, void* shadow, int64_t n_shadow, int grid_cap,
                      int n_tiles, const int64_t* tile_off, const int64_t* tile_len, void* const* tile_dst,
                      void* stream);
int capgen_debug_adam_scaled(float* p, const float* g, float* m, float* v, int64_t n, float lr, float b1, float b2,
                             float eps, int64_t* step, float* scal, void* shadow, int64_t n_shadow, int grid_cap,
                             int n_tiles, const int64_t* tile_off, const int64_t* tile_len, void* const* tile_dst,
                             const float* gscale, void* stream);
int capgen_debug_grad_norm(const float* g, int64_t n, float max_norm, int grid_cap, double* partials, int cap,
                           float* out2, void* stream);
int capgen_debug_to_bf16(const float* src, void* dst, int64_t n, void* stream);
int capgen_debug_arena_checksum(const float* p, int64_t n, uint64_t* out, void* stream);
int capgen_debug_argmax_softmax(const float* logits, int B, int V, int64_t* ids_out, int64_t ids_ld, int col,
                                int32_t* next_ids, int64_t next_ld, int logsm, void* stream);
int capgen_debug_sample_softmax(const float* logits, int R, int V, float inv_tau, int top_k, uint64_t seed,
// ... 54 lines not shown
```

Baseline: 23830 images/s.

## Fold FFN bias-gradient column sum into the W1 dW GEMM via MFMA ones-vector

Adds an a_colsum epilogue to the grouped bf16 TN GEMM: tiles with nt==0 also multiply the A fragments by a ones vector on MFMA and atomically add the per-row sums into the striped bias-gradient buffer. This replaces the separate column-sum job for the FFN b1 gradient when the side-stream colsum path is active, behind a new knob that is on by default. It also hoists the dropout seed load in the fused QKV attention kernels to the kernel start. The trade-off is extra MFMA work and atomics on the first N-tile column, and forcing those dW GEMMs through the grouped path.

```diff
diff --git a/image-caption_amd/capgen/_lib.py b/image-caption_amd/capgen/_lib.py
--- a/image-caption_amd/capgen/_lib.py
+++ b/image-caption_amd/capgen/_lib.py
@@ -73,6 +73,8 @@
     "capgen_set_rng_seed": (C.c_int, [_P, C.c_uint64]),
     "capgen_debug_gemm": (C.c_int, [C.c_int, C.c_int, C.c_int, _P, C.c_int64, C.c_int, _P, C.c_int64, C.c_int,
                                     _P, C.c_int64, C.c_int, C.c_int, _P, C.c_float, C.c_int, C.c_int, _P]),
+    "capgen_debug_gemm_dw": (C.c_int, [C.c_int, C.POINTER(C.c_int32), C.POINTER(_P), C.POINTER(C.c_int64), C.c_int,
+                                       C.c_int64, C.c_int, _P]),
     "capgen_debug_gemm_tiled": (C.c_int, [C.c_int, C.c_int, C.c_int, _P, C.c_int64, _P, C.c_int64, C.c_int, _P, _P,
                                           C.c_int64, C.c_int, _P, C.c_int, C.c_int, _P, C.c_int64, _P]),
     "capgen_debug_gemm_tiled_ln": (C.c_int, [C.c_int, C.c_int, _P, _P, _P, _P, _P, C.c_int, _P, C.c_int, C.c_int, _P, _P,
@@ -82,6 +84,7 @@
     "capgen_debug_splitk_diag": (C.c_int, [_P, C.c_int]),
     "capgen_debug_gemm_timing_buf": (C.c_int, [_P]),
     "capgen_debug_copy_buffer": (C.c_int, [_P, C.c_int, _P, C.c_int64]),
+    "capgen_debug_tiled_bytes": (C.c_int64, [_P]),
     "capgen_train_step_indexed": (C.c_int, [_P, _P, C.c_int, _P, C.c_int, _P, _P, C.c_int, C.c_int, C.c_int, _P,
                                             _P]),
     "capgen_train_step_weighted": (C.c_int, [_P, _P, C.c_int, _P, C.c_int, _P, _P, _P, C.c_int, C.c_int, C.c_int, _P,
@@ -176,6 +179,8 @@
                           "`python -c 'import __graft_entry__ as g; g.build()'` (make -C image-caption_amd/csrc)")
     lib = C.CDLL(LIB_PATH)
     for name, (res, args) in _SIGS.items():
+        if name.startswith("capgen_debug_") and os.environ.get("CAPGEN_LIB_PATH") and not hasattr(lib, name):
+            continue
         fn = getattr(lib, name)
         fn.restype = res
         fn.argtypes = args
diff --git a/image-caption_amd/csrc/attn_mfma_dev.h b/image-caption_amd/csrc/attn_mfma_dev.h
--- a/image-caption_amd/csrc/attn_mfma_dev.h
+++ b/image-caption_amd/csrc/attn_mfma_dev.h
@@ -117,7 +117,7 @@
 
 __device__ __forceinline__ void attn_fwd_images(const AttnGeom& g, bf16* __restrict__ o, float* __restrict__ probs,
                                                 int b, int h, const char* Qimg, const char* Kimg, const char* Vimg,
-                                                const unsigned char* kok) {
+                                                const unsigned char* kok, const uint64_t* seed_early = nullptr) {
   const int tid = threadIdx.x, lane = tid & 63, w = tid >> 6;
   const int q0 = 16 * w, q = q0 + (lane & 15);
   if (q0 >= g.Lq) return;
@@ -135,7 +135,7 @@
       }
   }
   if (g.drop.seed_ptr) {
-    const uint64_t seed = *g.drop.seed_ptr;
+    const uint64_t seed = seed_early ? *seed_early : *g.drop.seed_ptr;
 #pragma unroll
     for (int j = 0; j < 4; ++j)
 #pragma unroll
@@ -157,8 +157,9 @@
 }
 
 __device__ __forceinline__ void attn_fwd_staged(const AttnGeom& g, bf16* __restrict__ o, float* __restrict__ probs,
-                                                int b, int h, const char* sm) {
-  attn_fwd_images(g, o, probs, b, h, sm, sm + IMG, sm + 2 * IMG, reinterpret_cast<const unsigned char*>(sm + 3 * IMG));
+                                                int b, int h, const char* sm, const uint64_t* seed_early = nullptr) {
+  attn_fwd_images(g, o, probs, b, h, sm, sm + IMG, sm + 2 * IMG, reinterpret_cast<const unsigned char*>(sm + 3 * IMG),
+                  seed_early);
 }
 
 __device__ __forceinline__ void attn_fwd_one(const AttnGeom& g, bf16* __restrict__ o, float* __restrict__ probs, int b,
@@ -186,7 +187,8 @@
 __device__ __forceinline__ void attn_bwd_staged(const AttnGeom& g, bf16* __restrict__ dq, bf16* __restrict__ dkp,
                                                 bf16* __restrict__ dvp, int b, int h, const char* Kimg,
                                                 const char* dOimg, const char* Qimg, const char* Vimg, char* Pdimg,
-                                                char* dSimg, const unsigned char* kok) {
+                                                char* dSimg, const unsigned char* kok,
+                                                const uint64_t* seed_early = nullptr) {
   const int tid = threadIdx.x, lane = tid & 63, w = tid >> 6;
   const int64_t qoff = (int64_t)b * g.q_bs + h * DK, koff = (int64_t)b * g.k_bs + h * DK,
                 voff = (int64_t)b * g.v_bs + h * DK;
@@ -199,7 +201,7 @@
     softmax_rows(g, kok, q, lane, s, p);
     scores(dOimg, q0, Vimg, lane, dp);
     const int64_t row_idx = (((int64_t)b * g.H + h) * g.Lq + q) * g.Lk;
-    const uint64_t seed = g.drop.seed_ptr ? *g.drop.seed_ptr : 0;
+    const uint64_t seed = !g.drop.seed_ptr ? 0 : seed_early ? *seed_early : *g.drop.seed_ptr;
     float rs = 0.f;
 #pragma unroll
     for (int j = 0; j < 4; ++j)
diff --git a/image-caption_amd/csrc/capgen_host.h b/image-caption_amd/csrc/capgen_host.h
--- a/image-caption_amd/csrc/capgen_host.h
+++ b/image-caption_amd/csrc/capgen_host.h
@@ -14,7 +14,7 @@
 }
 
 enum class Knob : int {
-  FusedCe, GroupDw, FusedQkv, FusedAttnBwd, ColsumSide, DecodeCrossMfma, SlabDecode, DecodeGroupLds, AttnWave,
+  FusedCe, GroupDw, FusedQkv, FusedAttnBwd, ColsumSide, DwColsum, DecodeCrossMfma, SlabDecode, DecodeGroupLds, AttnWave,
   CeVec8, BregDecode, DecodeLnFold, FusedBeamStep, OverlapFront, OverlapDec0, StripeClear, BucketBlocks, Zero, FwdGraph, Streams,
   EventFence, DeferLoss, FrontJoin, ClipAdamGrid, Autotune, AutotuneLog,
   Skip, DebugDropJoin, SplitkProto, AllowPartialLines, DwVariant, HostTiming,
diff --git a/image-caption_amd/csrc/engine.hip b/image-caption_amd/csrc/engine.hip
--- a/image-caption_amd/csrc/engine.hip
+++ b/image-caption_amd/csrc/engine.hip
@@ -576,10 +576,12 @@
     gemm(ga, act, act, false, true, s);
   }
   void linear_dw(const void* dY, int64_t ldy, const void* X, int64_t ldx, int64_t goff, int64_t ldg, int M, int N,
-                 int K, const float* alpha_ptr, hipStream_t s) {
+                 int K, const float* alpha_ptr, hipStream_t s, float* a_colsum = nullptr) {
     GemmArgs ga;
     ga.M = N, ga.N = K, ga.K = M, ga.A = dY, ga.lda = ldy, ga.B = X, ga.ldb = ldx, ga.C = G(goff), ga.ldc = ldg;
     ga.alpha_ptr = alpha_ptr;
+    ga.a_colsum = a_colsum;
+    if (a_colsum) ga.colsum_stripes = NSTRIPE, ga.colsum_stride = n_small;
     ga.prio = prio(s);
     if (stamp_on) ga.stamp = stamp(s, "gemm dW " + dims(N, K, M));
     gemm(ga, act, DType::F32, true, true, s);
@@ -945,21 +947,24 @@
     int64_t ldy, ldx, goff, ldg;
     int M, N, K;
     const float* alpha_ptr;
+    float* a_colsum;
   };
   std::vector<DwJob> dw_pending;
   bool group_dw = knob(Knob::GroupDw) != 0;
   void dw_side(const void* dY, int64_t ldy, const void* X, int64_t ldx, int64_t goff, int64_t ldg, int M, int N,
-               int K, const float* alpha_ptr, hipStream_t s) {
+               int K, const float* alpha_ptr, hipStream_t s, float* a_colsum = nullptr) {
     if (es2 == s) {
-      linear_dw(dY, ldy, X, ldx, goff, ldg, M, N, K, alpha_ptr, s);
+      linear_dw(dY, ldy, X, ldx, goff, ldg, M, N, K, alpha_ptr, s, a_colsum);
       return;
     }
-    dw_pending.push_back(DwJob{dY, X, ldy, ldx, goff, ldg, M, N, K, alpha_ptr});
+    dw_pending.push_back(DwJob{dY, X, ldy, ldx, goff, ldg, M, N, K, alpha_ptr, a_colsum});
   }
   GemmArgs dw_args(const DwJob& j) const {
     GemmArgs ga;
     ga.M = j.N, ga.N = j.K, ga.K = j.M, ga.A = j.dY, ga.lda = j.ldy, ga.B = j.X, ga.ldb = j.ldx;
     ga.C = G(j.goff), ga.ldc = j.ldg, ga.alpha_ptr = j.alpha_ptr;
+    ga.a_colsum = j.a_colsum;
+    if (j.a_colsum) ga.colsum_stripes = NSTRIPE, ga.colsum_stride = n_small;
     return ga;
   }
   void dw_launch(const DwJob* jobs, size_t n, hipStream_t st) {
@@ -973,7 +978,7 @@
     } else {
       for (size_t i = 0; i < n; ++i) {
         const DwJob& j = jobs[i];
-        linear_dw(j.dY, j.ldy, j.X, j.ldx, j.goff, j.ldg, j.M, j.N, j.K, j.alpha_ptr, st);
+        linear_dw(j.dY, j.ldy, j.X, j.ldx, j.goff, j.ldg, j.M, j.N, j.K, j.alpha_ptr, st, j.a_colsum);
       }
     }
   }
@@ -984,6 +989,7 @@
   };
   std::vector<ColJob> col_pending;
   bool colsum_side = knob(Knob::ColsumSide) != 0;
+  bool dw_colsum = knob(Knob::DwColsum) != 0;
   void flush(hipStream_t s) {
     fork(s);
     dw_launch(dw_pending.data(), dw_pending.size(), es2);
@@ -1008,8 +1014,9 @@
     dw_side(gA, d, H, f, W2, f, M, d, f, nullptr, s);
     const bool side = colsum_side && es2 != s;
     linear_dx(gA, d, W2, f, gH, f, M, d, f, 0, H, nullptr, s, side ? nullptr : GS(b1));
-    if (side) col_pending.push_back(ColJob{gH, M, f, GS(b1)});
-    dw_side(gH, f, X, d, W1, d, M, f, d, nullptr, s);
+    const bool fold = side && dw_colsum && act == DType::BF16;
+    if (side && !fold) col_pending.push_back(ColJob{gH, M, f, GS(b1)});
+    dw_side(gH, f, X, d, W1, d, M, f, d, nullptr, s, fold ? GS(b1) : nullptr);
     linear_dx(gH, f, W1, d, lb.d_res, d, M, f, d, 1, nullptr, nullptr, s);
   }
   void mha_out_bwd(int M, int d, const LnBwd& lb, const void* att, int64_t Wo, void* gATT, hipStream_t s) {
@@ -1249,7 +1256,7 @@
       flush(s);
       lnb(lb, es2);
       linear_dx(a.gAd, dd, L.Wel, L.dwe, a.gE, L.dwe, Md, dd, L.dwe, 0, nullptr, nullptr, es2);
-      const DwJob wel{a.gAd, a.E, dd, L.dwe, L.Wel, L.dwe, Md, dd, L.dwe, nullptr};
+      const DwJob wel{a.gAd, a.E, dd, L.dwe, L.Wel, L.dwe, Md, dd, L.dwe, nullptr, nullptr};
       dw_launch(&wel, 1, es2);
       embedding_scatter_add(a.gE, a.ids, Md, L.dwe, cfg.pad_idx, G(L.emb), act, es2, L.V);
       stripe_reduce(GS(L.dec_lng), NSTRIPE, n_small, L.total - L.dec_lng, G(L.dec_lng), 0, es2, stripe_clear);
@@ -2226,6 +2233,29 @@
   });
 }
 
+int capgen_debug_gemm_dw(int n, const int32_t* mnk, void* const* ptrs, const int64_t* lds, int stripes,
+                         int64_t stripe_stride, int single, void* stream) {
+  return guarded([&] {
+    gemm_init();
+    require(n >= 1 && n <= kMaxGroup && mnk && ptrs && lds, "debug_gemm_dw: 1..kMaxGroup problems");
+    GemmArgs ga[kMaxGroup];
+    for (int i = 0; i < n; ++i) {
+      GemmArgs& g = ga[i];
+      g.M = mnk[3 * i], g.N = mnk[3 * i + 1], g.K = mnk[3 * i + 2];
+      g.A = ptrs[4 * i], g.B = ptrs[4 * i + 1], g.C = ptrs[4 * i + 2];
+      g.a_colsum = reinterpret_cast<float*>(ptrs[4 * i + 3]);
+      g.lda = lds[3 * i], g.ldb = lds[3 * i + 1], g.ldc = lds[3 * i + 2];
+      g.colsum_stripes = stripes, g.colsum_stride = stripe_stride;
+    }
+    const hipStream_t s = (hipStream_t)stream;
+    if (single) {
+      for (int i = 0; i < n; ++i) gemm(ga[i], DType::BF16, DType::F32, true, true, s);
+    } else {
+      gemm_grouped(ga, n, DType::F32, true, true, s);
+    }
+  });
+}
+
 int capgen_debug_gemm_tiled(int M, int N, int K, const void* A, int64_t lda, const void* B, int64_t ldb, int tb,
                             void* Bt, void* Cp, int64_t ldc, int out_dtype, const float* bias, int beta, int relu,
                             const void* aux, int64_t ldaux, void* stream) {
@@ -2731,6 +2761,7 @@
     void* src = which == 0 ? h->a.tmp : which == 1 ? h->a.gOut : which == 2 ? h->a.gRes : which == 3 ? h->a.gKV
               : which == 4 ? h->a.genc[Le - 1].gH : which == 5 ? h->a.genc[Le - 1].gAf
               : which == 6 ? h->a.genc[Le - 1].gA1 : which == 7 ? h->a.genc[Le - 1].gQKV
+              : which == 8 ? (void*)h->wtile
               : which >= 32 && (which - 32) / 8 < Le && (which - 32) % 8 < 5
                   ? (&h->a.genc[(which - 32) / 8].gAf)[(which - 32) % 8 == 0 ? 0 : (which - 32) % 8 == 1 ? 1
                                                         : (which - 32) % 8 == 2 ? 2 : (which - 32) % 8 == 3 ? 3 : 4]
@@ -2748,10 +2779,17 @@
               : which >= 216 && which - 216 < h->L.Ld ? h->a.dec[which - 216].H
                   : nullptr;
     require(src != nullptr,
-            "debug_copy_buffer: which in 0..7, 32 + 8 l + 0..4, 80 + 0..Le, 128 + 8 l + 0..7, 200 + l, 216 + l");
+            "debug_copy_buffer: which in 0..8, 32 + 8 l + 0..4, 80 + 0..Le, 128 + 8 l + 0..7, 200 + l, 216 + l");
     hz::host_sync(nullptr);
     CAPGEN_HIP(hipMemcpy(host_dst, src, (size_t)bytes, hipMemcpyDeviceToHost));
   });
+}
+
+int64_t capgen_debug_tiled_bytes(capgen_t* h) {
+  int64_t n = 0;
+  if (h)
+    for (auto& kv : h->tiled) n += (int64_t)std::abs(kv.second.second) * 512 * 2;
+  return n;
 }
 
 int capgen_debug_gemm_timing_buf(void* dev_buf) {
diff --git a/image-caption_amd/csrc/gemm.h b/image-caption_amd/csrc/gemm.h
--- a/image-caption_amd/csrc/gemm.h
+++ b/image-caption_amd/csrc/gemm.h
@@ -26,7 +26,7 @@
   int beta = 0;
   int prio = 0;
   const void* bt = nullptr;
-  int64_t bt_pad_ = 0;
+  float* a_colsum = nullptr;
   void* C2 = nullptr;
   int64_t ldc2 = 0;
   int nsplit = 0;
diff --git a/image-caption_amd/csrc/gemm.hip b/image-caption_amd/csrc/gemm.hip
--- a/image-caption_amd/csrc/gemm.hip
+++ b/image-caption_amd/csrc/gemm.hip
@@ -240,6 +240,7 @@
   v.push_back(rd(g.bias, g.N * 4));
   v.push_back(rd(g.alpha_ptr, 4));
   v.push_back(blk(g.colsum, g.colsum_stripes, g.N * 4, g.colsum_stride * 4, ACC));
+  v.push_back(blk(g.a_colsum, g.colsum_stripes, g.M * 4, g.colsum_stride * 4, ACC));
   v.push_back(blk(g.ce_stats, g.M, (int64_t)((g.N + 15) / 16) * 8, g.ce_ld * 8, WR));
   v.push_back(blk(g.dec_stats, g.M, (int64_t)((g.N + 15) / 16) * 8, g.dec_ld * 8, WR));
   v.push_back(rd(g.ce_tgt, (int64_t)g.M * 4));
@@ -274,6 +275,11 @@
   require(((uintptr_t)g.A & 15) == 0 && ((uintptr_t)g.B & 15) == 0, "gemm: operands must be 16-B aligned");
   require(g.K > 0, "gemm: K must be positive");
   require(!g.colsum || !g.beta, "gemm: colsum requires beta == 0");
+  if (g.a_colsum) {
+    require(in == DType::BF16 && out == DType::F32 && ta && tb, "gemm: a_colsum needs a bf16 TN launch with f32 output");
+    gemm_grouped(&g, 1, DType::F32, true, true, s);
+    return;
+  }
   require(!g.bt || (in == DType::BF16 && !ta), "gemm: a tiled B (bt) needs the bf16 path with A stored [M][K]");
   require(!g.dec_stats || in == DType::BF16, "gemm: dec_stats is a bf16-path epilogue output");
   require(!g.a_ids || (in == DType::BF16 && !ta && !tb && g.bt && gemm_breg_ok(g) && g.a_table_rows > 0),
diff --git a/image-caption_amd/csrc/gemm_bf16.hip b/image-caption_amd/csrc/gemm_bf16.hip
--- a/image-caption_amd/csrc/gemm_bf16.hip
+++ b/image-caption_amd/csrc/gemm_bf16.hip
@@ -43,6 +43,9 @@
   gemm_tile<TO, TA, TB, BM, BN, WM, WN, STAGES, KG>(g, mt, nt, tile, split, splitk, zero, ws, tile_cnt, smem, proto);
 }
 
+template <typename TO, bool TA, bool TB>
+constexpr bool kGroupAcs = TA && TB && sizeof(TO) == 4;
+
 template <typename TO, bool TA, bool TB, int BM, int BN, int WM, int WN, int STAGES>
 __global__ void __launch_bounds__(64 * WM * WN) gemm_bf16_grouped_kernel(GemmGroup gg, int nblk, int G,
                                                                         const void* zero) {
@@ -55,7 +58,8 @@
     while (q + 1 < gg.n && slot >= gg.start[q + 1]) ++q;
     const int tile = slot - gg.start[q];
     const int mt = tile / gg.tiles_n[q], nt = tile % gg.tiles_n[q];
-    gemm_tile<TO, TA, TB, BM, BN, WM, WN, STAGES>(gg.p[q], mt, nt, tile, 0, 1, zero, nullptr, nullptr, smem);
+    gemm_tile<TO, TA, TB, BM, BN, WM, WN, STAGES, 1, kGroupAcs<TO, TA, TB>>(gg.p[q], mt, nt, tile, 0, 1, zero, nullptr,
+                                                                           nullptr, smem);
   }
 }
 
@@ -72,7 +76,8 @@
     while (q + 1 < gg.n && slot >= gg.start[q + 1]) ++q;
     const int tile = slot - gg.start[q];
     const int mt = tile / gg.tiles_n[q], nt = tile % gg.tiles_n[q];
-    gemm_tile<TO, TA, TB, BM, BN, WM, WN, STAGES>(gg.p[q], mt, nt, tile, 0, 1, zero, nullptr, nullptr, smem);
+    gemm_tile<TO, TA, TB, BM, BN, WM, WN, STAGES, 1, kGroupAcs<TO, TA, TB>>(gg.p[q], mt, nt, tile, 0, 1, zero, nullptr,
+                                                                           nullptr, smem);
   }
 }
 
@@ -447,7 +452,7 @@
         std::vector<void*> scratch(n);
         for (int i = 0; i < n; ++i) {
           CAPGEN_HIP(hipMalloc(&scratch[i], (size_t)t[i].M * t[i].ldc * sizeof(TO)));
-          t[i].C = scratch[i], t[i].beta = 0, t[i].colsum = nullptr, t[i].stamp = nullptr;
+          t[i].C = scratch[i], t[i].beta = 0, t[i].colsum = nullptr, t[i].a_colsum = nullptr, t[i].stamp = nullptr;
         }
         hipEvent_t e0, e1;
         CAPGEN_HIP(hipEventCreate(&e0));
@@ -496,6 +501,8 @@
     require(g.M > 0 && g.N > 0 && g.K > 0 && g.N % 4 == 0 && g.ldc % 4 == 0 && (g.aux == nullptr || g.ldaux % 4 == 0),
             "gemm_grouped: bad problem shape");
     require(((uintptr_t)g.A & 15) == 0 && ((uintptr_t)g.B & 15) == 0, "gemm_grouped: operands must be 16-B aligned");
+    require(!g.a_colsum || (ta && tb && out == DType::F32 && g.colsum_stripes >= 1),
+            "gemm_grouped: a_colsum needs the TN layout with f32 output");
   }
   if (hz::active()) {
     std::vector<hz::Rgn> v;
diff --git a/image-caption_amd/csrc/gemm_tile.h b/image-caption_amd/csrc/gemm_tile.h
--- a/image-caption_amd/csrc/gemm_tile.h
+++ b/image-caption_amd/csrc/gemm_tile.h
@@ -147,6 +147,14 @@
 template <typename TO, int FM, int FN, int TM, int TN>
 __device__ __forceinline__ void tile_epilogue(const GemmArgs& g, const f32x4 (&acc)[FM][FN], int m0, int n0, int wm,
                                               int wn, int lane, float alpha, int kgrp = 0, int kgs = 1);
+
+template <int FM>
+struct AcsState {
+  bool on;
+  f32x4 cs[FM];
+  bf16x8 ones;
+};
+struct AcsNone {};
 
 #ifdef CAPGEN_GEMM_ABLATE
 #define ABL_NO_MFMA (proto & 1024)
@@ -170,7 +178,7 @@
 
 static __device__ int g_sk_diag[4];
 
-template <typename TO, bool TA, bool TB, int BM, int BN, int WM, int WN, int STAGES, int KG = 1>
+template <typename TO, bool TA, bool TB, int BM, int BN, int WM, int WN, int STAGES, int KG = 1, bool ACS = false>
 __device__ __forceinline__ void gemm_tile(const GemmArgs& g, int mt, int nt, int tile, int split, int splitk,
                                           const void* zero, float* ws, int* tile_cnt, char* smem, int proto = 0) {
   typedef TileCfg<TA, TB, BM, BN, WM, WN, STAGES, KG> Cfg;
@@ -198,6 +206,15 @@
   for (int i = 0; i < FM; ++i)
 #pragma unroll
     for (int j = 0; j < FN; ++j) acc[i][j] = f32x4{0.f, 0.f, 0.f, 0.f};
+  static_assert(!ACS || (TA && KG == 1 && sizeof(TO) == 4), "a_colsum: TN f32 tiles without k-groups");
+  std::conditional_t<ACS, AcsState<FM>, AcsNone> acs;
+  if constexpr (ACS) {
+    acs.on = g.a_colsum != nullptr && nt == 0 && wn == 0;
+#pragma unroll
+    for (int i = 0; i < FM; ++i) acs.cs[i] = f32x4{0.f, 0.f, 0.f, 0.f};
+#pragma unroll
+    for (int e = 0; e < 8; ++e) acs.ones[e] = (__bf16)1.0f;
+  }
 
   const int nk_all = (g.K + BK - 1) / BK;
   const int per = (nk_all + splitk - 1) / splitk;
@@ -257,6 +274,13 @@
 #pragma unroll
               for (int j = 0; j < FN; ++j)
                 acc[i][j] = __builtin_amdgcn_mfma_f32_16x16x32_bf16(bfr[j], af[i], acc[i][j], 0, 0, 0);
+            if constexpr (ACS) {
+              if (acs.on) {
+#pragma unroll
+                for (int i = 0; i < FM; ++i)
+                  acs.cs[i] = __builtin_amdgcn_mfma_f32_16x16x32_bf16(acs.ones, af[i], acs.cs[i], 0, 0, 0);
+              }
+            }
           }
         } else {
           constexpr int KS = BK / 32;
@@ -287,6 +311,13 @@
 #pragma unroll
                 for (int j = 0; j < FN; ++j)
                   acc[i][j] = __builtin_amdgcn_mfma_f32_16x16x32_bf16(bfr[ks][j], af[ks][i], acc[i][j], 0, 0, 0);
+              if constexpr (ACS) {
+                if (acs.on) {
+#pragma unroll
+                  for (int i = 0; i < FM; ++i)
+                    acs.cs[i] = __builtin_amdgcn_mfma_f32_16x16x32_bf16(acs.ones, af[ks][i], acs.cs[i], 0, 0, 0);
+                }
+              }
             }
           }
         }
@@ -404,6 +435,16 @@
 #pragma unroll
       for (int j = 0; j < FN; ++j) acc[i][j] = sum[i][j];
   }
+  if constexpr (ACS) {
+    if (acs.on && lane < 16) {
+      float* dst = g.a_colsum + (int64_t)(mt % g.colsum_stripes) * g.colsum_stride;
+#pragma unroll
+      for (int i = 0; i < FM; ++i) {
+        const int m = m0 + wm * TM + i * 16 + lane;
+        if (m < g.M) atomicAdd(dst + m, alpha * acs.cs[i][0]);
+      }
+    }
+  }
   tile_epilogue<TO, FM, FN, TM, TN>(g, acc, m0, n0, wm, wn, lane, alpha);
   ABL_T(35);
 }
diff --git a/image-caption_amd/csrc/knobs.cpp b/image-caption_amd/csrc/knobs.cpp
--- a/image-caption_amd/csrc/knobs.cpp
+++ b/image-caption_amd/csrc/knobs.cpp
@@ -22,6 +22,7 @@
     {Knob::FusedQkv, "FUSED_QKV", 1, false},
     {Knob::FusedAttnBwd, "FUSED_ATTN_BWD", 1, false},
     {Knob::ColsumSide, "COLSUM_SIDE", 1, false},
+    {Knob::DwColsum, "DW_COLSUM", 1, false},
     {Knob::DecodeCrossMfma, "DECODE_CROSS_MFMA", 1, false},
     {Knob::SlabDecode, "SLAB_DECODE", 1, false},
     {Knob::DecodeGroupLds, "DECODE_GROUP_LDS", 1, false},
diff --git a/image-caption_amd/csrc/qkv_attn.hip b/image-caption_amd/csrc/qkv_attn.hip
--- a/image-caption_amd/csrc/qkv_attn.hip
+++ b/image-caption_amd/csrc/qkv_attn.hip
@@ -16,6 +16,7 @@
 
 __device__ __forceinline__ int xswz(int row, int chunk) { return chunk ^ (row & 15); }
 __device__ int32_t g_qa_dummy[64];
+__device__ uint64_t g_qa_dummy_seed;
 
 template <int LT>
 __device__ __forceinline__ void dma_rows(const bf16* rows, int64_t ld, int L, char* xs, int w, int lane) {
@@ -66,6 +67,7 @@
   for (int kk = 0; kk < QKB; ++kk)
 #pragma unroll
     for (int f = 0; f < NF; ++f) bq[0][kk][f] = *reinterpret_cast<const bf16x8*>(wrow[f] + 512 * kk);
+  const uint64_t seed = *opaque(g.drop.seed_ptr ? g.drop.seed_ptr : &g_qa_dummy_seed);
   {
     dma_rows<LT>(xb, a.ldx, L, xs, w, lane);
     uint4 kv[2][2];
@@ -157,7 +159,7 @@
     }
   }
   __syncthreads();
-  attn_fwd_staged(g, a.o, nullptr, b, h, sm);
+  attn_fwd_staged(g, a.o, nullptr, b, h, sm, &seed);
 }
 
 template <int LT>
@@ -185,6 +187,7 @@
   bf16x8 bq[QKS];
 #pragma unroll
   for (int ks = 0; ks < QKS; ++ks) bq[ks] = *reinterpret_cast<const bf16x8*>(wrow + 512 * ks);
+  const uint64_t seed = *opaque(g.drop.seed_ptr ? g.drop.seed_ptr : &g_qa_dummy_seed);
   dma_rows<LT>(a.dA + (int64_t)b * L * a.ldda, a.ldda, L, xs, w, lane);
   const int bk = g.kv_bmod ? b % g.kv_bmod : b;
   const bf16* src[3] = {reinterpret_cast<const bf16*>(g.k) + (int64_t)bk * g.k_bs + h * DK,
@@ -243,7 +246,7 @@
     if (w == 0) kok[lane] = lane < g.Lk && (!g.key_valid || kvl != 0) && (!g.key_ids || kid != g.pad_idx);
   }
   __syncthreads();
-  attn_bwd_staged(g, a.dq, a.dk, a.dv, b, h, Kimg, dOimg, Qimg, Vimg, Pdimg, dSimg, kok);
+  attn_bwd_staged(g, a.dq, a.dk, a.dv, b, h, Kimg, dOimg, Qimg, Vimg, Pdimg, dSimg, kok, &seed);
 }
 
 __global__ void __launch_bounds__(256) tile_weights_t_kernel(const bf16* __restrict__ src, int64_t ld,
diff --git a/include/capgen.h b/include/capgen.h
--- a/include/capgen.h
+++ b/include/capgen.h
@@ -95,6 +95,8 @@
                       void* C, int64_t ldc, int in_dtype, int out_dtype, const float* bias, float alpha, int beta,
                       int relu, void* stream);
 
+int capgen_debug_gemm_dw(int n, const int32_t* mnk, void* const* ptrs, const int64_t* lds, int stripes,
+                         int64_t stripe_stride, int single, void* stream);
 int capgen_debug_gemm_tiled(int M, int N, int K, const void* A, int64_t lda, const void* B, int64_t ldb, int tb,
                             void* Bt, void* C, int64_t ldc, int out_dtype, const float* bias, int beta, int relu,
                             const void* aux, int64_t ldaux, void* stream);
@@ -109,6 +111,7 @@
 int capgen_debug_splitk_diag(int* out4, int reset);
 int capgen_debug_gemm_timing_buf(void* dev_buf);
 int capgen_debug_copy_buffer(capgen_t* h, int which, void* host_dst, int64_t bytes);
+int64_t capgen_debug_tiled_bytes(capgen_t* h);
 
 int capgen_train_step_indexed(capgen_t* h, const void* feat_store, int feats_dtype, const float* pos_store,
                               int n_images, const int32_t* img_idx, const int32_t* caps, int B, int N, int T,
```

New measurement: 23980 images/s, median of 6. No clear change (+0.7%).
